# caki35/UNet-Torch

Measured on AMD Instinct MI355X. Metric: images/sec training step, 4-level U-Net 1ch→2cls 512×512, at 1/2/4/8 MI355X, higher is better.
Workload: dtype f16

## Files before the change

include/unetmi.h:

```cpp
#ifndef UNETMI_H
#define UNETMI_H
#include <stddef.h>
#include <stdint.h>

#ifdef __cplusplus
extern "C" {
#endif

typedef void* umi_stream_t;

enum { UMI_F32 = 0, UMI_F16 = 1 };
enum { UMI_OK = 0, UMI_ERR_BADARG = -1, UMI_ERR_UNSUPPORTED = -2, UMI_ERR_WORKSPACE = -3 };
enum { UMI_CONV_UPSAMPLE2 = 1,
       UMI_CONV_FORCE_GENERIC = 2,
       UMI_CONV_DGRAD_STRIDED = 4,
       UMI_CONV_ACCUMULATE = 8,
       UMI_CONV_F32_MFMA = 16,
       UMI_CONV_F32_MFMA_1X1 = 32   };

int umi_version(void);
const char* umi_arch(void);

int umi_tune_conv3x3_impl(int impl);

int umi_pack_kn(const float* src, void* dst, int T, int K, int N, long st, long sk, long sn,
                int flip_t, int Kpad, int Npad, int dtype, umi_stream_t stream);

int umi_pack_kn8(const float* src, void* dst, int T, int K, int N, long st, long sk, long sn,
                 int flip_t, int Kpad, int Npad, int dtype, umi_stream_t stream);

int umi_conv_fwd(const void* x, int ldx, const void* tx, const void* wp, const float* bias,
                 void* y, int ldy, float* stat_part,
                 int N, int H, int W, int Ci, int Co, int R, int S, int stride, int pad,
                 int Ho, int Wo, int off_h, int off_w, int out_H, int out_W,
                 int in_dtype, int out_dtype, int flags, umi_stream_t stream);
int umi_linear_fused(const void* x, int ldx, const void* wp8, const float* bias, void* y, int ldy, long M, int Ci, int Co,
                     int epi, float p, unsigned seed, const unsigned* seed_dev, void* mask, const void* aux, int ldaux,
                     void* y2, int ldy2, int dtype, umi_stream_t stream);

int umi_conv_fwd_plan(int N, int H, int W, int Ci, int Co, int R, int S, int stride, int pad,
                      int ldx, int ldy, int in_dtype, int out_dtype, int flags, int has_bias,
                      int* layout, int* stat_rows);

int umi_bn_finalize(const float* stat_part, int rows, int C, double count,
                    const float* gamma, const float* beta, float eps, float momentum,
                    float* running_mean, float* running_var,
                    void* tx_out, float* rstd_out, umi_stream_t stream);

int umi_pool2_fwd(const void* x, int ldx, const void* tx, void* y, int ldy,
                  int N, int H, int W, int C, int dtype, umi_stream_t stream);
int umi_pool2_bwd(const void* dpool, int lddp, const void* x, int ldx, const void* tx,
                  void* da, int ldda, int accumulate,
                  int N, int H, int W, int C, int dtype, umi_stream_t stream);

size_t umi_bn_bwd_ws_bytes(long M, int C);
int umi_bn_bwd_reduce(const void* da, int ldda, const void* y, int ldy, const void* tx,
                      const float* rstd, float* sum_dz, float* sum_dzx,
                      long M, int C, int dtype, void* ws, size_t ws_bytes, umi_stream_t stream);
int umi_bn_bwd_apply(void* da, int ldda, const void* y, int ldy, const void* tx,
                     const float* rstd, const float* sum_dz, const float* sum_dzx,
                     long M, int C, int dtype, umi_stream_t stream);

int umi_conv_dgrad_bnred(const void* dy, int lddy, const void* wp8, void* da, int ldda, const void* ybn, int ldybn,
                         const void* txbn, const float* rstd, float* part, int N, int H, int W, int Ci, int Co,
                         int dtype, umi_stream_t stream);

int umi_conv_gather_bnred_rows(int N, int H, int W, int Ci, int Co, int R, int S, int stride, int pad, int Ho, int Wo,
                               int ldx, int ldy, int dtype, int flags);
int umi_conv_gather_bnred(const void* x, int ldx, const void* wp8, void* y, int ldy, const void* ybn, int ldybn,
                          const void* txbn, const float* rstd, float* part, int N, int H, int W, int Ci, int Co, int R, int S,
                          int stride, int pad, int Ho, int Wo, int dtype, int flags, umi_stream_t stream);

int umi_head_dgrad_bnred_rows(long P, int Ci, int Co, int ldda, int dtype);
int umi_head_dgrad_bnred(const void* dl, int lddl, const void* wp, void* da, int ldda, const void* ybn, int ldybn,
                         const void* txbn, const float* rstd, float* part, long P, int Ci, int Co, int dtype,
                         umi_stream_t stream);
size_t umi_head_bwd_fused_ws_bytes(long P, int Ci, int Co);
int umi_head_bwd_fused(const void* dl, int lddl, const void* wp, void* da, int ldda, const void* ybn, int ldybn,
                       const void* txbn, const float* rstd, float* part, float* dW, long s_co, long s_ci, float out_scale,
                       void* ws, size_t ws_bytes, long P, int Ci, int Co, int dtype, umi_stream_t stream);

int umi_conv3x3_fwd_act(const void* x, int ldx, const void* tx, const void* wp8, const void* out_tx, void* y, int ldy,
                        int N, int H, int W, int Ci, int Co, int dtype, umi_stream_t stream);
int umi_bn_stats_rows(long M, int C);
int umi_bn_stats(const void* x, int ldx, float* part, long M, int C, int dtype, umi_stream_t stream);
int umi_pool2_bwd_bnred_stat_rows(int N, int H, int W, int C);
int umi_pool2_bwd_bnred(const void* dpool, int lddp, const void* x, int ldx, const void* tx, const float* rstd, void* da,
                        int ldda, int accumulate, float* part, int N, int H, int W, int C, int dtype, umi_stream_t stream);
int umi_bn_bwd_from_partials(const float* part, int rows, int C, float* sum_dz, float* sum_dzx, umi_stream_t stream);

size_t umi_conv_wgrad_ws_bytes(int N, int Ho, int Wo, int Ci, int Co, int R, int S, int dtype, int flags);
int umi_conv_wgrad(const void* x, int ldx, const void* txa, const void* dy, int lddy, const void* txb,
                   float* dW, long s_co, long s_ci, long s_t, float out_scale,
                   int N, int H, int W, int Ci, int Co, int R, int S, int stride, int pad,
                   int Ho, int Wo, int dtype, int flags, void* ws, size_t ws_bytes, umi_stream_t stream);
typedef struct umi_wgrad_pending {
    const float* part;
    float* dW;
    long s_co, s_ci, s_t;
    float scale;
    int splits, RS, Ci, Co;
} umi_wgrad_pending;
int umi_conv_wgrad_deferred(const void* x, int ldx, const void* txa, const void* dy, int lddy, const void* txb,
                            float* dW, long s_co, long s_ci, long s_t, float out_scale, int N, int H, int W, int Ci, int Co,
                            int R, int S, int stride, int pad, int Ho, int Wo, int dtype, int flags, void* ws, size_t ws_bytes,
                            umi_wgrad_pending* out, umi_stream_t stream);
int umi_wgrad_reduce_group(int n, const void* items , umi_stream_t stream);
int umi_conv_wgrad_bias(const void* x, int ldx, const void* dy, int lddy, const void* txb, float* dW, long s_co, long s_ci,
                        long s_t, float* dbias, float out_scale, int N, int H, int W, int Ci, int Co, int Ho, int Wo, int dtype,
                        int flags, void* ws, size_t ws_bytes, umi_wgrad_pending* out, umi_stream_t stream);
int umi_conv_wgrad_group(int n, const void* const* x, int ldx, const void* const* dy, int lddy, float* const* dW, long s_co,
                         long s_ci, float out_scale, long M, int Ci, int Co, int dtype, umi_stream_t stream);
int umi_conv_wgrad_bnapply(const void* x, int ldx, const void* txa, const void* da, int ldda, const void* y, int ldy,
                           const void* tx_bn, const float* rstd, const float* sum_dz, const float* sum_dzx, void* dz,
                           int lddz, float* dW, long s_co, long s_ci, long s_t, float out_scale, int N, int H, int W,
                           int Ci, int Co, int R, int S, int stride, int pad, int dtype, int flags, void* ws,
                           size_t ws_bytes, umi_stream_t stream);

size_t umi_colsum_ws_bytes(long M, int C);
int umi_colsum(const void* x, int ldx, float* out, float out_scale, long M, int C, int dtype,
               void* ws, size_t ws_bytes, umi_stream_t stream);
int umi_colsum_group(int n, const void* const* xs, int ldx, float* const* outs, float out_scale, long M, int C, int dtype,
                     void* ws, size_t ws_bytes, umi_stream_t stream);

int umi_materialize_nchw(const void* x, int ldx, const void* tx, float* y_nchw,
                         int N, int H, int W, int C, int dtype, umi_stream_t stream);


int umi_wstd_fwd(const float* w, float* wstd, float* rstd, int Co, int K, float eps, umi_stream_t stream);
int umi_wstd_bwd(const float* wstd, const float* rstd, const float* g, float* dw, int Co, int K, umi_stream_t stream);
typedef struct umi_wstd_desc {
    const float* w;
    float* ws;
    float* rstd;
    long off;
    int Co, K;
    float eps;
    int blk0;
    float* dw;
} umi_wstd_desc;
int umi_wstd_fwd_multi(const void* descs, int n_desc, int total_rows, umi_stream_t stream);
int umi_wstd_bwd_multi(const void* descs, int n_desc, int total_rows, const float* g_base, float* dw_base, umi_stream_t stream);

size_t umi_gn_fwd_ws_bytes(int N, long HW, int C);
int umi_gn_fwd(const void* x, int ldx, const float* gamma, const float* beta, const void* res, int ldr, void* y, int ldy,
               float* mean, float* rstd, int relu, int N, long HW, int C, int G, float eps, int dtype,
               void* ws, size_t ws_bytes, umi_stream_t stream);
size_t umi_gn_bwd_ws_bytes(int N, long HW, int C, int G);
int umi_gn_bwd(const void* dy, int lddy, const void* y, int ldy, const void* x, int ldx, const float* mean,
               const float* rstd, const float* gamma, int relu, void* dx, int lddx, void* dres, int lddr,
               float* dgamma, float* dbeta, float out_scale, int N, long HW, int C, int G, int dtype,
               void* ws, size_t ws_bytes, float* part_out, umi_stream_t stream);
int umi_gn_param_grads_group(int n, const float* const* parts, const int* Cs, int N, float* const* dgammas,
                             float* const* dbetas, float out_scale, umi_stream_t stream);

int umi_pool3s2_fwd(const void* x, int ldx, void* y, int ldy, void* idx, int N, int H, int W, int C, int dtype,
                    umi_stream_t stream);
int umi_pool3s2_bwd(const void* dy, int lddy, const void* x, int ldx, const void* idx, void* dx, int lddx, int N, int H, int W,
                    int C, int dtype, umi_stream_t stream);

int umi_ln_fwd(const void* x, int ldx, const float* gamma, const float* beta, void* y, int ldy, float* mean, float* rstd,
               long M, int C, float eps, int dtype, umi_stream_t stream);
size_t umi_ln_bwd_ws_bytes(long M, int C);
int umi_ln_bwd(const void* dy, int lddy, const void* x, int ldx, const float* gamma, const float* mean,
               const float* rstd, void* dx, int lddx, float* dgamma, float* dbeta, float out_scale, long M, int C,
               int dtype, void* ws, size_t ws_bytes, int* rows_out, umi_stream_t stream);

int umi_elementwise(int mode, const void* x, int ldx, const void* g, int ldg, void* y, int ldy, long M, int C,
                    long bcast_rows, int dtype, umi_stream_t stream);

int umi_dropout(const void* x, int ldx, void* y, int ldy, void* mask, int backward, float p, unsigned seed, long M, int C,
                int dtype, const void* tx, const unsigned* seed_dev, umi_stream_t stream);
int umi_dropout_fused(const void* x, int ldx, void* y, int ldy, void* mask, int backward, float p, unsigned seed, long M, int C,
                      int dtype, const unsigned* seed_dev, const void* aux, int ldaux, int gelu, umi_stream_t stream);

int umi_attn_fwd(const void* q, const void* k, const void* v, int ld, void* o, int ldo, float* lse, int B, int N, int heads,
                 int D, int dtype, umi_stream_t stream);
int umi_attn_bwd(const void* q, const void* k, const void* v, int ld, const void* o, const void* dO, int ldo,
                 const float* lse, void* dq, void* dk, void* dv, int ldd, float* delta, int B, int N, int heads, int D,
                 int dtype, umi_stream_t stream);
enum { UMI_ATTN_F32_MFMA = 1  };
int umi_attn_fwd_flags(const void* q, const void* k, const void* v, int ld, void* o, int ldo, float* lse, int B, int N, int heads,
                       int D, int dtype, int flags, umi_stream_t stream);
int umi_attn_bwd_flags(const void* q, const void* k, const void* v, int ld, const void* o, const void* dO, int ldo,
                       const float* lse, void* dq, void* dk, void* dv, int ldd, float* delta, int B, int N, int heads, int D,
                       int dtype, int flags, umi_stream_t stream);
int umi_attn_plan(int N, int heads, int D, int ld, int ldo, int ldd, int dtype, int flags, const void* q, const void* k,
                  const void* v, const void* o, int* kernel);

int umi_bilinear2x(const void* x, int ldx, const void* tx, void* y, int ldy, int backward, int N, int H, int W, int C,
                   int dtype, umi_stream_t stream);

size_t umi_dice_ce_ws_bytes(int N, int C, long HW);
int umi_dice_ce_fwd(const float* logits, const void* target, int target_dtype, int N, int C, long HW, float* stats, void* ws,
                    size_t ws_bytes, umi_stream_t stream);
int umi_dice_ce_bwd(const float* logits, const void* target, int target_dtype, const float* stats, const float* gout, int N,
                    int C, long HW, float* dlogits, umi_stream_t stream);

size_t umi_hdt_ws_bytes(int B, int H, int W);
int umi_hdt_fwd(const float* pred, const float* target, int B, int C, int H, int W, float alpha, float* D, float* fields,
                float* loss, void* ws, size_t ws_bytes, umi_stream_t stream);
int umi_hdt_bwd(const float* pred, const float* target, const float* D, const float* gout, int B, int C, int H, int W,
                float* dpred, umi_stream_t stream);

size_t umi_binloss_ws_bytes(int B, int C, long HW);
int umi_dice_bce_fwd(const float* pred, const float* target, int B, long HW, double* stats, float* loss, void* ws,
                     size_t ws_bytes, umi_stream_t stream);
int umi_dice_bce_bwd(const float* pred, const float* target, const double* stats, const float* gout, int B, long HW,
                     float* dpred, umi_stream_t stream);
int umi_tversky_fwd(const float* pred, const void* target, int target_dtype, int B, int C, long HW, float alpha, float beta,
                    double* stats, float* loss, void* ws, size_t ws_bytes, umi_stream_t stream);
int umi_tversky_bwd(const float* pred, const void* target, int target_dtype, const double* stats, const float* gout, int B,
                    int C, long HW, float alpha, float beta, float* dpred, umi_stream_t stream);

size_t umi_topk_loss_ws_bytes(long N);
int umi_topk_loss_fwd(const float* pred, const float* target, long N, long k, int mode, unsigned char* mask, float* loss,
                      void* ws, size_t ws_bytes, umi_stream_t stream);
int umi_topk_loss_bwd(const float* pred, const float* target, const unsigned char* mask, const float* gout, long N, long k,
                      float* dpred, umi_stream_t stream);

size_t umi_mt_ratio_ws_bytes(int B, long HW);
size_t umi_mt_ratio_stats_len(int B);
int umi_mt_ratio_fwd(const float* o1, const float* o2, const float* l1, const float* l2, int B, long HW, int gate,
                     const float* gate_dev, double* stats, float* loss, float* loss1, float* loss2, float* ratio, void* ws, size_t ws_bytes,
                     umi_stream_t stream);
int umi_mt_ratio_bwd(const float* o1, const float* o2, const float* l1, const float* l2, const double* stats,
                     const float* gout, int B, long HW, float* d1, float* d2, umi_stream_t stream);

typedef struct umi_optim_desc {
    float* p;
    const float* g;
    float* s0;
    float* s1;
    long n;
    int blk0;
    int pad_;
} umi_optim_desc;
int umi_optim_block_elems(void);
int umi_table_upload(const void* host_pinned, void* dev, size_t nbytes, umi_stream_t stream);
int umi_optim_sgd_multi(const void* descs, int n_desc, int total_blocks, double lr, double momentum, double dampening,
                        double weight_decay, int nesterov, int first_step, umi_stream_t stream);
int umi_optim_adam_multi(const void* descs, int n_desc, int total_blocks, double step_size, double beta1, double beta2,
                         double bc2_sqrt, double eps, double weight_decay, umi_stream_t stream);

typedef struct umi_optim_hyper {
    double lr, base_lr, iter, max_iter, power, adam_t, beta1, beta2;
    float lr_f, step_size_f, bc2_sqrt_f, pad_;
    double pad2_[2];
} umi_optim_hyper;
size_t umi_optim_hyper_bytes(void);
int umi_optim_hyper_pre(void* hyper, int adam, umi_stream_t stream);
int umi_optim_hyper_poly(void* hyper, umi_stream_t stream);
int umi_optim_sgd_multi_dev(const void* descs, int n_desc, int total_blocks, const void* hyper, double momentum,
                            double dampening, double weight_decay, int nesterov, int first_step, umi_stream_t stream);
int umi_optim_adam_multi_dev(const void* descs, int n_desc, int total_blocks, const void* hyper, double beta1, double beta2,
                             double eps, double weight_decay, umi_stream_t stream);

typedef struct umi_pack_desc {
    const float* src;
    void* dst;
    long st, sk, sn;
    int T, K, N, flip_t, Kpad, Npad, k8, blk0;
    int ldn, pad_;
} umi_pack_desc;
int umi_pack_block_elems(void);
int umi_pack_kn_multi(const void* descs, int n_desc, int total_blocks, int dtype, umi_stream_t stream);

int umi_add2_relu_fwd(const void* a, int lda, const void* txa, const void* b, int ldb, const void* txb, void* y, int ldy,
                      long M, int C, int dtype, umi_stream_t stream);
int umi_add2_relu_bwd(const void* dy, int lddy, const void* y, int ldy, void* da, int ldda, void* db, int lddb, long M, int C,
                      int dtype, umi_stream_t stream);
int umi_gate_fwd(const void* x, int ldx, const void* txx, const void* p, const void* txp, void* y, int ldy, long M, int C,
                 int dtype, umi_stream_t stream);
int umi_gate_bwd(const void* dy, int lddy, const void* x, int ldx, const void* txx, const void* p, const void* txp, void* dx,
                 int lddx, void* dp, long M, int C, int dtype, umi_stream_t stream);

size_t umi_znorm_ws_bytes(void);
int umi_znorm_hwc(const void* img, int src_dtype, float* out_chw, long HW, int C, int reverse_channels, void* ws,
                  size_t ws_bytes, umi_stream_t stream);
int umi_argmax_mask(const float* logits, unsigned char* mask, int N, int C, long HW, umi_stream_t stream);
size_t umi_zoom_cubic_ws_bytes(int H, int W, int C);
int umi_zoom_cubic_hwc(const void* img, int src_dtype, void* out, int H, int W, int C, int out_h, int out_w, void* ws,
                       size_t ws_bytes, umi_stream_t stream);

int umi_binary_mask(const float* logits, unsigned char* mask, long n, umi_stream_t stream);
int umi_zoom_nearest(const void* in, int dtype, void* out, int N, int H, int W, int out_h, int out_w, umi_stream_t stream);
size_t umi_sum_trunc_ws_bytes(int N);
int umi_sum_trunc(const float* x, int* out, int N, long HW, void* ws, size_t ws_bytes, umi_stream_t stream);

size_t umi_components_ws_bytes(int N, int H, int W);
int umi_components_cap(int H, int W);
int umi_count_components(const unsigned char* mask, int* counts, int N, int H, int W, void* ws, size_t ws_bytes,
                         umi_stream_t stream);
int umi_label_components(const unsigned char* mask, int* labels, int* counts, int* area, long long* sum_y, long long* sum_x,
                         int N, int H, int W, void* ws, size_t ws_bytes, umi_stream_t stream);

size_t umi_class_components_ws_bytes(int N, int H, int W, int n_classes);
int umi_count_class_components(const unsigned char* mask, int* class_counts, int N, int H, int W, int n_classes, void* ws,
                               size_t ws_bytes, umi_stream_t stream);
int umi_label_class_components(const unsigned char* mask, int* labels, int* counts, int* class_counts, unsigned char* label_class,
                               int* area, long long* sum_y, long long* sum_x, int N, int H, int W, int n_classes, int cap, void* ws,
                               size_t ws_bytes, umi_stream_t stream);

int umi_match_max_dots(void);
size_t umi_dot_lists_ws_bytes(int N, int H, int W);
int umi_dot_lists(const void* map, int dtype, int* dots, int* g_count, int N, int H, int W, int max_dots, void* ws, size_t ws_bytes,
                  umi_stream_t stream);
int umi_component_centers(const int* counts, const int* area, const long long* sum_y, const long long* sum_x, int* centers, int N,
                          int cap, umi_stream_t stream);
int umi_crowd_match(const int* dots, const int* g_count, int max_dots, const int* centers, const int* c_count, int cap,
                    const double* tables, size_t table_len, const int* radii, int S, const double* thresh, int T, int* out, int N,
                    umi_stream_t stream);
size_t umi_distance_match_ws_bytes(int N, int cap);
int umi_distance_match(const int* dots, const int* g_count, int max_dots, const int* centers, const int* c_count, int cap,
                       long long d2_max, int* out, int N, void* ws, size_t ws_bytes, umi_stream_t stream);
int umi_grid_sums(const void* map, int dtype, void* out, int N, int H, int W, int size, umi_stream_t stream);
int umi_scatter_centers(const int* centers, const int* c_count, int cap, unsigned char* map, int N, int H, int W,
                        umi_stream_t stream);
int umi_split_classes(const unsigned char* map, unsigned char* planes, int N, int H, int W, int n_classes, umi_stream_t stream);
int umi_class_center_lists(const int* counts, const unsigned char* label_class, const int* area, const long long* sum_y,
                           const long long* sum_x, int* centers, int* c_count, int N, int cap, int n_classes, umi_stream_t stream);

int umi_augment_geometry(const void* src, int dtype, void* dst, const int* params, const double* geom, int N, int H, int W, int C,
                         umi_stream_t stream);
int umi_augment_labels(const void* src, int src_dtype, void* dst, int dst_dtype, float scale, const int* params, const double* geom,
                       int N, int H, int W, int out_h, int out_w, umi_stream_t stream);
size_t umi_augment_znorm_ws_bytes(int N);
int umi_augment_znorm(const void* src, int dtype, float* out_nchw, const int* params, const double* geom, int N, int H, int W, int C,
                      int reverse_channels, void* ws, size_t ws_bytes, umi_stream_t stream);

#ifdef __cplusplus
}
#endif
#endif
```

unet-torch_amd/csrc/api.hip:

```cpp
#include "kernels.h"
#include <stdio.h>
#include <stdlib.h>

static ConvFwdProblem fwd_problem(int N, int H, int W, int Ci, int Co, int R, int S, int stride, int pad, int Ho, int Wo, int ldx,
                                  int ldy, int in_dtype, int out_dtype, int flags, bool has_tx, bool has_bias, bool has_stats) {
    return ConvFwdProblem{N, H, W, Ci, Co, R, S, stride, pad, Ho, Wo, ldx, ldy, in_dtype, out_dtype, flags, has_tx, has_bias, has_stats};
}
static ConvFwdProblem fwd_problem_3x3(int N, int H, int W, int Ci, int Co, int ldx, int ldy, int dtype, bool has_tx) {
    return fwd_problem(N, H, W, Ci, Co, 3, 3, 1, 1, H, W, ldx, ldy, dtype, dtype, 0, has_tx, false, false);
}

extern "C" int umi_version(void) { return 1; }
extern "C" const char* umi_arch(void) { return "gfx950"; }

extern "C" int umi_linear_fused(const void* x, int ldx, const void* wp8, const float* bias, void* y, int ldy, long M, int Ci,
                                int Co, int epi, float p, unsigned seed, const unsigned* seed_dev, void* mask, const void* aux,
                                int ldaux, void* y2, int ldy2, int dtype, umi_stream_t stream) {
    if (!x || !wp8 || !y || !mask || M <= 0 || M >= (1L << 31) || Ci <= 0 || Co <= 0 || !(p >= 0.f && p <= 1.f)) return UMI_ERR_BADARG;
    if (epi != 1 && epi != 2) return UMI_ERR_BADARG;
    if ((epi == 1 && (!y2 || ldy2 % 8)) || (epi == 2 && (!aux || ldaux % 8))) return UMI_ERR_BADARG;
    const ConvFwdProblem pr = fwd_problem(1, 1, (int)M, Ci, Co, 1, 1, 1, 0, 1, (int)M, ldx, ldy, dtype, dtype, 0, false, bias != nullptr, false);
    if (umi_conv_fwd_path(pr) != FWD_MFMA1X1) return UMI_ERR_UNSUPPORTED;
    if (((uintptr_t)x | (uintptr_t)y | (uintptr_t)wp8 | (uintptr_t)y2 | (uintptr_t)aux) & 15 || ((uintptr_t)mask & 7)) return UMI_ERR_UNSUPPORTED;
    const UmiLinearEpi e{epi, p, seed, seed_dev, mask, aux, ldaux, y2, ldy2, nullptr, nullptr, nullptr};
    return umi_conv1x1_mfma(pr, x, nullptr, wp8, bias, y, 0, 0, 1, (int)M, (hipStream_t)stream, &e);
}

extern "C" int umi_conv_gather_bnred_rows(int N, int H, int W, int Ci, int Co, int R, int S, int stride, int pad, int Ho, int Wo,
                                          int ldx, int ldy, int dtype, int flags) {
    if (flags & (UMI_CONV_UPSAMPLE2 | UMI_CONV_ACCUMULATE | UMI_CONV_FORCE_GENERIC)) return 0;
    const ConvFwdProblem p = fwd_problem(N, H, W, Ci, Co, R, S, stride, pad, Ho, Wo, ldx, ldy, dtype, dtype, flags, false, false, false);
    if (umi_conv_fwd_path(p) != FWD_MFMA1X1 || umi_conv3x3_mfma_ok(p)) return 0;
    return umi_conv1x1_bnred_rows((long)N * Ho * Wo, Co);
}
extern "C" int umi_conv_gather_bnred(const void* x, int ldx, const void* wp8, void* y, int ldy, const void* ybn, int ldybn,
                                     const void* txbn, const float* rstd, float* part, int N, int H, int W, int Ci, int Co, int R,
                                     int S, int stride, int pad, int Ho, int Wo, int dtype, int flags, umi_stream_t stream) {
    if (!x || !wp8 || !y || !ybn || !txbn || !rstd || !part || N <= 0 || H <= 0 || W <= 0) return UMI_ERR_BADARG;
    if (umi_conv_gather_bnred_rows(N, H, W, Ci, Co, R, S, stride, pad, Ho, Wo, ldx, ldy, dtype, flags) <= 0 || ldybn % 8 || ldybn < Co)
        return UMI_ERR_UNSUPPORTED;
    if (((uintptr_t)x | (uintptr_t)y | (uintptr_t)wp8 | (uintptr_t)ybn) & 15) return UMI_ERR_BADARG;
    const UmiLinearEpi e{3, 0.f, 0u, nullptr, nullptr, ybn, ldybn, nullptr, 0, txbn, rstd, part};
    const ConvFwdProblem p = fwd_problem(N, H, W, Ci, Co, R, S, stride, pad, Ho, Wo, ldx, ldy, dtype, dtype, flags, false, false, false);
    return umi_conv1x1_mfma(p, x, nullptr, wp8, nullptr, y, 0, 0, Ho, Wo, (hipStream_t)stream, &e);
}

extern "C" int umi_conv_fwd_plan(int N, int H, int W, int Ci, int Co, int R, int S, int stride, int pad, int ldx,
                                 int ldy, int in_dtype, int out_dtype, int flags, int has_bias, int* layout,
                                 int* stat_rows) {
    if (N <= 0 || H <= 0 || W <= 0 || Ci <= 0 || Co <= 0 || R <= 0 || S <= 0 || stride <= 0) return UMI_ERR_BADARG;
    const bool ups = flags & UMI_CONV_UPSAMPLE2;
    const int Ho = ups ? H : (H + 2 * pad - R) / stride + 1, Wo = ups ? W : (W + 2 * pad - S) / stride + 1;
    const ConvFwdPath path = umi_conv_fwd_path(fwd_problem(N, H, W, Ci, Co, R, S, stride, pad, Ho, Wo, ldx, ldy, in_dtype, out_dtype,
                                                           flags, false, has_bias != 0, true));
    if ((flags & UMI_CONV_ACCUMULATE) && path != FWD_MFMA1X1) return UMI_ERR_UNSUPPORTED;
    if (layout) *layout = (path == FWD_MFMA3X3 || path == FWD_MFMA1X1) ? 1 : 0;
    if (stat_rows)
        *stat_rows = path == FWD_MFMA3X3_F32 ? umi_conv3x3_f32_mfma_stat_rows(N, H, W)
                     : path == FWD_GEMM_F32 ? umi_gemm_f32_mfma_stat_rows((long)N * H * W)
                     : path == FWD_MFMA3X3 ? umi_conv3x3_mfma_stat_rows(N, H, W, Co)
                     : path == FWD_STEM  ? umi_stem_stat_rows(N, H, W)
                     : path == FWD_HEAD  ? umi_head_stat_rows((long)N * H * W, Ci)
                                         : umi_cdiv((long)N * Ho * Wo, 64);
    return UMI_OK;
}

extern "C" int umi_conv_dgrad_bnred(const void* dy, int lddy, const void* wp8, void* da, int ldda, const void* ybn, int ldybn,
                                    const void* txbn, const float* rstd, float* part, int N, int H, int W, int Ci, int Co,
                                    int dtype, umi_stream_t stream) {
    if (!dy || !wp8 || !da || !ybn || !txbn || !rstd || !part || N <= 0 || H <= 0 || W <= 0) return UMI_ERR_BADARG;
    const ConvFwdProblem p = fwd_problem_3x3(N, H, W, Ci, Co, lddy, ldda, dtype, false);
    if (umi_conv_fwd_path(p) != FWD_MFMA3X3 || ldybn % 8 || ldybn < Co) return UMI_ERR_UNSUPPORTED;
    if (((uintptr_t)dy | (uintptr_t)da | (uintptr_t)wp8 | (uintptr_t)ybn) & 15) return UMI_ERR_BADARG;
    return umi_conv3x3_mfma_bnred(p, dy, wp8, da, ybn, ldybn, txbn, rstd, part, (hipStream_t)stream);
}

static bool head_dgrad_ok(int Ci, int Co, int ldda, int dtype) {
    return umi_smallk_fwd_ok(fwd_problem(1, 1, 1, Ci, Co, 1, 1, 1, 0, 1, 1, Ci, ldda, dtype, dtype, 0, false, false, false));
}
extern "C" int umi_head_dgrad_bnred_rows(long P, int Ci, int Co, int ldda, int dtype) {
    if (!head_dgrad_ok(Ci, Co, ldda, dtype)) return 0;
    return umi_smallk_bnred_rows(P, Co);
}
extern "C" int umi_head_dgrad_bnred(const void* dl, int lddl, const void* wp, void* da, int ldda, const void* ybn, int ldybn,
                                    const void* txbn, const float* rstd, float* part, long P, int Ci, int Co, int dtype,
                                    umi_stream_t stream) {
    if (!dl || !wp || !da || !ybn || !txbn || !rstd || !part || P <= 0) return UMI_ERR_BADARG;
    if (!head_dgrad_ok(Ci, Co, ldda, dtype) || ldybn % 8 || ldybn < Co || lddl < Ci) return UMI_ERR_UNSUPPORTED;
    return umi_smallk_fwd_bnred(dl, lddl, wp, da, ldda, ybn, ldybn, txbn, rstd, part, P, Ci, Co, (hipStream_t)stream);
}
extern "C" size_t umi_head_bwd_fused_ws_bytes(long P, int Ci, int Co) {
    return (size_t)umi_smallk_bnred_rows(P, Co) * Co * Ci * sizeof(float);
}
extern "C" int umi_head_bwd_fused(const void* dl, int lddl, const void* wp, void* da, int ldda, const void* ybn, int ldybn,
                                  const void* txbn, const float* rstd, float* part, float* dW, long s_co, long s_ci, float out_scale,
                                  void* ws, size_t ws_bytes, long P, int Ci, int Co, int dtype, umi_stream_t stream) {
    if (!dl || !wp || !da || !ybn || !txbn || !rstd || !part || !dW || !ws || P <= 0) return UMI_ERR_BADARG;
    if (!head_dgrad_ok(Ci, Co, ldda, dtype) || Co > 256 || ldybn % 8 || ldybn < Co || lddl < Ci) return UMI_ERR_UNSUPPORTED;
    return umi_smallk_fwd_bnred(dl, lddl, wp, da, ldda, ybn, ldybn, txbn, rstd, part, P, Ci, Co, (hipStream_t)stream, dW, s_co, s_ci,
                                out_scale, ws, ws_bytes);
}

extern "C" int umi_conv3x3_fwd_act(const void* x, int ldx, const void* tx, const void* wp8, const void* out_tx, void* y, int ldy,
                                   int N, int H, int W, int Ci, int Co, int dtype, umi_stream_t stream) {
    if (!x || !wp8 || !out_tx || !y || N <= 0 || H <= 0 || W <= 0 || ldx < Ci || ldy < Co) return UMI_ERR_BADARG;
    const ConvFwdProblem p = fwd_problem_3x3(N, H, W, Ci, Co, ldx, ldy, dtype, tx != nullptr);
    if (umi_conv_fwd_path(p) != FWD_MFMA3X3) return UMI_ERR_UNSUPPORTED;
    if (((uintptr_t)x | (uintptr_t)y | (uintptr_t)wp8 | (uintptr_t)out_tx) & 15) return UMI_ERR_BADARG;
    return umi_conv3x3_mfma_act(p, x, tx, wp8, out_tx, y, (hipStream_t)stream);
}

extern "C" int umi_bn_stats_rows(long M, int C) { return umi_colsum_rows_f16v(M, C); }
extern "C" int umi_bn_stats(const void* x, int ldx, float* part, long M, int C, int dtype, umi_stream_t stream) {
    if (!x || !part || M <= 0 || C <= 0 || ldx < C) return UMI_ERR_BADARG;
    if (dtype != UMI_F16 || !umi_bn_stats_f16v(x, ldx, part, M, C, (hipStream_t)stream)) return UMI_ERR_UNSUPPORTED;
    UMI_LAUNCH_CHECK();
    return UMI_OK;
}

extern "C" int umi_pool2_bwd_bnred(const void* dpool, int lddp, const void* x, int ldx, const void* tx, const float* rstd,
                                   void* da, int ldda, int accumulate, float* part, int N, int H, int W, int C, int dtype,
                                   umi_stream_t stream) {
    if (!dpool || !x || !tx || !rstd || !da || !part || N <= 0 || H <= 0 || W <= 0 || C <= 0) return UMI_ERR_BADARG;
    if (dtype != UMI_F16) return UMI_ERR_UNSUPPORTED;
    if (!umi_pool2_bwd_bnred_f16v(dpool, lddp, x, ldx, tx, rstd, da, ldda, accumulate, part, N, H, W, C, (hipStream_t)stream))
        return UMI_ERR_UNSUPPORTED;
    UMI_LAUNCH_CHECK();
    return UMI_OK;
}
extern "C" int umi_pool2_bwd_bnred_stat_rows(int N, int H, int W, int C) { return umi_pool2_bwd_bnred_rows(N, H, W, C); }

extern "C" int umi_bn_bwd_from_partials(const float* part, int rows, int C, float* sum_dz, float* sum_dzx, umi_stream_t stream) {
    if (!part || !sum_dz || !sum_dzx || rows <= 0 || C <= 0) return UMI_ERR_BADARG;
    umi_launch_reduce_rows2(part, rows, C, sum_dz, sum_dzx, 1.f, (hipStream_t)stream);
    UMI_LAUNCH_CHECK();
    return UMI_OK;
}

static bool trace_generic() {
    static const bool on = [] { const char* e = getenv("UMI_TRACE_GENERIC"); return e && e[0] == '1'; }();
    return on;
}
#define UMI_TRACE(kind)                                                                                                  \
    if (trace_generic())                                                                                                 \
        fprintf(stderr, "[umi generic %s] N=%d H=%d W=%d Ci=%d Co=%d R=%d stride=%d pad=%d flags=%d\n", kind, N, H, W, Ci, Co, R, \
                stride, pad, flags)

extern "C" int umi_conv_fwd(const void* x, int ldx, const void* tx, const void* wp, const float* bias, void* y, int ldy,
                            float* stat_part, int N, int H, int W, int Ci, int Co, int R, int S, int stride, int pad,
                            int Ho, int Wo, int off_h, int off_w, int out_H, int out_W, int in_dtype, int out_dtype,
                            int flags, umi_stream_t stream) {
    if (!x || !wp || !y || N <= 0 || H <= 0 || W <= 0 || Ci <= 0 || Co <= 0 || R <= 0 || S <= 0 || stride <= 0 ||
        Ho <= 0 || Wo <= 0 || ldx < Ci || ldy < Co || out_H <= 0 || out_W <= 0)
        return UMI_ERR_BADARG;
    ConvFwdProblem p = fwd_problem(N, H, W, Ci, Co, R, S, stride, pad, Ho, Wo, ldx, ldy, in_dtype, out_dtype, flags,
                                   tx != nullptr, bias != nullptr, stat_part != nullptr);
    const ConvFwdPath path = umi_conv_fwd_path(p);
    if (path != FWD_MFMA3X3_F32 && path != FWD_GEMM_F32) p.flags = flags &= ~UMI_CONV_F32_OPT_IN;
    if ((flags & UMI_CONV_ACCUMULATE) && (stat_part || path != FWD_MFMA1X1)) return UMI_ERR_UNSUPPORTED;
    if (flags & UMI_CONV_DGRAD_STRIDED) {
        if (flags & UMI_CONV_UPSAMPLE2) return UMI_ERR_BADARG;
        if (H != (Ho + 2 * pad - R) / stride + 1 || W != (Wo + 2 * pad - S) / stride + 1) return UMI_ERR_BADARG;
        if (out_H != Ho || out_W != Wo || off_h || off_w || stat_part) return UMI_ERR_BADARG;
    } else if (!(flags & UMI_CONV_UPSAMPLE2)) {
        if (Ho != (H + 2 * pad - R) / stride + 1 || Wo != (W + 2 * pad - S) / stride + 1) return UMI_ERR_BADARG;
        if (out_H != Ho || out_W != Wo || off_h || off_w) return UMI_ERR_BADARG;
    } else {
        if (Ho != H || Wo != W) return UMI_ERR_BADARG;
    }
    const hipStream_t s = (hipStream_t)stream;
    switch (path) {
    case FWD_MFMA3X3_F32: return umi_conv3x3_f32_mfma(p, x, tx, wp, y, stat_part, s);
    case FWD_GEMM_F32: return umi_gemm_f32_mfma(p, x, tx, wp, bias, y, stat_part, s);
    case FWD_MFMA3X3:
        if (((uintptr_t)x | (uintptr_t)y | (uintptr_t)wp) & 15) return UMI_ERR_BADARG;
        return umi_conv3x3_mfma(p, x, tx, wp, y, stat_part, s);
    case FWD_MFMA1X1:
        if (stat_part) return UMI_ERR_UNSUPPORTED;
        if (((uintptr_t)x | (uintptr_t)y | (uintptr_t)wp) & 15) return UMI_ERR_BADARG;
        return umi_conv1x1_mfma(p, x, tx, wp, bias, y, off_h, off_w, out_H, out_W, s);
    case FWD_STEM: return umi_stem_fwd(p, x, tx, wp, y, stat_part, s);
    case FWD_HEAD: return umi_head_fwd(p, x, tx, wp, bias, y, stat_part, s);
    case FWD_SMALLK: return umi_smallk_fwd(p, x, wp, y, s);
    case FWD_ROOT: return umi_root_fwd(p, x, wp, y, s);
    case FWD_HEAD3: return umi_head3_fwd(p, x, tx, wp, bias, y, s);
    case FWD_GENERIC: break;
    }
    UMI_TRACE((flags & UMI_CONV_DGRAD_STRIDED) ? "dgrad_strided" : "fwd");
    return umi_conv_fwd_generic(p, x, tx, wp, bias, y, stat_part, off_h, off_w, out_H, out_W, s);
}

static WgradProblem wgrad_problem(int N, int H, int W, int Ci, int Co, int R, int S, int stride, int pad, int Ho, int Wo, int ldx,
                                  int lddy, int dtype, int flags, bool has_txa, bool has_txb) {
    return WgradProblem{N, H, W, Ci, Co, R, S, stride, pad, Ho, Wo, ldx, lddy, dtype, flags, has_txa, has_txb};
}

extern "C" size_t umi_conv_wgrad_ws_bytes(int N, int Ho, int Wo, int Ci, int Co, int R, int S, int dtype, int flags) {
    WgradProblem p = wgrad_problem(N, 0, 0, Ci, Co, R, S, 0, 0, Ho, Wo, 0, 0, dtype, flags, false, false);
    const size_t f32_mfma = umi_wgrad3x3_f32_mfma_ws_bound(p), f32_gemm = umi_wgrad_gemm_f32_mfma_ws_bound(p);
    p.flags &= ~UMI_CONV_F32_OPT_IN;
    const size_t bounds[] = {f32_mfma, f32_gemm, umi_wgrad3x3_mfma_ws_bound(p), umi_wgrad1x1_mfma_ws_bound(p), umi_wgradT_mfma_ws_bound(p),
                             umi_wgrad_gather_mfma_ws_bound(p), umi_stem_wgrad_ws_bound(p), umi_head_wgrad_ws_bound(p),
                             umi_root_wgrad_ws_bound(p), umi_head3_wgrad_ws_bound(p), umi_conv_wgrad_generic_ws_bound(p)};
    size_t most = 0;
    for (size_t b : bounds) most = b > most ? b : most;
    return most;
}

static int conv_wgrad(const WgradProblem& asked, WgradPath path, const void* x, const void* txa, const void* dy, const void* txb,
                      const WgradOut& o, hipStream_t s) {
    WgradProblem p = asked;
    if (path != WGRAD_MFMA3X3_F32 && path != WGRAD_GEMM_F32) p.flags &= ~UMI_CONV_F32_OPT_IN;
    if (!x || !dy || !o.dW || !o.ws || p.N <= 0 || p.H <= 0 || p.W <= 0 || p.Ci <= 0 || p.Co <= 0 || p.ldx < p.Ci || p.lddy < p.Co)
        return UMI_ERR_BADARG;
    switch (path) {
    case WGRAD_MFMA3X3_F32: return umi_wgrad3x3_f32_mfma(p, x, txa, dy, o, s);
    case WGRAD_GEMM_F32: return umi_wgrad_gemm_f32_mfma(p, x, txa, dy, o, s);
    case WGRAD_MFMA3X3: return umi_wgrad3x3_mfma(p, x, txa, dy, o, s);
    case WGRAD_MFMA1X1: return umi_wgrad1x1_mfma(p, x, txa, dy, o, s);
    case WGRAD_T: return umi_wgradT_mfma(p, x, dy, txb, o, s);
    case WGRAD_GATHER: return umi_wgrad_gather_mfma(p, x, txa, dy, o, s);
    case WGRAD_STEM: return umi_stem_wgrad(p, x, txa, dy, o, s);
    case WGRAD_HEAD: return umi_head_wgrad(p, x, txa, dy, o, s);
    case WGRAD_ROOT: return umi_root_wgrad(p, x, dy, o, s);
    case WGRAD_HEAD3: return umi_head3_wgrad(p, x, txa, dy, o, s);
    case WGRAD_GENERIC: break;
    }
    if (trace_generic())
        fprintf(stderr, "[umi generic wgrad] N=%d H=%d W=%d Ci=%d Co=%d R=%d stride=%d pad=%d flags=%d\n", p.N, p.H, p.W, p.Ci, p.Co,
                p.R, p.stride, p.pad, p.flags);
    return umi_conv_wgrad_generic(p, x, txa, dy, txb, o, s);
}

extern "C" int umi_conv_wgrad(const void* x, int ldx, const void* txa, const void* dy, int lddy, const void* txb,
                              float* dW, long s_co, long s_ci, long s_t, float out_scale, int N, int H, int W, int Ci,
                              int Co, int R, int S, int stride, int pad, int Ho, int Wo, int dtype, int flags, void* ws,
                              size_t ws_bytes, umi_stream_t stream) {
    const WgradProblem p = wgrad_problem(N, H, W, Ci, Co, R, S, stride, pad, Ho, Wo, ldx, lddy, dtype, flags, txa != nullptr, txb != nullptr);
    const WgradOut o{dW, s_co, s_ci, s_t, out_scale, ws, ws_bytes, nullptr, nullptr};
    return conv_wgrad(p, umi_conv_wgrad_path(p), x, txa, dy, txb, o, (hipStream_t)stream);
}

extern "C" int umi_conv_wgrad_deferred(const void* x, int ldx, const void* txa, const void* dy, int lddy, const void* txb,
                                       float* dW, long s_co, long s_ci, long s_t, float out_scale, int N, int H, int W, int Ci,
                                       int Co, int R, int S, int stride, int pad, int Ho, int Wo, int dtype, int flags, void* ws,
                                       size_t ws_bytes, umi_wgrad_pending* out, umi_stream_t stream) {
    if (!out) return UMI_ERR_BADARG;
    out->part = nullptr;
    const WgradProblem p = wgrad_problem(N, H, W, Ci, Co, R, S, stride, pad, Ho, Wo, ldx, lddy, dtype, flags, txa != nullptr, txb != nullptr);
    const WgradOut o{dW, s_co, s_ci, s_t, out_scale, ws, ws_bytes, out, nullptr};
    return conv_wgrad(p, umi_conv_wgrad_path(p), x, txa, dy, txb, o, (hipStream_t)stream);
}

extern "C" int umi_conv_wgrad_bias(const void* x, int ldx, const void* dy, int lddy, const void* txb, float* dW, long s_co,
                                   long s_ci, long s_t, float* dbias, float out_scale, int N, int H, int W, int Ci, int Co, int Ho,
                                   int Wo, int dtype, int flags, void* ws, size_t ws_bytes, umi_wgrad_pending* out,
                                   umi_stream_t stream) {
    if (!dbias) return UMI_ERR_BADARG;
    const WgradProblem p = wgrad_problem(N, H, W, Ci, Co, 2, 2, 2, 0, Ho, Wo, ldx, lddy, dtype, flags, false, txb != nullptr);
    if (umi_conv_wgrad_path(p) != WGRAD_T) return UMI_ERR_UNSUPPORTED;
    if (out) out->part = nullptr;
    const WgradOut o{dW, s_co, s_ci, s_t, out_scale, ws, ws_bytes, out, dbias};
    return conv_wgrad(p, WGRAD_T, x, nullptr, dy, txb, o, (hipStream_t)stream);
}

extern "C" int umi_conv_wgrad_group(int n, const void* const* x, int ldx, const void* const* dy, int lddy, float* const* dW,
                                    long s_co, long s_ci, float out_scale, long M, int Ci, int Co, int dtype,
                                    umi_stream_t stream) {
    if (n <= 0 || !x || !dy || !dW || M <= 0 || Ci <= 0 || Co <= 0 || ldx < Ci || lddy < Co) return UMI_ERR_BADARG;
    for (int i = 0; i < n; ++i)
        if (!x[i] || !dy[i] || !dW[i]) return UMI_ERR_BADARG;
    if (M >= (1L << 31) ||
        umi_conv_wgrad_path(wgrad_problem(1, 1, (int)M, Ci, Co, 1, 1, 1, 0, 1, (int)M, ldx, lddy, dtype, 0, false, false)) != WGRAD_MFMA1X1)
        return UMI_ERR_UNSUPPORTED;
    return umi_wgrad1x1_mfma_group(n, x, ldx, dy, lddy, dW, s_co, s_ci, out_scale, M, Ci, Co, (hipStream_t)stream);
}

extern "C" int umi_conv_wgrad_bnapply(const void* x, int ldx, const void* txa, const void* da, int ldda, const void* y, int ldy,
                                      const void* tx_bn, const float* rstd, const float* sum_dz, const float* sum_dzx,
                                      void* dz, int lddz, float* dW, long s_co, long s_ci, long s_t, float out_scale, int N,
                                      int H, int W, int Ci, int Co, int R, int S, int stride, int pad, int dtype, int flags,
                                      void* ws, size_t ws_bytes, umi_stream_t stream) {
    if (!x || !da || !y || !tx_bn || !rstd || !sum_dz || !sum_dzx || !dW || !ws || N <= 0 || H <= 0 || W <= 0 || Ci <= 0 ||
        Co <= 0 || ldx < Ci || ldda < Co || ldy < Co || (dz && (lddz < Co || dz == da || dz == y)))
        return UMI_ERR_BADARG;
    const WgradProblem p = wgrad_problem(N, H, W, Ci, Co, R, S, stride, pad, H, W, ldx, ldda, dtype, flags, txa != nullptr, false);
    const WgradPath path = umi_conv_wgrad_path(p);
    const WgradOut o{dW, s_co, s_ci, s_t, out_scale, ws, ws_bytes, nullptr, nullptr};
    const WgradBnApply bna{y, ldy, tx_bn, rstd, sum_dz, sum_dzx, dz, lddz};
    if (!dz) {
        if (path != WGRAD_STEM || ldy % 8) return UMI_ERR_UNSUPPORTED;
        return umi_stem_wgrad(p, x, txa, da, o, (hipStream_t)stream, &bna);
    }
    if (path != WGRAD_MFMA3X3 || ldy % 8 || lddz % 8 || (long)H * W * (ldy > lddz ? ldy : lddz) * 2 >= 0x7FFFFFF0L)
        return UMI_ERR_UNSUPPORTED;
    return umi_wgrad3x3_mfma(p, x, txa, da, o, (hipStream_t)stream, &bna);
}
```

unet-torch_amd/csrc/generic_kernels.hip:

```cpp
#include "kernels.h"

template <typename T, bool K8>
__global__ void pack_kn_kernel(const float* __restrict__ src, T* __restrict__ dst, int Tn, int K, int N,
                               long st, long sk, long sn, int flip_t, int Kpad, int Npad) {
    long total = (long)Tn * Kpad * Npad;
    for (long i = (long)blockIdx.x * blockDim.x + threadIdx.x; i < total; i += (long)gridDim.x * blockDim.x) {
        int n, k, t;
        if (K8) {
            int k8 = (int)(i & 7);
            long r = i >> 3;
            n = (int)(r % Npad); r /= Npad;
            int kb = (int)(r % (Kpad / 8));
            t = (int)(r / (Kpad / 8));
            k = kb * 8 + k8;
        } else {
            n = (int)(i % Npad);
            long r = i / Npad;
            k = (int)(r % Kpad);
            t = (int)(r / Kpad);
        }
        float v = 0.f;
        if (k < K && n < N) {
            int ts = flip_t ? (Tn - 1 - t) : t;
            v = src[ts * st + k * sk + n * sn];
// ... 523 lines not shown
            vs[i] = ws[((long)rc * 2 + 0) * C + c];
            vq[i] = ws[((long)rc * 2 + w1) * C + c];
        }
#pragma unroll
        for (int i = 0; i < 8; ++i) asm volatile("" : "+v"(vs[i]), "+v"(vq[i]));
#pragma unroll
        for (int i = 0; i < 8; ++i) { const bool ok = r0 + 256 * i < rows; vs[i] = ok ? vs[i] : 0.f; vq[i] = (ok && out1) ? vq[i] : 0.f; }
#pragma unroll
        for (int i = 0; i < 8; ++i) { s += (double)vs[i]; q += (double)vq[i]; }
    }
    sh[0][tid] = s;
    sh[1][tid] = q;
    __syncthreads();
    for (int o = 128; o > 0; o >>= 1) {
        if (tid < o) { sh[0][tid] += sh[0][tid + o]; sh[1][tid] += sh[1][tid + o]; }
        __syncthreads();
    }
    if (tid == 0) {
        out0[c] = (float)(sh[0][0] * (double)scale);
        if (out1) out1[c] = (float)(sh[1][0] * (double)scale);
    }
}

__global__ __launch_bounds__(256) void reduce_rows2_2d_kernel(const float* __restrict__ ws, int rows, int C,
                                                              float* __restrict__ out0, float* __restrict__ out1,
                                                              float scale, int region) {
    double tot = 0.0;
    if (!red2d_block(ws, rows, C, out1 != nullptr, region, tot)) return;
    const int lane = threadIdx.x & 63, c = blockIdx.x * 32 + (lane & 31);
    if (c < C) {
        if (lane < 32) out0[c] = (float)(tot * (double)scale);
        else if (out1) out1[c] = (float)(tot * (double)scale);
    }
}

__global__ __launch_bounds__(256) void reduce_rows2_wide_kernel(const float* __restrict__ ws, int rows, int C,
                                                                float* __restrict__ out0, float* __restrict__ out1, float scale) {
    const int c = blockIdx.x * 256 + threadIdx.x;
    if (c >= C) return;
    double s = 0.0, q = 0.0;
    for (int r = 0; r < rows; ++r) {
        s += (double)ws[((long)r * 2 + 0) * C + c];
        if (out1) q += (double)ws[((long)r * 2 + 1) * C + c];
    }
    out0[c] = (float)(s * (double)scale);
    if (out1) out1[c] = (float)(q * (double)scale);
}

void umi_launch_reduce_rows2(const float* ws, int rows, int C, float* out0, float* out1, float scale, hipStream_t s) {
    if (rows <= 64 && C >= 4096)
        hipLaunchKernelGGL(reduce_rows2_wide_kernel, dim3((C + 255) / 256), dim3(256), 0, s, ws, rows, C, out0, out1, scale);
    else if (red2d_ok(rows, C))
        hipLaunchKernelGGL(reduce_rows2_2d_kernel, dim3((C + 31) / 32, (rows + RED_RPS - 1) / RED_RPS), dim3(256), 0, s, ws,
                           rows, C, out0, out1, scale, red2d_region());
    else
        hipLaunchKernelGGL(reduce_rows2_kernel, dim3(C), dim3(256), 0, s, ws, rows, C, out0, out1, scale);
}

template <typename T>
__global__ void bn_bwd_apply_kernel(T* __restrict__ da, int ldda, const T* __restrict__ y, int ldy,
                                    const float4* __restrict__ tx, const float* __restrict__ rstd,
                                    const float* __restrict__ sum_dz, const float* __restrict__ sum_dzx, long M, int C) {
    const float invM = 1.f / (float)M;
    long total = M * C;
    for (long i = (long)blockIdx.x * blockDim.x + threadIdx.x; i < total; i += (long)gridDim.x * blockDim.x) {
        int c = (int)(i % C);
        long r = i / C;
        da[r * ldda + c] = umi_bn_dz<T>((float)y[r * ldy + c], (float)da[r * ldda + c], tx[c], rstd[c], sum_dz[c] * invM,
                                        sum_dzx[c] * invM);
    }
}

extern "C" size_t umi_bn_bwd_ws_bytes(long M, int C) {
    const int a = umi_cdiv(M, BNB_RPB), b = umi_cdiv(M, umi_bn_bwd_rpb_f16v(M));
    return (size_t)(a > b ? a : b) * 2 * (size_t)C * sizeof(float);
}

extern "C" int umi_bn_bwd_reduce(const void* da, int ldda, const void* y, int ldy, const void* tx, const float* rstd,
                                 float* sum_dz, float* sum_dzx, long M, int C, int dtype, void* ws, size_t ws_bytes,
                                 umi_stream_t stream) {
    if (!da || !y || !tx || !rstd || M <= 0 || C <= 0) return UMI_ERR_BADARG;
    if (ws_bytes < umi_bn_bwd_ws_bytes(M, C)) return UMI_ERR_WORKSPACE;
    int rows = umi_cdiv(M, BNB_RPB);
    hipStream_t s = (hipStream_t)stream;
    if (dtype == UMI_F16 && umi_bn_bwd_reduce1_f16v(da, ldda, y, ldy, tx, rstd, (float*)ws, M, C, s)) {
        UMI_LAUNCH_CHECK();
        rows = umi_cdiv(M, umi_bn_bwd_rpb_f16v(M));
        umi_launch_reduce_rows2((const float*)ws, rows, C, sum_dz, sum_dzx, 1.f, s);
        UMI_LAUNCH_CHECK();
        return UMI_OK;
    }
    if (dtype == UMI_F32) hipLaunchKernelGGL(bn_bwd_reduce1_kernel<float>, dim3(rows), dim3(256), 0, s, (const float*)da, ldda, (const float*)y, ldy, (const float4*)tx, rstd, (float*)ws, M, C);
    else if (dtype == UMI_F16) hipLaunchKernelGGL(bn_bwd_reduce1_kernel<half_t>, dim3(rows), dim3(256), 0, s, (const half_t*)da, ldda, (const half_t*)y, ldy, (const float4*)tx, rstd, (float*)ws, M, C);
    else return UMI_ERR_BADARG;
    UMI_LAUNCH_CHECK();
    umi_launch_reduce_rows2((const float*)ws, rows, C, sum_dz, sum_dzx, 1.f, s);
    UMI_LAUNCH_CHECK();
    return UMI_OK;
}

extern "C" int umi_bn_bwd_apply(void* da, int ldda, const void* y, int ldy, const void* tx, const float* rstd,
                                const float* sum_dz, const float* sum_dzx, long M, int C, int dtype,
                                umi_stream_t stream) {
    if (!da || !y || !tx || !rstd || M <= 0 || C <= 0) return UMI_ERR_BADARG;
    long total = M * C;
    int grid = (int)((total + 255) / 256);
    if (grid > 16384) grid = 16384;
    hipStream_t s = (hipStream_t)stream;
    if (dtype == UMI_F16 && umi_bn_bwd_apply_f16v(da, ldda, y, ldy, tx, rstd, sum_dz, sum_dzx, M, C, s)) {
        UMI_LAUNCH_CHECK();
        return UMI_OK;
    }
    if (dtype == UMI_F32) hipLaunchKernelGGL(bn_bwd_apply_kernel<float>, dim3(grid), dim3(256), 0, s, (float*)da, ldda, (const float*)y, ldy, (const float4*)tx, rstd, sum_dz, sum_dzx, M, C);
    else if (dtype == UMI_F16) hipLaunchKernelGGL(bn_bwd_apply_kernel<half_t>, dim3(grid), dim3(256), 0, s, (half_t*)da, ldda, (const half_t*)y, ldy, (const float4*)tx, rstd, sum_dz, sum_dzx, M, C);
    else return UMI_ERR_BADARG;
    UMI_LAUNCH_CHECK();
    return UMI_OK;
}

template <typename T>
__global__ __launch_bounds__(256) void colsum1_kernel(const T* __restrict__ x, int ldx, float* __restrict__ ws, long M,
                                                      int C, long rows_per_split, float* __restrict__ out, float scale) {
    __shared__ float red[4][64];
    const int cl = threadIdx.x & 63, rl = threadIdx.x >> 6;
    const int c = blockIdx.x * 64 + cl;
    const long r0 = (long)blockIdx.y * rows_per_split;
    long r1 = r0 + rows_per_split;
    if (r1 > M) r1 = M;
    float s = 0.f;
    if (c < C)
        for (long r = r0 + rl; r < r1; r += 4) s += (float)x[r * ldx + c];
    red[rl][cl] = s;
    __syncthreads();
    if (rl == 0 && c < C) {
        const float t = red[0][cl] + red[1][cl] + red[2][cl] + red[3][cl];
        if (gridDim.y == 1) out[c] = t * scale;
        else ws[((long)blockIdx.y * 2 + 0) * C + c] = t;
    }
}

__global__ void fold_cols_kernel(const float* __restrict__ tmp8, int C, float* __restrict__ out, float scale) {
    const int c = threadIdx.x;
    if (c < C) {
        float s = 0.f;
        for (int k = c; k < 8; k += C) s += tmp8[k];
        out[c] = s * scale;
    }
}

static void colsum_plan(long M, int C, int* splits, long* rps) {
    long ctiles = (C + 63) / 64;
    long want = (1024 + ctiles - 1) / ctiles;
    long maxs = (M + 31) / 32;
    if (want > maxs) want = maxs;
    if (want < 1) want = 1;
    *rps = (M + want - 1) / want;
    *splits = (int)((M + *rps - 1) / *rps);
}

extern "C" size_t umi_colsum_ws_bytes(long M, int C) {
    int splits; long rps;
    colsum_plan(M, C, &splits, &rps);
    const int vrows = umi_colsum_rows_f16v(M, C);
    size_t b = (size_t)(splits > vrows ? splits : vrows) * 2 * (size_t)C * sizeof(float);
    if (C < 8 && 8 % C == 0 && (M * C) % 8 == 0) {
        const size_t b8 = ((size_t)umi_colsum_rows_f16v(M * C / 8, 8) * 2 * 8 + 8) * sizeof(float);
        if (b8 > b) b = b8;
    }
    return b;
}

extern "C" int umi_colsum_group(int n, const void* const* xs, int ldx, float* const* outs, float out_scale, long M, int C,
                                int dtype, void* ws, size_t ws_bytes, umi_stream_t stream) {
    if (n <= 0 || !xs || !outs || M <= 0 || C <= 0 || !ws) return UMI_ERR_BADARG;
    for (int i = 0; i < n; ++i)
        if (!xs[i] || !outs[i]) return UMI_ERR_BADARG;
    if (ws_bytes < (size_t)(n < 16 ? n : 16) * umi_colsum_ws_bytes(M, C)) return UMI_ERR_WORKSPACE;
    if (dtype != UMI_F16 || !umi_colsum_group_f16v(n, xs, ldx, outs, out_scale, (float*)ws, M, C, (hipStream_t)stream))
        return UMI_ERR_UNSUPPORTED;
    UMI_LAUNCH_CHECK();
    return UMI_OK;
}

extern "C" int umi_colsum(const void* x, int ldx, float* out, float out_scale, long M, int C, int dtype, void* ws,
                          size_t ws_bytes, umi_stream_t stream) {
    if (!x || !out || M <= 0 || C <= 0) return UMI_ERR_BADARG;
    if (ws_bytes < umi_colsum_ws_bytes(M, C)) return UMI_ERR_WORKSPACE;
    int splits; long rps;
    colsum_plan(M, C, &splits, &rps);
    hipStream_t s = (hipStream_t)stream;
    if (dtype == UMI_F16 && umi_colsum_f16v(x, ldx, (float*)ws, M, C, s)) {
        UMI_LAUNCH_CHECK();
        umi_launch_reduce_rows2((const float*)ws, umi_colsum_rows_f16v(M, C), C, out, (float*)nullptr, out_scale, s);
        UMI_LAUNCH_CHECK();
        return UMI_OK;
    }
    if (dtype == UMI_F16 && C < 8 && 8 % C == 0 && ldx == C && (M * C) % 8 == 0 &&
        ws_bytes >= ((size_t)umi_colsum_rows_f16v(M * C / 8, 8) * 2 * 8 + 8) * sizeof(float)) {
        const long M8 = M * C / 8;
        float* tmp = (float*)ws + (size_t)umi_colsum_rows_f16v(M8, 8) * 2 * 8;
        if (umi_colsum_f16v(x, 8, (float*)ws, M8, 8, s)) {
            UMI_LAUNCH_CHECK();
            umi_launch_reduce_rows2((const float*)ws, umi_colsum_rows_f16v(M8, 8), 8, tmp, (float*)nullptr, 1.f, s);
            hipLaunchKernelGGL(fold_cols_kernel, dim3(1), dim3(64), 0, s, (const float*)tmp, C, out, out_scale);
            UMI_LAUNCH_CHECK();
            return UMI_OK;
        }
    }
    dim3 grid((C + 63) / 64, splits);
    if (dtype == UMI_F32) hipLaunchKernelGGL(colsum1_kernel<float>, grid, dim3(256), 0, s, (const float*)x, ldx, (float*)ws, M, C, rps, out, out_scale);
    else if (dtype == UMI_F16) hipLaunchKernelGGL(colsum1_kernel<half_t>, grid, dim3(256), 0, s, (const half_t*)x, ldx, (float*)ws, M, C, rps, out, out_scale);
    else return UMI_ERR_BADARG;
    UMI_LAUNCH_CHECK();
    if (splits > 1) {
        umi_launch_reduce_rows2((const float*)ws, splits, C, out, (float*)nullptr, out_scale, s);
        UMI_LAUNCH_CHECK();
    }
    return UMI_OK;
}

template <typename T>
__global__ __launch_bounds__(256) void wgrad_generic_kernel(
    const T* __restrict__ x, int ldx, const float4* __restrict__ txa, const T* __restrict__ dy, int lddy,
    const float4* __restrict__ txb, float* __restrict__ part, int N, int H, int W, int Ci, int Co, int R, int S,
    int stride, int pad, int Ho, int Wo, long chunk, int tiles_co) {
    __shared__ __attribute__((aligned(16))) float As[GBK][64 + 4];
    __shared__ __attribute__((aligned(16))) float Bs[GBK][64 + 4];
    const int tid = threadIdx.x;
    const int txi = tid & 15, tyi = tid >> 4;
    const int tile_ci = blockIdx.x / tiles_co, tile_co = blockIdx.x % tiles_co;
    const int ci0 = tile_ci * 64, co0 = tile_co * 64;
    const int tap = blockIdx.y;
    const int r = tap / S, s = tap - r * S;
    const long P = (long)N * Ho * Wo;
    const long k_begin = (long)blockIdx.z * chunk;
    long k_end = k_begin + chunk;
    if (k_end > P) k_end = P;

    const int lk = tid >> 4;
    const int lc = (tid & 15) * 4;
    float acc[4][4];
#pragma unroll
    for (int i = 0; i < 4; ++i)
#pragma unroll
        for (int j = 0; j < 4; ++j) acc[i][j] = 0.f;

    for (long k0 = k_begin; k0 < k_end; k0 += GBK) {
        long pg = k0 + lk;
        bool pv = pg < k_end;
        int n = 0, ho = 0, wo = 0;
        if (pv) {
            n = (int)(pg / ((long)Ho * Wo));
            int rem = (int)(pg - (long)n * Ho * Wo);
            ho = rem / Wo;
            wo = rem - ho * Wo;
        }
        int hi = ho * stride - pad + r, wi = wo * stride - pad + s;
        bool inb = pv && hi >= 0 && hi < H && wi >= 0 && wi < W;
        const T* xp = x + ((long)((long)n * H + hi) * W + wi) * ldx;
        const T* dp = dy + pg * lddy;
#pragma unroll
        for (int j = 0; j < 4; ++j) {
            int ci = ci0 + lc + j;
            float v = 0.f;
            if (inb && ci < Ci) {
                v = (float)xp[ci];
                if (txa) v = umi_tx(v, txa[ci]);
            }
            As[lk][lc + j] = v;
            int co = co0 + lc + j;
            float g = 0.f;
            if (pv && co < Co) {
                g = (float)dp[co];
                if (txb) g = umi_tx(g, txb[co]);
            }
            Bs[lk][lc + j] = g;
        }
        __syncthreads();
#pragma unroll
        for (int kk = 0; kk < GBK; ++kk) {
            float4 a = *(const float4*)&As[kk][tyi * 4];
            float4 b = *(const float4*)&Bs[kk][txi * 4];
            float av[4] = {a.x, a.y, a.z, a.w};
            float bv[4] = {b.x, b.y, b.z, b.w};
#pragma unroll
            for (int i = 0; i < 4; ++i)
#pragma unroll
                for (int j = 0; j < 4; ++j) acc[i][j] = fmaf(av[i], bv[j], acc[i][j]);
        }
        __syncthreads();
    }
#pragma unroll
    for (int i = 0; i < 4; ++i) {
        int ci = ci0 + tyi * 4 + i;
        if (ci >= Ci) continue;
#pragma unroll
        for (int j = 0; j < 4; ++j) {
            int co = co0 + txi * 4 + j;
            if (co < Co) part[(((long)blockIdx.z * R * S + tap) * Ci + ci) * Co + co] = acc[i][j];
        }
    }
}

__global__ __launch_bounds__(256) void wgrad_reduce_kernel(const float* __restrict__ part, int splits, int RS, int Ci,
                                                           int Co, float* __restrict__ dW, long s_co, long s_ci, long s_t,
                                                           float scale) {
    __shared__ float red[8][33];
    const long total = (long)RS * Ci * Co;
    const int ox = threadIdx.x & 31, sl = threadIdx.x >> 5;
    for (long base = (long)blockIdx.x * 32; base < total; base += (long)gridDim.x * 32) {
        long i = base + ox;
        float s = 0.f;
        if (i < total)
            for (int z = sl; z < splits; z += 8) s += part[(long)z * total + i];
        red[sl][ox] = s;
        __syncthreads();
        if (sl == 0 && i < total) {
            float a = 0.f;
#pragma unroll
            for (int k = 0; k < 8; ++k) a += red[k][ox];
            int co = (int)(i % Co);
            long rr = i / Co;
            int ci = (int)(rr % Ci);
            int t = (int)(rr / Ci);
            dW[co * s_co + ci * s_ci + t * s_t] = a * scale;
        }
        __syncthreads();
    }
}

__global__ __launch_bounds__(256) void wgrad_reduce_v4_kernel(const float* __restrict__ part, int splits, int RS, int Ci,
                                                              int Co, float* __restrict__ dW, long s_co, long s_ci, long s_t,
                                                              float scale) {
    __shared__ float4 red[8][33];
    const long total4 = (long)RS * Ci * Co / 4;
    const int Co4 = Co >> 2;
    const int ox = threadIdx.x & 31, sl = threadIdx.x >> 5;
    for (long base = (long)blockIdx.x * 32; base < total4; base += (long)gridDim.x * 32) {
        const long i = base + ox;
        float4 a = make_float4(0.f, 0.f, 0.f, 0.f), b = a;
        if (i < total4) {
            const float4* p = reinterpret_cast<const float4*>(part) + i;
            int z = sl;
            for (; z + 8 < splits; z += 16) {
                float4 u = p[(long)z * total4], v = p[(long)(z + 8) * total4];
                a.x += u.x; a.y += u.y; a.z += u.z; a.w += u.w;
                b.x += v.x; b.y += v.y; b.z += v.z; b.w += v.w;
            }
            if (z < splits) { float4 u = p[(long)z * total4]; a.x += u.x; a.y += u.y; a.z += u.z; a.w += u.w; }
        }
        red[sl][ox] = make_float4(a.x + b.x, a.y + b.y, a.z + b.z, a.w + b.w);
        __syncthreads();
        if (sl == 0 && i < total4) {
            float4 t4 = red[0][ox];
#pragma unroll
            for (int k = 1; k < 8; ++k) { float4 u = red[k][ox]; t4.x += u.x; t4.y += u.y; t4.z += u.z; t4.w += u.w; }
            const int co = (int)(i % Co4) * 4;
            const long rr = i / Co4;
            const int ci = (int)(rr % Ci), t = (int)(rr / Ci);
            float* o = dW + ci * s_ci + t * s_t;
            o[(co + 0) * s_co] = t4.x * scale;
            o[(co + 1) * s_co] = t4.y * scale;
            o[(co + 2) * s_co] = t4.z * scale;
            o[(co + 3) * s_co] = t4.w * scale;
        }
        __syncthreads();
    }
}

constexpr int WGT_CO = 32, WGT_CI = 8;
__host__ __device__ inline int wg_tmode(const umi_wgrad_pending& d) {
    if (d.Co % WGT_CO || d.Ci % WGT_CI || d.RS > 9 || d.s_t != 1 || (((uintptr_t)d.part) & 15)) return 0;
    if ((long)(d.Co / WGT_CO) * (d.Ci / WGT_CI) < 512) return 0;
    if (d.s_ci == d.RS && d.s_co == (long)d.Ci * d.RS) return 1;
    if (d.s_co == d.RS && d.s_ci == (long)d.Co * d.RS) return 2;
    return 0;
}
__device__ void wg_reduce_tiles(const umi_wgrad_pending& d, int mode, int my_blk, int n_blk) {
    __shared__ float4 redt[8][33];
    __shared__ float tile[WGT_CO * WGT_CI * 9 + 64];
    const int ox = threadIdx.x & 31, sl = threadIdx.x >> 5;
    const int RS = d.RS, ncob = d.Co / WGT_CO, ncib = d.Ci / WGT_CI, rows = WGT_CI * RS;
    const long total4 = (long)RS * d.Ci * d.Co / 4;
    for (int tl = my_blk; tl < ncob * ncib; tl += n_blk) {
        const int cob = tl % ncob, cib = tl / ncob;
        for (int r0 = 0; r0 < rows; r0 += 4) {
            const int row = r0 + (ox >> 3), c4 = ox & 7;
            const int tap = row / WGT_CI, cil = row - tap * WGT_CI;
            float4 a = make_float4(0.f, 0.f, 0.f, 0.f), b = a;
            if (row < rows) {
                const float4* p = reinterpret_cast<const float4*>(d.part) + (((long)tap * d.Ci + cib * WGT_CI + cil) * d.Co + cob * WGT_CO) / 4 + c4;
                int z = sl;
                for (; z + 8 < d.splits; z += 16) {
                    float4 u = p[(long)z * total4], v = p[(long)(z + 8) * total4];
                    a.x += u.x; a.y += u.y; a.z += u.z; a.w += u.w;
                    b.x += v.x; b.y += v.y; b.z += v.z; b.w += v.w;
                }
                if (z < d.splits) { float4 u = p[(long)z * total4]; a.x += u.x; a.y += u.y; a.z += u.z; a.w += u.w; }
                a = make_float4(a.x + b.x, a.y + b.y, a.z + b.z, a.w + b.w);
            }
            redt[sl][ox] = a;
            __syncthreads();
            if (sl == 0 && row < rows) {
                float4 t4 = redt[0][ox];
#pragma unroll
                for (int k = 1; k < 8; ++k) { float4 u = redt[k][ox]; t4.x += u.x; t4.y += u.y; t4.z += u.z; t4.w += u.w; }
                const float v[4] = {t4.x * d.scale, t4.y * d.scale, t4.z * d.scale, t4.w * d.scale};
#pragma unroll
                for (int k = 0; k < 4; ++k) {
                    const int co = c4 * 4 + k;
                    const int idx = mode == 1 ? co * (WGT_CI * RS + 1) + cil * RS + tap : cil * (WGT_CO * RS + 1) + co * RS + tap;
                    tile[idx] = v[k];
                }
            }
            __syncthreads();
        }
        const int inner = mode == 1 ? WGT_CI * RS : WGT_CO * RS, outer = mode == 1 ? WGT_CO : WGT_CI;
        for (int e = threadIdx.x; e < inner * outer; e += 256) {
            const int o = e / inner, r = e - o * inner;
            float* dst = mode == 1 ? d.dW + (long)(cob * WGT_CO + o) * d.s_co + (long)(cib * WGT_CI) * d.s_ci + r
                                   : d.dW + (long)(cib * WGT_CI + o) * d.s_ci + (long)(cob * WGT_CO) * d.s_co + r;
            *dst = tile[o * (inner + 1) + r];
        }
        __syncthreads();
    }
}

struct WgTable { umi_wgrad_pending e[16]; int blk0[17]; };
__global__ __launch_bounds__(256) void wgrad_reduce_group_kernel(WgTable t) {
    __shared__ float4 red[8][33];
    int ent = 0;
#pragma unroll
    for (int i = 1; i < 16; ++i) ent += (int)blockIdx.x >= t.blk0[i];
    const umi_wgrad_pending d = t.e[ent];
    const int my_blk = (int)blockIdx.x - t.blk0[ent], n_blk = t.blk0[ent + 1] - t.blk0[ent];
    if (const int tm = wg_tmode(d)) { wg_reduce_tiles(d, tm, my_blk, n_blk); return; }
    const int ox = threadIdx.x & 31, sl = threadIdx.x >> 5;
    const bool vec = d.Co % 4 == 0 && (((uintptr_t)d.part) & 15) == 0;
    const int W4 = vec ? 4 : 1;
    const long total = (long)d.RS * d.Ci * d.Co / W4;
    const int CoW = d.Co / W4;
    for (long base = (long)my_blk * 32; base < total; base += (long)n_blk * 32) {
        const long i = base + ox;
        float4 a = make_float4(0.f, 0.f, 0.f, 0.f), b = a;
        if (i < total) {
            if (vec) {
                const float4* p = reinterpret_cast<const float4*>(d.part) + i;
                int z = sl;
                for (; z + 8 < d.splits; z += 16) {
                    float4 u = p[(long)z * total], v = p[(long)(z + 8) * total];
                    a.x += u.x; a.y += u.y; a.z += u.z; a.w += u.w;
                    b.x += v.x; b.y += v.y; b.z += v.z; b.w += v.w;
                }
                if (z < d.splits) { float4 u = p[(long)z * total]; a.x += u.x; a.y += u.y; a.z += u.z; a.w += u.w; }
                a = make_float4(a.x + b.x, a.y + b.y, a.z + b.z, a.w + b.w);
            } else {
                for (int z = sl; z < d.splits; z += 8) a.x += d.part[(long)z * total + i];
            }
        }
        red[sl][ox] = a;
        __syncthreads();
        if (sl == 0 && i < total) {
            float4 t4 = red[0][ox];
            if (vec) {
#pragma unroll
                for (int k = 1; k < 8; ++k) { float4 u = red[k][ox]; t4.x += u.x; t4.y += u.y; t4.z += u.z; t4.w += u.w; }
            } else {
                float s0 = 0.f;
#pragma unroll
                for (int k = 0; k < 8; ++k) s0 += red[k][ox].x;
                t4.x = s0;
            }
            const int co = (int)(i % CoW) * W4;
            const long rr = i / CoW;
            const int ci = (int)(rr % d.Ci), tp = (int)(rr / d.Ci);
            float* o = d.dW + ci * d.s_ci + tp * d.s_t;
            o[(co + 0) * d.s_co] = t4.x * d.scale;
            if (vec) {
                o[(co + 1) * d.s_co] = t4.y * d.scale;
                o[(co + 2) * d.s_co] = t4.z * d.scale;
                o[(co + 3) * d.s_co] = t4.w * d.scale;
            }
        }
        __syncthreads();
    }
}

extern "C" int umi_wgrad_reduce_group(int n, const void* items, umi_stream_t stream) {
    if (n <= 0 || !items) return UMI_ERR_BADARG;
    const umi_wgrad_pending* it = (const umi_wgrad_pending*)items;
    for (int i = 0; i < n; ++i)
        if (!it[i].part || !it[i].dW || it[i].splits <= 0 || it[i].RS <= 0 || it[i].Ci <= 0 || it[i].Co <= 0) return UMI_ERR_BADARG;
    for (int g0 = 0; g0 < n; g0 += 16) {
        const int cnt = n - g0 < 16 ? n - g0 : 16;
        WgTable t;
        int total_blk = 0;
        for (int i = 0; i < 16; ++i) {
            t.e[i] = it[g0 + (i < cnt ? i : 0)];
            t.blk0[i] = total_blk;
            if (i >= cnt) continue;
            const bool vec = t.e[i].Co % 4 == 0 && (((uintptr_t)t.e[i].part) & 15) == 0;
            long g = ((long)t.e[i].RS * t.e[i].Ci * t.e[i].Co / (vec ? 4 : 1) + 31) / 32;
            if (wg_tmode(t.e[i])) g = (long)(t.e[i].Co / WGT_CO) * (t.e[i].Ci / WGT_CI);
            total_blk += (int)(g > 4096 ? 4096 : g);
        }
        t.blk0[16] = total_blk;
        hipLaunchKernelGGL(wgrad_reduce_group_kernel, dim3((unsigned)total_blk), dim3(256), 0, (hipStream_t)stream, t);
        UMI_LAUNCH_CHECK();
    }
    return UMI_OK;
}

void umi_launch_wgrad_reduce(int splits, int RS, int Ci, int Co, const WgradOut& o, hipStream_t st) {
    const float* part = (const float*)o.ws;
    float* const dW = o.dW;
    const long s_co = o.s_co, s_ci = o.s_ci, s_t = o.s_t;
    const float scale = o.out_scale;
    if (o.defer) {
        *o.defer = umi_wgrad_pending{part, dW, s_co, s_ci, s_t, scale, splits, RS, Ci, Co};
        return;
    }
    {
        const umi_wgrad_pending one{part, dW, s_co, s_ci, s_t, scale, splits, RS, Ci, Co};
        if (wg_tmode(one)) {
            WgTable t;
            for (int i = 0; i < 16; ++i) { t.e[i] = one; t.blk0[i] = 0; }
            long g = (long)(Co / WGT_CO) * (Ci / WGT_CI);
            if (g > 4096) g = 4096;
            for (int i = 1; i <= 16; ++i) t.blk0[i] = (int)g;
            hipLaunchKernelGGL(wgrad_reduce_group_kernel, dim3((unsigned)g), dim3(256), 0, st, t);
            return;
        }
    }
    if (Co % 4 == 0 && (((uintptr_t)part) & 15) == 0) {
        long g4 = ((long)RS * Ci * Co / 4 + 31) / 32;
        if (g4 > 16384) g4 = 16384;
        hipLaunchKernelGGL(wgrad_reduce_v4_kernel, dim3((unsigned)g4), dim3(256), 0, st, part, splits, RS, Ci, Co, dW, s_co, s_ci, s_t, scale);
        return;
    }
    long total = (long)RS * Ci * Co;
    long g = (total + 31) / 32;
    if (g > 16384) g = 16384;
    hipLaunchKernelGGL(wgrad_reduce_kernel, dim3((unsigned)g), dim3(256), 0, st, part, splits, RS, Ci, Co, dW, s_co, s_ci, s_t, scale);
}


static void wgrad_generic_plan(long P, int Ci, int Co, int RS, int* splits, long* chunk) {
    long tiles = (long)umi_cdiv(Ci, 64) * umi_cdiv(Co, 64) * RS;
    long want = (2048 + tiles - 1) / tiles;
    long maxs = (P + 255) / 256;
    if (want > maxs) want = maxs;
    if (want < 1) want = 1;
    long ch = (P + want - 1) / want;
    ch = (ch + GBK - 1) / GBK * GBK;
    *chunk = ch;
    *splits = (int)((P + ch - 1) / ch);
}

size_t umi_conv_wgrad_generic_ws_bound(const WgradProblem& p) {
    int splits; long chunk;
    wgrad_generic_plan((long)p.N * p.Ho * p.Wo, p.Ci, p.Co, p.R * p.S, &splits, &chunk);
    return (size_t)splits * p.R * p.S * p.Ci * p.Co * sizeof(float);
}

int umi_conv_wgrad_generic(const WgradProblem& p, const void* x, const void* txa, const void* dy, const void* txb,
                           const WgradOut& o, hipStream_t st) {
    const int N = p.N, H = p.H, W = p.W, Ci = p.Ci, Co = p.Co, R = p.R, S = p.S, stride = p.stride, pad = p.pad, Ho = p.Ho, Wo = p.Wo,
              ldx = p.ldx, lddy = p.lddy, dtype = p.dtype;
    void* const ws = o.ws;
    if (o.ws_bytes < umi_conv_wgrad_generic_ws_bound(p)) return UMI_ERR_WORKSPACE;
    int splits; long chunk;
    wgrad_generic_plan((long)N * Ho * Wo, Ci, Co, R * S, &splits, &chunk);
    const int tiles_co = umi_cdiv(Co, 64);
    dim3 grid(umi_cdiv(Ci, 64) * tiles_co, R * S, splits), block(256);
    if (dtype == UMI_F32) hipLaunchKernelGGL(wgrad_generic_kernel<float>, grid, block, 0, st, (const float*)x, ldx, (const float4*)txa, (const float*)dy, lddy, (const float4*)txb, (float*)ws, N, H, W, Ci, Co, R, S, stride, pad, Ho, Wo, chunk, tiles_co);
    else if (dtype == UMI_F16) hipLaunchKernelGGL(wgrad_generic_kernel<half_t>, grid, block, 0, st, (const half_t*)x, ldx, (const float4*)txa, (const half_t*)dy, lddy, (const float4*)txb, (float*)ws, N, H, W, Ci, Co, R, S, stride, pad, Ho, Wo, chunk, tiles_co);
    else return UMI_ERR_BADARG;
    UMI_LAUNCH_CHECK();
    umi_launch_wgrad_reduce(splits, R * S, Ci, Co, o, st);
    UMI_LAUNCH_CHECK();
    return UMI_OK;
}

template <typename T>
__global__ void materialize_nchw_kernel(const T* __restrict__ x, int ldx, const float4* __restrict__ tx,
                                        float* __restrict__ y, int N, int H, int W, int C) {
    long total = (long)N * C * H * W;
    for (long i = (long)blockIdx.x * blockDim.x + threadIdx.x; i < total; i += (long)gridDim.x * blockDim.x) {
        int w = (int)(i % W);
        long r = i / W;
        int h = (int)(r % H);
        r /= H;
        int c = (int)(r % C);
        int n = (int)(r / C);
        float v = (float)x[((long)((long)n * H + h) * W + w) * ldx + c];
        if (tx) v = umi_tx(v, tx[c]);
        y[i] = v;
    }
}

extern "C" int umi_materialize_nchw(const void* x, int ldx, const void* tx, float* y, int N, int H, int W, int C,
                                    int dtype, umi_stream_t stream) {
    if (!x || !y || N <= 0 || H <= 0 || W <= 0 || C <= 0) return UMI_ERR_BADARG;
    long total = (long)N * C * H * W;
    int grid = (int)((total + 255) / 256);
    if (grid > 16384) grid = 16384;
    hipStream_t s = (hipStream_t)stream;
    if (dtype == UMI_F32) hipLaunchKernelGGL(materialize_nchw_kernel<float>, dim3(grid), dim3(256), 0, s, (const float*)x, ldx, (const float4*)tx, y, N, H, W, C);
    else if (dtype == UMI_F16) hipLaunchKernelGGL(materialize_nchw_kernel<half_t>, dim3(grid), dim3(256), 0, s, (const half_t*)x, ldx, (const float4*)tx, y, N, H, W, C);
    else return UMI_ERR_BADARG;
    UMI_LAUNCH_CHECK();
    return UMI_OK;
}
```

unet-torch_amd/csrc/optim_kernels.hip:

```cpp
#include "common.h"
#include <stdint.h>

namespace {

constexpr int OPT_BLOCK = 4096;
constexpr int PACK_BLOCK = 2048;

template <typename D>
__device__ inline int find_desc(const D* d, int n, int blk) {
    int lo = 0, hi = n - 1;
    while (lo < hi) {
        int mid = (lo + hi + 1) >> 1;
        if (d[mid].blk0 <= blk) lo = mid; else hi = mid - 1;
    }
    return lo;
}

struct Hyper {
    double lr, base_lr, iter, max_iter, power, adam_t, beta1, beta2;
    float lr_f, step_size_f, bc2_sqrt_f, pad_;
    double pad2_[2];
};
static_assert(sizeof(Hyper) == 96, "umi_optim_hyper is 96 bytes");

struct SgdArgs { float lr, momentum, omd, wd; int nesterov, first; const Hyper* hp; };

__device__ inline void sgd_one(float& p, float g, float& m, const SgdArgs a) {
    if (a.wd != 0.f) g = fmaf(a.wd, p, g);
    if (a.momentum != 0.f) {
        if (a.first) m = g;
        else {
            float mm = __fmul_rn(m, a.momentum);
            m = a.omd == 1.f ? __fadd_rn(mm, g) : fmaf(a.omd, g, mm);
        }
        g = a.nesterov ? fmaf(a.momentum, m, g) : m;
    }
    p = fmaf(-a.lr, g, p);
}

struct AdamArgs { float step_size, omb1, beta2, omb2, bc2_sqrt, eps, wd; const Hyper* hp; };

__device__ inline void adam_one(float& p, float g, float& m, float& v, const AdamArgs a) {
    if (a.wd != 0.f) g = fmaf(a.wd, p, g);
    m = fmaf(a.omb1, g - m, m);
    v = fmaf(a.omb2 * g, g, __fmul_rn(v, a.beta2));
    const float denom = __fdiv_rn(__fsqrt_rn(v), a.bc2_sqrt) + a.eps;
    p = fmaf(-a.step_size, __fdiv_rn(m, denom), p);
}

template <bool ADAM, typename A>
__global__ __launch_bounds__(256) void optim_multi_kernel(const umi_optim_desc* __restrict__ descs, int n_desc, A a) {
    if (a.hp) {
        if constexpr (ADAM) { a.step_size = a.hp->step_size_f; a.bc2_sqrt = a.hp->bc2_sqrt_f; }
        else a.lr = a.hp->lr_f;
    }
    const int blk = blockIdx.x;
    const umi_optim_desc d = descs[find_desc(descs, n_desc, blk)];
    const long base = (long)(blk - d.blk0) * OPT_BLOCK;
    const long left = d.n - base;
    const int cnt = left < OPT_BLOCK ? (int)left : OPT_BLOCK;
    float* p = d.p + base;
    const float* g = d.g + base;
    float* s0 = d.s0 ? d.s0 + base : nullptr;
    float* s1 = d.s1 ? d.s1 + base : nullptr;
    const unsigned long al = (unsigned long)p | (unsigned long)g | (unsigned long)s0 | (unsigned long)s1;
    if ((al & 15) == 0) {
        for (int i = threadIdx.x * 4; i + 4 <= cnt; i += 1024) {
            float4 pv = *reinterpret_cast<float4*>(p + i);
            const float4 gv = *reinterpret_cast<const float4*>(g + i);
            float4 mv = s0 ? *reinterpret_cast<float4*>(s0 + i) : make_float4(0.f, 0.f, 0.f, 0.f);
            float4 vv = (ADAM && s1) ? *reinterpret_cast<float4*>(s1 + i) : make_float4(0.f, 0.f, 0.f, 0.f);
            if constexpr (ADAM) {
                adam_one(pv.x, gv.x, mv.x, vv.x, a); adam_one(pv.y, gv.y, mv.y, vv.y, a);
                adam_one(pv.z, gv.z, mv.z, vv.z, a); adam_one(pv.w, gv.w, mv.w, vv.w, a);
                *reinterpret_cast<float4*>(s1 + i) = vv;
            } else {
                sgd_one(pv.x, gv.x, mv.x, a); sgd_one(pv.y, gv.y, mv.y, a);
                sgd_one(pv.z, gv.z, mv.z, a); sgd_one(pv.w, gv.w, mv.w, a);
            }
            *reinterpret_cast<float4*>(p + i) = pv;
            if (s0) *reinterpret_cast<float4*>(s0 + i) = mv;
        }
        const int tail0 = cnt & ~3;
        const int i = tail0 + threadIdx.x;
        if (i < cnt) {
            float pv = p[i], mv = s0 ? s0[i] : 0.f;
            if constexpr (ADAM) { float vv = s1[i]; adam_one(pv, g[i], mv, vv, a); s1[i] = vv; }
            else sgd_one(pv, g[i], mv, a);
            p[i] = pv;
            if (s0) s0[i] = mv;
        }
    } else {
        for (int i = threadIdx.x; i < cnt; i += 256) {
            float pv = p[i], mv = s0 ? s0[i] : 0.f;
            if constexpr (ADAM) { float vv = s1[i]; adam_one(pv, g[i], mv, vv, a); s1[i] = vv; }
            else sgd_one(pv, g[i], mv, a);
            p[i] = pv;
            if (s0) s0[i] = mv;
        }
    }
}

constexpr int PT = 32;
template <typename T, int U>
__device__ __forceinline__ void pack_stage(const umi_pack_desc& d, T* tl, int k0, int n0, bool k_inner) {
    const int TT = d.T;
    for (int e0 = threadIdx.x; e0 < PT * PT * TT; e0 += 256 * U) {
        float v[U];
        int li[U];
        bool ok[U];
#pragma unroll
        for (int u = 0; u < U; ++u) {
            const int e = e0 + 256 * u;
            const int o_ = e / (PT * TT), r = e - o_ * (PT * TT);
            const int i_ = r / TT, t = r - i_ * TT;
            const int kl = k_inner ? i_ : o_, nl = k_inner ? o_ : i_;
            const int k = k0 + kl, n = n0 + nl;
            ok[u] = e < PT * PT * TT && k < d.K && n < d.N;
            li[u] = e < PT * PT * TT ? (t * PT + kl) * (PT + 2) + nl : -1;
            const int tc = t < TT ? t : TT - 1, kc = k < d.K ? k : d.K - 1, nc = n < d.N ? n : d.N - 1;
            v[u] = d.src[(long)(d.flip_t ? TT - 1 - tc : tc) * d.st + (long)kc * d.sk + (long)nc * d.sn];
        }
#pragma unroll
        for (int u = 0; u < U; ++u) asm volatile("" : "+v"(v[u]));
#pragma unroll
        for (int u = 0; u < U; ++u) v[u] = ok[u] ? v[u] : 0.f;
#pragma unroll
        for (int u = 0; u < U; ++u)
            if (li[u] >= 0) tl[li[u]] = (T)v[u];
    }
}

template <typename T>
__device__ void pack_tiles_k8(const umi_pack_desc& d, int my_blk, int n_blk) {
    __shared__ T tl[9 * PT * (PT + 2)];
    const int nkt = (d.Kpad + PT - 1) / PT, nnt = (d.Npad + PT - 1) / PT;
    const int kb8 = d.Kpad >> 3, ldn = d.ldn ? d.ldn : d.Npad, TT = d.T;
    const bool k_inner = d.sk <= d.sn;
    T* dst = (T*)d.dst;
    for (int tile = my_blk; tile < nkt * nnt; tile += n_blk) {
        const int k0 = (tile % nkt) * PT, n0 = (tile / nkt) * PT;
        if (TT == 9) pack_stage<T, 12>(d, tl, k0, n0, k_inner);
        else pack_stage<T, 4>(d, tl, k0, n0, k_inner);
        __syncthreads();
        for (int e = threadIdx.x; e < TT * (PT / 8) * PT; e += 256) {
            const int nl = e % PT, r = e / PT, kg = r % (PT / 8), t = r / (PT / 8);
            const int k = k0 + kg * 8, n = n0 + nl;
            if (k >= d.Kpad || n >= d.Npad) continue;
            T pk[8];
#pragma unroll
            for (int j = 0; j < 8; ++j) pk[j] = tl[(t * PT + kg * 8 + j) * (PT + 2) + nl];
            T* o = dst + (((long)t * kb8 + (k >> 3)) * ldn + n) * 8;
            typedef T vec8 __attribute__((ext_vector_type(8)));
            vec8 pv;
#pragma unroll
            for (int j = 0; j < 8; ++j) pv[j] = pk[j];
            *reinterpret_cast<vec8*>(o) = pv;
        }
        __syncthreads();
    }
}

template <typename T>
__global__ __launch_bounds__(256) void pack_multi_kernel(const umi_pack_desc* __restrict__ descs, int n_desc) {
    const int blk = blockIdx.x;
    const umi_pack_desc d = descs[find_desc(descs, n_desc, blk)];
    const long total = (long)d.T * d.Kpad * d.Npad;
    if (d.k8 && d.T <= 9 && sizeof(T) == 2) {
        pack_tiles_k8<T>(d, blk - d.blk0, (int)((total + PACK_BLOCK - 1) / PACK_BLOCK));
        return;
    }
    const long base = (long)(blk - d.blk0) * PACK_BLOCK;
    T* dst = (T*)d.dst;
    const int kb8 = d.Kpad >> 3;
    const int ldn = d.ldn ? d.ldn : d.Npad;
#pragma unroll 2
    for (int j = 0; j < PACK_BLOCK / 256; ++j) {
        const long i = base + j * 256 + threadIdx.x;
        if (i >= total) break;
        int n, k, t;
        long o;
        if (d.k8) {
            const int k8 = (int)(i & 7);
            long r = i >> 3;
            n = (int)(r % d.Npad); r /= d.Npad;
            const int kb = (int)(r % kb8);
            t = (int)(r / kb8);
            k = kb * 8 + k8;
            o = (((long)t * kb8 + kb) * ldn + n) * 8 + k8;
        } else {
            n = (int)(i % d.Npad);
            const long r = i / d.Npad;
            k = (int)(r % d.Kpad);
            t = (int)(r / d.Kpad);
            o = ((long)t * d.Kpad + k) * ldn + n;
        }
        float v = 0.f;
        if (k < d.K && n < d.N) {
            const int ts = d.flip_t ? (d.T - 1 - t) : t;
            v = d.src[ts * d.st + k * d.sk + n * d.sn];
        }
        dst[o] = (T)v;
    }
}

}

__global__ __launch_bounds__(256) void table_upload_kernel(const uint4* __restrict__ src, uint4* __restrict__ dst, int n16) {
    for (int i = blockIdx.x * 256 + threadIdx.x; i < n16; i += gridDim.x * 256) dst[i] = src[i];
}
extern "C" int umi_table_upload(const void* host_pinned, void* dev, size_t nbytes, umi_stream_t stream) {
    if (!host_pinned || !dev || nbytes == 0 || (nbytes & 15) || (((uintptr_t)host_pinned | (uintptr_t)dev) & 15)) return UMI_ERR_BADARG;
    const int n16 = (int)(nbytes / 16);
    int grid = (n16 + 255) / 256;
    if (grid > 64) grid = 64;
    hipLaunchKernelGGL(table_upload_kernel, dim3(grid), dim3(256), 0, (hipStream_t)stream, (const uint4*)host_pinned, (uint4*)dev, n16);
    UMI_LAUNCH_CHECK();
    return UMI_OK;
}

extern "C" int umi_optim_block_elems(void) { return OPT_BLOCK; }
extern "C" int umi_pack_block_elems(void) { return PACK_BLOCK; }

extern "C" int umi_optim_sgd_multi(const void* descs, int n_desc, int total_blocks, double lr, double momentum,
                                   double dampening, double weight_decay, int nesterov, int first_step,
                                   umi_stream_t stream) {
    if (!descs || n_desc <= 0 || total_blocks <= 0) return UMI_ERR_BADARG;
    SgdArgs a{(float)lr, (float)momentum, (float)(1.0 - dampening), (float)weight_decay, nesterov, first_step, nullptr};
    hipLaunchKernelGGL((optim_multi_kernel<false, SgdArgs>), dim3(total_blocks), dim3(256), 0, (hipStream_t)stream,
                       (const umi_optim_desc*)descs, n_desc, a);
    UMI_LAUNCH_CHECK();
    return UMI_OK;
}

extern "C" int umi_optim_adam_multi(const void* descs, int n_desc, int total_blocks, double step_size, double beta1,
                                    double beta2, double bc2_sqrt, double eps, double weight_decay, umi_stream_t stream) {
    if (!descs || n_desc <= 0 || total_blocks <= 0) return UMI_ERR_BADARG;
    AdamArgs a{(float)step_size, (float)(1.0 - beta1), (float)beta2, (float)(1.0 - beta2), (float)bc2_sqrt, (float)eps,
               (float)weight_decay, nullptr};
    hipLaunchKernelGGL((optim_multi_kernel<true, AdamArgs>), dim3(total_blocks), dim3(256), 0, (hipStream_t)stream,
                       (const umi_optim_desc*)descs, n_desc, a);
    UMI_LAUNCH_CHECK();
    return UMI_OK;
}

__global__ void hyper_pre_kernel(Hyper* h, int adam) {
    if (adam) {
        const double t = h->adam_t + 1.0;
        h->adam_t = t;
        const double bc1 = 1.0 - pow(h->beta1, t), bc2 = 1.0 - pow(h->beta2, t);
        h->step_size_f = (float)(h->lr / bc1);
        h->bc2_sqrt_f = (float)sqrt(bc2);
    }
    h->lr_f = (float)h->lr;
}
__global__ void hyper_poly_kernel(Hyper* h) {
    h->lr = h->base_lr * pow(1.0 - h->iter / h->max_iter, h->power);
    h->iter += 1.0;
}

extern "C" size_t umi_optim_hyper_bytes(void) { return sizeof(Hyper); }

extern "C" int umi_optim_hyper_pre(void* hyper, int adam, umi_stream_t stream) {
    if (!hyper || ((uintptr_t)hyper & 7)) return UMI_ERR_BADARG;
    hipLaunchKernelGGL(hyper_pre_kernel, dim3(1), dim3(1), 0, (hipStream_t)stream, (Hyper*)hyper, adam);
    UMI_LAUNCH_CHECK();
    return UMI_OK;
}

extern "C" int umi_optim_hyper_poly(void* hyper, umi_stream_t stream) {
    if (!hyper || ((uintptr_t)hyper & 7)) return UMI_ERR_BADARG;
    hipLaunchKernelGGL(hyper_poly_kernel, dim3(1), dim3(1), 0, (hipStream_t)stream, (Hyper*)hyper);
    UMI_LAUNCH_CHECK();
    return UMI_OK;
}

extern "C" int umi_optim_sgd_multi_dev(const void* descs, int n_desc, int total_blocks, const void* hyper, double momentum,
                                       double dampening, double weight_decay, int nesterov, int first_step,
                                       umi_stream_t stream) {
    if (!descs || !hyper || n_desc <= 0 || total_blocks <= 0) return UMI_ERR_BADARG;
    SgdArgs a{0.f, (float)momentum, (float)(1.0 - dampening), (float)weight_decay, nesterov, first_step, (const Hyper*)hyper};
    hipLaunchKernelGGL((optim_multi_kernel<false, SgdArgs>), dim3(total_blocks), dim3(256), 0, (hipStream_t)stream,
                       (const umi_optim_desc*)descs, n_desc, a);
    UMI_LAUNCH_CHECK();
    return UMI_OK;
}

extern "C" int umi_optim_adam_multi_dev(const void* descs, int n_desc, int total_blocks, const void* hyper, double beta1,
                                        double beta2, double eps, double weight_decay, umi_stream_t stream) {
    if (!descs || !hyper || n_desc <= 0 || total_blocks <= 0) return UMI_ERR_BADARG;
    AdamArgs a{0.f, (float)(1.0 - beta1), (float)beta2, (float)(1.0 - beta2), 1.f, (float)eps, (float)weight_decay,
               (const Hyper*)hyper};
    hipLaunchKernelGGL((optim_multi_kernel<true, AdamArgs>), dim3(total_blocks), dim3(256), 0, (hipStream_t)stream,
                       (const umi_optim_desc*)descs, n_desc, a);
    UMI_LAUNCH_CHECK();
    return UMI_OK;
}

extern "C" int umi_pack_kn_multi(const void* descs, int n_desc, int total_blocks, int dtype, umi_stream_t stream) {
    if (!descs || n_desc <= 0 || total_blocks <= 0) return UMI_ERR_BADARG;
    if (dtype == UMI_F16)
        hipLaunchKernelGGL((pack_multi_kernel<half_t>), dim3(total_blocks), dim3(256), 0, (hipStream_t)stream,
                           (const umi_pack_desc*)descs, n_desc);
    else if (dtype == UMI_F32)
        hipLaunchKernelGGL((pack_multi_kernel<float>), dim3(total_blocks), dim3(256), 0, (hipStream_t)stream,
                           (const umi_pack_desc*)descs, n_desc);
    else return UMI_ERR_BADARG;
    UMI_LAUNCH_CHECK();
    return UMI_OK;
}
```

unet-torch_amd/umi/graph.py:

```python
import math
import os

import torch

from . import lib as L
from . import ops
from .deferred import Deferred


def _fuse_bnred():
    return os.environ.get("UMI_NO_BNRED_FUSION") != "1"


def _defer_wgrad_reduce():
    return os.environ.get("UMI_NO_WGRAD_REDUCE_GROUP") != "1"


def _fuse_bnapply(Ci):
    mode = os.environ.get("UMI_BNAPPLY_FUSION", "")
    return mode != "0" and (Ci <= int(os.environ.get("UMI_BNAPPLY_MAXCI", "64")) or mode == "all")


class Act:
    __slots__ = ("raw", "tx", "grad", "parts", "needs_grad", "bn_rstd", "bn_part", "bn_part_at", "gives")

    def __init__(self, raw, tx=None, parts=None, needs_grad=True):
        self.raw, self.tx, self.grad, self.parts, self.needs_grad = raw, tx, None, parts, needs_grad
        self.bn_rstd = None
        self.bn_part = None
        self.gives = 0
        self.bn_part_at = -1

    @property
    def shape(self):
        return tuple(self.raw.shape)

    def full_tx(self):
        return self.tx


class Tape:
    def __init__(self, dtype, training, record, loss_scale=1.0, grad_sink=None, pack_cache=None, seed=0, seed_dev=None):
        self.dtype = dtype
        self._seed = int(seed)
        self._seed_dev = seed_dev
        self._drop_count = 0
        self.pack_cache = pack_cache
        self.grad_sink = grad_sink
        self.training = training
        self.record = record
        self.loss_scale = float(loss_scale)
        self.inv = (grad_sink.grad_scale if grad_sink is not None else 1.0) / self.loss_scale
        self.steps = []
        self.param_grads = {}
        self._deferred_unscale = []
        self._nbt = []
        d = self.deferred = Deferred(self)
        d.register("wgrad_reduce", lambda _, items, tape: ops.wgrad_reduce_flush(items),
                   on=lambda tape: (tape.grad_sink is None or tape.deferred.marks) and _defer_wgrad_reduce())
        d.register("zero", lambda _, items, tape: torch._foreach_zero_(items),
                   on=lambda tape: tape.grad_sink is None)
        self._inputs = []
        self.conv3x3_flags = 0
        self.conv1x1_flags = 0

    def alloc(self, N, H, W, C, dtype=None, zero=False, device=None):
        f = torch.zeros if zero else torch.empty
        return f((N, H, W, C), dtype=dtype or self.dtype, device=device)

    def _pack(self, kind, weight, wf, k8):
        c = self.pack_cache
        if c is not None and isinstance(weight, torch.nn.Parameter) and weight.dtype == torch.float32:
            return c.get(kind, weight, self.dtype, k8)
        return ops.PACKERS[kind](wf, self.dtype, k8=k8)

    def _fk(self, R, S, stride, pad, cin, cout):
        if (R, S, stride, pad) == (3, 3, 1, 1):
            return self.conv3x3_flags if cin % 8 == 0 else 0
        if (R, S, stride, pad) == (1, 1, 1, 0):
            return self.conv1x1_flags if cin % 8 == 0 and cout % 8 == 0 else 0
        return 0

    def _packer(self, kind, weight, wf):
        return lambda lay: self._pack(kind, weight, wf, bool(lay))

    def _new_pgrad(self, p):
        v = self.grad_sink.buffer_for(p) if self.grad_sink is not None else None
        return v if v is not None else torch.empty_like(p, dtype=torch.float32)

    def _set_pgrad(self, p, g):
        key = id(p)
        if key in self.param_grads:
            dst = self.param_grads[key][1]
            if self.grad_sink is not None and self.grad_sink.buffer_for(p) is not None:
                raise NotImplementedError("a parameter used twice in one tape under a gradient sink (umi.ddp.GradReducer)")
            if self.deferred.pending(dst) or self.deferred.pending(g):
                self.deferred.park_add(dst, g)
            else:
                dst.add_(g)
            return
        v = self.grad_sink.buffer_for(p) if self.grad_sink is not None else None
        late = False
        if v is not None:
            late = self.deferred.pending(g)
            if v.data_ptr() != g.data_ptr():
                if late:
                    raise RuntimeError("deferred gradient fills must target the sink's bucket slot (Tape._new_pgrad)")
                v.copy_(g)
            g = v
        self.param_grads[key] = (p, g)
        if v is not None:
            if late:
                self.deferred.park_ready(p)
            else:
                self.grad_sink.mark_ready(p)

    def _set_pgrad_scaled(self, p, g, scale):
        v = self.grad_sink.buffer_for(p) if self.grad_sink is not None else None
        if v is not None and id(p) not in self.param_grads and v.shape == g.shape:
            torch.mul(g, scale, out=v)
            self._set_pgrad(p, v)
        else:
            self._set_pgrad(p, g * scale)

    def _give(self, act: Act, g):
        if act.parts is not None:
            for part, c0, c1 in act.parts:
                self._give(part, g[..., c0:c1])
            return
        if not act.needs_grad:
            return
        act.gives += 1
        if act.grad is None:
            act.grad = g
        else:
            act.grad.add_(g)

    def _accumulate_target(self, act: Act, src, R, S, stride, pad):
        if (act.parts is not None or not act.needs_grad or act.grad is None or act.grad.dtype != torch.float16
                or os.environ.get("UMI_NO_DGRAD_ACCUMULATE") == "1"):
            return None
        return act.grad if ops.conv_accumulate_ok(src, act.grad, R, S, stride, pad) else None

    def finish_forward(self):
        if self._nbt:
            torch._foreach_add_(self._nbt, 1)
            self._nbt = []

    def input_nchw(self, x: torch.Tensor, needs_grad=False):
        if not x.is_cuda:
            raise RuntimeError("unet-torch_amd: the HIP path needs the input on device 'cuda' (MI355X); "
                               "no CPU fallback exists in the product path")
        N, C, H, W = x.shape
        raw = torch.empty((N, H, W, C), dtype=self.dtype, device=x.device)
        if C == 1 and x.is_contiguous():
            raw.view(-1).copy_(x.view(-1))
        else:
            raw.copy_(x.permute(0, 2, 3, 1))
        a = Act(raw, None, needs_grad=needs_grad)
        self._inputs.append(a)
        return a

    def input_nhwc(self, raw, tx=None, needs_grad=False):
        a = Act(raw, tx, needs_grad=needs_grad)
        self._inputs.append(a)
        return a

    def conv_bn(self, a: Act, weight, bn, out=None, stride=1, pad=1, input_exclusive=False, relu=True, bias=None):
        Co, Ci, R, S = weight.shape
        N, H, W, Ca = a.shape
        assert Ca == Ci, f"conv expects {Ci} input channels, got {Ca}"
        Ho, Wo = (H + 2 * pad - R) // stride + 1, (W + 2 * pad - S) // stride + 1
        if out is None:
            out = self.alloc(N, Ho, Wo, Co, device=a.raw.device)
        wf = weight.detach().float()
        if (not self.training and not self.record and _eval_fold() and self.dtype == torch.float16 and (R, S, stride, pad) == (3, 3, 1, 1)
                and ops.conv_plan(a.raw, out, 3, 3, 1, 1)[0] == 1):
            tx, _ = ops.eval_bn_tx(bn.weight.detach(), bn.bias.detach(), bn.running_mean, bn.running_var, bn.eps)
            if bias is not None:
                tx[:, 2] += tx[:, 1] * bias.detach().float()
            if not relu:
                tx[:, 3] = ops.NEG_INF
            if ops.conv3x3_fwd_act(a.raw, a.tx, self._pack("conv_fwd", weight, wf, True), tx, out):
                return Act(out, None)
        part, flags, two_pass = None, self._fk(R, S, stride, pad, Ci, Co), False
        if self.training and (R, S) == (1, 1) and not (flags and self.dtype == torch.float32):
            two_pass = (self.dtype == torch.float16 and Co % 8 == 0 and
                        ops.conv_plan(a.raw, out, R, S, stride, pad, 0, False)[0] == 1)
            narrow = self.dtype == torch.float16 and Co <= 8
            flags = 0 if (two_pass or narrow) else L.CONV_FORCE_GENERIC
        res = ops.conv_fwd(a.raw, a.tx, self._packer("conv_fwd", weight, wf), None, out,
                           R, S, stride, pad, want_stats=self.training and not two_pass, flags=flags)
        part = ops.bn_stats(out) if two_pass else res
        if self.training and part is None:
            raise RuntimeError("conv_bn: no BatchNorm statistics were produced for this layer")
        if self.training:
            mom = bn.momentum if bn.momentum is not None else 0.1
            tx, rstd = ops.bn_finalize(part, Co, N * Ho * Wo, bn.weight.detach(), bn.bias.detach(), bn.eps, mom,
                                       bn.running_mean if bn.track_running_stats else None,
                                       bn.running_var if bn.track_running_stats else None)
            if bn.track_running_stats and bn.num_batches_tracked is not None:
                self._nbt.append(bn.num_batches_tracked)
            if bias is not None and bn.track_running_stats:
                bn.running_mean.add_(bias.detach().float(), alpha=mom)
        else:
            tx, rstd = ops.eval_bn_tx(bn.weight.detach(), bn.bias.detach(), bn.running_mean, bn.running_var, bn.eps)
            if bias is not None:
                tx[:, 2] += tx[:, 1] * bias.detach().float()
        if not relu:
            tx[:, 3] = ops.NEG_INF
        o = Act(out, tx)
        o.bn_rstd = rstd
        if self.record:
            def bwd():
                if o.grad is None:
                    return
                if not self.training:
                    raise RuntimeError("backward through BatchNorm in eval mode is not supported by the HIP path")
                inv = self.inv
                partials = o.bn_part if o.bn_part_at == o.gives else None
                fuse = (_fuse_bnapply(Ci) and self.dtype == torch.float16 and (R, S, stride, pad) == (3, 3, 1, 1)
                        and Ci % 8 == 0 and Co % 8 == 0)
                stem_fuse = (not fuse and self.dtype == torch.float16 and (R, S, stride, pad) == (3, 3, 1, 1) and Ci <= 4
                             and Co % 8 == 0 and not _wants_grad(a) and os.environ.get("UMI_NO_STEM_BNAPPLY") != "1")
                dbeta, dgamma = ops.bn_bwd(o.grad, out, tx, rstd, partials=partials, apply=not (fuse or stem_fuse))
                o.bn_part = None
                if self.grad_sink is None and inv != 1.0:
                    self._deferred_unscale += [dgamma, dbeta]
                    self._set_pgrad(bn.weight, dgamma)
                    self._set_pgrad(bn.bias, dbeta)
                else:
                    self._set_pgrad_scaled(bn.weight, dgamma, inv)
                    self._set_pgrad_scaled(bn.bias, dbeta, inv)
                gw = self._new_pgrad(weight)
                if fuse:
                    dz = self.alloc(N, Ho, Wo, Co, device=out.device)
                    if ops.conv_wgrad_bnapply(a.raw, a.tx, o.grad, out, tx, rstd, dbeta, dgamma, dz, gw, Ci * R * S, R * S, 1,
                                              inv, R, S, stride, pad):
                        o.grad = dz
                    else:
                        fuse = False
                        ops.bn_bwd_apply(o.grad, out, tx, rstd, dbeta, dgamma)
                if stem_fuse:
                    if not ops.conv_wgrad_bnapply(a.raw, a.tx, o.grad, out, tx, rstd, dbeta, dgamma, None, gw, Ci * R * S, R * S, 1,
                                                  inv, R, S, stride, pad):
                        stem_fuse = False
                        ops.bn_bwd_apply(o.grad, out, tx, rstd, dbeta, dgamma)
                if not fuse and not stem_fuse:
                    ops.conv_wgrad(a.raw, a.tx, o.grad, None, gw, Ci * R * S, R * S, 1, inv, R, S, stride, pad,
                                   flags=self._fk(R, S, stride, pad, Ci, Co), defer=self.deferred.open("wgrad_reduce", fills=(gw,)))
                self._set_pgrad(weight, gw)
                if bias is not None:
                    gb = self._new_pgrad(bias)
                    if not self.deferred.defer("zero", None, gb, fills=(gb,)):
                        gb.zero_()
                    self._set_pgrad(bias, gb)
                if _wants_grad(a):
                    if stride != 1:
                        raise NotImplementedError("dgrad for strided conv_bn")
                    tgt = self._accumulate_target(a, o.grad, R, S, 1, R - 1 - pad)
                    if tgt is not None:
                        ops.conv_fwd(o.grad, None, self._packer("conv_dgrad", weight, wf), None, tgt,
                                     R, S, 1, R - 1 - pad, flags=L.CONV_ACCUMULATE)
                        a.gives += 1
                        return
                    dx = self.alloc(N, H, W, Ci, device=out.device)
                    part = None
                    if (input_exclusive and _fuse_bnred() and a.grad is None and a.parts is None and a.bn_rstd is not None
                            and a.tx is not None and (R, S, pad) == (3, 3, 1) and self.dtype == torch.float16):
                        part = ops.conv_dgrad_bnred(o.grad, self._pack("conv_dgrad", weight, wf, True), dx, a.raw, a.tx,
                                                    a.bn_rstd)
                    if part is not None:
                        a.bn_part, a.bn_part_at = part, a.gives + 1
                    else:
                        ops.conv_fwd(o.grad, None, self._packer("conv_dgrad", weight, wf), None, dx,
                                     R, S, 1, R - 1 - pad, flags=self._fk(R, S, stride, R - 1 - pad, Co, Ci))
                    self._give(a, dx)
            self.steps.append(bwd)
        return o

    def conv_bias(self, a: Act, weight, bias, out_dtype=None, pad=0):
        Co, Ci, R, S = weight.shape
        N, H, W, Ca = a.shape
        assert Ca == Ci
        out = self.alloc(N, H + 2 * pad - R + 1, W + 2 * pad - S + 1, Co, dtype=out_dtype or self.dtype,
                         device=a.raw.device)
        wf0 = weight.detach().float()
        ops.conv_fwd(a.raw, a.tx, self._packer("conv_fwd", weight, wf0),
                     bias.detach().float() if bias is not None else None, out, R, S, 1, pad, flags=self._fk(R, S, 1, pad, Ci, Co))
        o = Act(out, None)
        if self.record:
            def bwd():
                if o.grad is None:
                    return
                inv = self.inv
                g = o.grad
                gw = self._new_pgrad(weight)
                dx, part, fused_w = None, None, False
                if (_wants_grad(a) and (R, S, pad) == (1, 1, 0) and _fuse_bnred() and os.environ.get("UMI_NO_HEAD_BNRED") != "1"
                        and a.grad is None and a.parts is None and a.bn_rstd is not None and a.tx is not None
                        and self.dtype == torch.float16 and g.dtype == torch.float16):
                    dx = self.alloc(N, H, W, Ci, device=out.device)
                    wf = weight.detach().float()
                    want_w = os.environ.get("UMI_NO_HEAD_WGRAD_FUSION") != "1"
                    part = ops.head_dgrad_bnred(g, self._pack("conv_dgrad", weight, wf, False), dx, a.raw, a.tx, a.bn_rstd,
                                                dW=gw if want_w else None, out_scale=inv)
                    fused_w = part is not None and want_w
                if not fused_w:
                    ops.conv_wgrad(a.raw, a.tx, g, None, gw, Ci * R * S, R * S, 1, inv, R, S, 1, pad,
                                   flags=self._fk(R, S, 1, pad, Ci, Co), defer=self.deferred.open("wgrad_reduce", fills=(gw,)))
                self._set_pgrad(weight, gw)
                if bias is not None:
                    gb = self._new_pgrad(bias)
                    ops.colsum(g, gb, inv)
                    self._set_pgrad(bias, gb)
                if _wants_grad(a):
                    if dx is None:
                        dx = self.alloc(N, H, W, Ci, device=out.device)
                    if part is not None:
                        a.bn_part, a.bn_part_at = part, a.gives + 1
                    else:
                        wf = weight.detach().float()
                        ops.conv_fwd(g, None, self._packer("conv_dgrad", weight, wf), None, dx,
                                     R, S, 1, R - 1 - pad, flags=self._fk(R, S, 1, R - 1 - pad, Co, Ci))
                    self._give(a, dx)
            self.steps.append(bwd)
        return o

    def pool2(self, a: Act):
        N, H, W, C = a.shape
        out = self.alloc(N, H // 2, W // 2, C, device=a.raw.device)
        ops.pool2_fwd(a.raw, a.tx, out)
        o = Act(out, None)
        if self.record:
            def bwd():
                if o.grad is None or not _wants_grad(a):
                    return
                if a.parts is not None:
                    raise NotImplementedError("pool2 backward into a concat input")
                acc = a.grad is not None
                if not acc:
                    a.grad = self.alloc(N, H, W, C, device=out.device)
                part = None
                if (a.bn_rstd is not None and a.tx is not None and self.dtype == torch.float16 and _fuse_bnred()
                        and os.environ.get("UMI_NO_POOLRED_FUSION") != "1"):
                    part = ops.pool2_bwd_bnred(o.grad, a.raw, a.tx, a.bn_rstd, a.grad, acc)
                if part is None:
                    ops.pool2_bwd(o.grad, a.raw, a.tx, a.grad, acc)
                a.gives += 1
                a.bn_part, a.bn_part_at = part, a.gives
            self.steps.append(bwd)
        return o

    def conv_transpose2x2(self, a: Act, weight, bias, dest, out_hw=None, bias_cancelled=False):
        Cin, Cout = weight.shape[:2]
        N, h, w, Ca = a.shape
        assert Ca == Cin
        _, Hd, Wd, Cd = dest.shape
        assert Cd == Cout
        dY, dX = Hd - 2 * h, Wd - 2 * w
        if dY < 0 or dX < 0:
            raise NotImplementedError("skip smaller than the upsampled map (negative F.pad) is not supported")
        oy, ox = dY // 2, dX // 2
        if dY or dX:
            dest.zero_()
        wf = weight.detach().float()
        ops.conv_fwd(a.raw, a.tx, self._packer("convT_fwd", weight, wf),
                     bias.detach().float() if bias is not None else None, dest, 2, 2, 2, 0,
                     flags=L.CONV_UPSAMPLE2, up_offset=(oy, ox))
        o = Act(dest, None)
        if self.record:
            def bwd():
                if o.grad is None:
                    return
                inv = self.inv
                g = o.grad
                if dY or dX:
                    g = g[:, oy:oy + 2 * h, ox:ox + 2 * w, :].contiguous()
                gw = self._new_pgrad(weight)
                dlist = self.deferred.open("wgrad_reduce", fills=(gw,))
                fused = False
                if bias is not None:
                    gb = self._new_pgrad(bias)
                    if bias_cancelled and self.training and not (dY or dX):
                        gb.zero_()
                    elif os.environ.get("UMI_NO_CONVT_BIAS_FUSION") != "1" and ops.convT_wgrad_bias(g, a.raw, a.tx, gw, gb, inv,
                                                                                                    defer=dlist):
                        fused = True
                    else:
                        ops.colsum(g, gb, inv)
                    self._set_pgrad(bias, gb)
                if not fused:
                    ops.conv_wgrad(g, None, a.raw, a.tx, gw, Cout * 4, 4, 1, inv, 2, 2, 2, 0, defer=dlist)
                self._set_pgrad(weight, gw)
                if _wants_grad(a):
                    tgt = self._accumulate_target(a, g, 2, 2, 2, 0)
                    if tgt is not None:
                        ops.conv_fwd(g, None, self._packer("convT_dgrad", weight, wf), None, tgt, 2, 2, 2, 0, flags=L.CONV_ACCUMULATE)
                        a.gives += 1
                        return
                    dx = self.alloc(N, h, w, Cin, device=dest.device)
                    part = None
                    if (_fuse_bnred() and os.environ.get("UMI_NO_CONVT_BNRED") != "1" and a.grad is None and a.parts is None
                            and a.bn_rstd is not None and a.tx is not None and self.dtype == torch.float16 and g.dtype == torch.float16):
                        part = ops.conv_gather_bnred(g, self._pack("convT_dgrad", weight, wf, True), dx, a.raw, a.tx, a.bn_rstd,
                                                     2, 2, 2, 0)
                    if part is not None:
                        a.bn_part, a.bn_part_at = part, a.gives + 1
                    else:
                        ops.conv_fwd(g, None, self._packer("convT_dgrad", weight, wf), None, dx, 2, 2, 2, 0)
                    self._give(a, dx)
            self.steps.append(bwd)
        return o

    def dropout(self, a: Act, p):
        if not self.training or p <= 0.0:
            return a
        from . import ops_tu
        N, H, W, C = a.shape
        out = self.alloc(N, H, W, C, device=a.raw.device)
        mask = torch.empty(N * H * W * C, dtype=torch.uint8, device=a.raw.device)
        self._drop_count += 1
        ops_tu.dropout(a.raw, out, mask, False, p, (self._seed * 7919 + self._drop_count) & 0x7FFFFFFF, a.tx,
                       seed_dev=self._seed_dev)
        o = Act(out, None)
        if self.record:
            def bwd():
                if o.grad is None or not _wants_grad(a):
                    return
                dx = self.alloc(N, H, W, C, device=out.device)
                ops_tu.dropout(o.grad, dx, mask, True, p, 0)
                self._give(a, dx)
            self.steps.append(bwd)
        return o

    def copy_into(self, a: Act, dest):
        assert a.parts is None and tuple(dest.shape) == a.shape
        dest.copy_(a.raw)
        o = Act(dest, a.tx, needs_grad=a.needs_grad)
        if self.record:
            def bwd():
                if o.grad is not None and _wants_grad(a):
                    self._give(a, o.grad)
            self.steps.append(bwd)
        return o

    def add_relu(self, a: Act, b: Act):
        N, H, W, C = a.shape
        assert b.shape == a.shape
        out = self.alloc(N, H, W, C, device=a.raw.device)
        ops.add2_relu(a.raw, a.tx, b.raw, b.tx, out)
        o = Act(out, None)
        if self.record:
            def bwd():
                if o.grad is None:
                    return
                da = self.alloc(N, H, W, C, device=out.device)
                db = self.alloc(N, H, W, C, device=out.device)
                ops.add2_relu_bwd(o.grad, out, da, db)
                self._give(a, da)
                self._give(b, db)
            self.steps.append(bwd)
        return o

    def gate(self, x: Act, p: Act, dest):
        N, H, W, C = x.shape
        assert p.shape == (N, H, W, 1) and tuple(dest.shape) == x.shape
        ops.gate(x.raw, x.tx, p.raw, p.tx, dest)
        o = Act(dest, None)
        if self.record:
            def bwd():
                if o.grad is None:
                    return
                dx = self.alloc(N, H, W, C, device=dest.device)
                dp = self.alloc(N, H, W, 1, device=dest.device)
                ops.gate_bwd(o.grad, x.raw, x.tx, p.raw, p.tx, dx, dp)
                self._give(x, dx)
                self._give(p, dp)
            self.steps.append(bwd)
        return o

    def concat(self, buf, acts):
        txs, parts, c0 = [], [], 0
        for a in acts:
            C = a.shape[3]
            assert a.raw.data_ptr() == buf[..., c0:c0 + C].data_ptr(), "concat part is not a slice of the buffer"
            txs.append(a.tx if a.tx is not None else ops.passthrough_tx_const(C, buf.device))
            parts.append((a, c0, c0 + C))
            c0 += C
        assert c0 == buf.shape[3]
        if all(a.tx is None for a in acts):
            return Act(buf, None, parts=parts)
        return Act(buf, torch.cat(txs, 0).contiguous(), parts=parts)

    def output_nchw_plain(self, a: Act):
        assert a.tx is None
        return a.raw.permute(0, 3, 1, 2).contiguous().float()

    def seed_grad_nchw(self, a: Act, g_nchw: torch.Tensor):
        N, C, H, W = g_nchw.shape
        g = g_nchw.permute(0, 2, 3, 1)
        if self.loss_scale != 1.0:
            g = g * self.loss_scale
        a.grad = torch.empty((N, H, W, C), dtype=self.dtype, device=g_nchw.device)
        a.grad.copy_(g)

    def backward(self):
        for step in reversed(self.steps):
            step()
        self.steps = []
        self.deferred.flush()
        if self._deferred_unscale:
            torch._foreach_mul_(self._deferred_unscale, self.inv)
            self._deferred_unscale = []
        if self.grad_sink is not None:
            self.grad_sink.finish()

    def input_grad_nchw(self, a: Act):
        if a.grad is None:
            return None
        g = a.grad.permute(0, 3, 1, 2).float()
        if self.loss_scale != 1.0:
            g = g / self.loss_scale
        return g.contiguous()


def _eval_fold():
    return os.environ.get("UMI_NO_EVAL_FOLD") != "1"


def dropout_seeds(module, device, training):
    if not training or device.type != "cuda":
        return 0, None
    if getattr(module, "_drop_base", None) is None:
        module._drop_base = int(torch.randint(0, 2 ** 31 - 1, (1,)).item())
    ctr = getattr(module, "_drop_step", None)
    if ctr is None or ctr.device != device:
        if torch.cuda.is_current_stream_capturing():
            raise RuntimeError("first training forward inside a HIP-graph capture; run one eager step first")
        ctr = module._drop_step = torch.zeros(1, dtype=torch.int32, device=device)
    ctr.add_(1)
    return module._drop_base, ctr


def pack_cache_of(module):
    if os.environ.get("UMI_NO_PACK_CACHE") == "1":
        return None
    c = module.__dict__.get("_umi_pack_cache")
# ... 17 lines not shown
```

unet-torch_amd/umi/ops.py:

```python

import numpy as np
import torch

from . import lib as L

NEG_INF = float("-inf")


def _dt(t: torch.Tensor) -> int:
    if t.dtype == torch.float32:
        return L.UMI_F32
    if t.dtype == torch.float16:
        return L.UMI_F16
    raise TypeError(f"libunetmi supports float32/float16 storage, got {t.dtype}")


def torch_dtype(code: int):
    return torch.float32 if code == L.UMI_F32 else torch.float16


def _stream():
    return torch.cuda.current_stream().cuda_stream


def _need_cuda(*ts):
    for t in ts:
        if t is not None and not t.is_cuda:
            raise RuntimeError("libunetmi ops need tensors on the MI355X (device 'cuda'); "
                               "there is no CPU fallback in the product path")


def _nhwc(t: torch.Tensor):
    if t.dim() != 4 or (t.stride(3) != 1 and t.shape[3] != 1):
        raise ValueError(f"expected NHWC view with contiguous channels, got {tuple(t.shape)} / {t.stride()}")
    N, H, W, C = t.shape
    ld = t.stride(2) if W > 1 else (t.stride(1) if H > 1 else (t.stride(0) // max(H * W, 1) if N > 1 else C))
    ok = ld >= C and (H == 1 or t.stride(1) == W * ld) and (N == 1 or t.stride(0) == H * W * ld)
    if not ok:
        raise ValueError(f"NHWC view must be dense in N,H,W with one pixel stride: {tuple(t.shape)} / {t.stride()}")
    return N, H, W, C, ld


def _ptr(t):
    return None if t is None else t.data_ptr()


def passthrough_tx(C, device):
    t = torch.zeros(C, 4, dtype=torch.float32, device=device)
    t[:, 1] = 1.0
    t[:, 3] = NEG_INF
    return t


_passthrough = {}


def passthrough_tx_const(C, device):
    key = (C, str(device))
    t = _passthrough.get(key)
    if t is None and torch.cuda.is_current_stream_capturing():
        return passthrough_tx(C, device)
    if t is None:
        t = _passthrough[key] = passthrough_tx(C, device)
    return t


def eval_bn_tx(weight, bias, running_mean, running_var, eps):
    rstd = torch.rsqrt(running_var.float() + eps)
    scale = weight.float() * rstd
    return torch.stack([running_mean.float(), scale, bias.float() - running_mean.float() * scale,
                        torch.zeros_like(rstd)], dim=1).contiguous(), rstd


def pack_kn(src: torch.Tensor, T, K, N, st, sk, sn, flip_t, dtype, Kpad=None, Npad=None, k8=False):
    _need_cuda(src)
    assert src.dtype == torch.float32 and src.is_contiguous()
    Kpad, Npad = Kpad or K, Npad or N
    out = torch.empty(T * Kpad * Npad, dtype=dtype, device=src.device)
    L.call("umi_pack_kn8" if k8 else "umi_pack_kn",
           src.data_ptr(), out.data_ptr(), T, K, N, st, sk, sn, int(flip_t), Kpad, Npad, _dt(out), _stream())
    return out


def pack_conv_fwd(w: torch.Tensor, dtype, k8=False):
    Co, Ci, R, S = w.shape
    return pack_kn(w, R * S, Ci, Co, 1, R * S, Ci * R * S, False, dtype, k8=k8)


def pack_conv_dgrad(w: torch.Tensor, dtype, k8=False):
    Co, Ci, R, S = w.shape
    return pack_kn(w, R * S, Co, Ci, 1, Ci * R * S, R * S, True, dtype, k8=k8)


def pack_convT_fwd(w: torch.Tensor, dtype, k8=False):
    Cin, Cout = w.shape[:2]
    return pack_kn(w, 4, Cin, Cout, 1, Cout * 4, 4, False, dtype, k8=k8)


def pack_convT_dgrad(w: torch.Tensor, dtype, k8=False):
    Cin, Cout = w.shape[:2]
    return pack_kn(w, 4, Cout, Cin, 1, 4, Cout * 4, False, dtype, k8=k8)


def _pack_args(kind, shape):
    if len(shape) == 2:
        shape = (shape[0], shape[1], 1, 1)
    if kind == "conv_fwd":
        Co, Ci, R, S = shape
        return R * S, Ci, Co, 1, R * S, Ci * R * S, 0
    if kind == "conv_dgrad":
        Co, Ci, R, S = shape
        return R * S, Co, Ci, 1, Ci * R * S, R * S, 1
    if kind == "conv_dgrad_strided":
        Co, Ci, R, S = shape
        return R * S, Co, Ci, 1, Ci * R * S, R * S, 0
    if kind == "bias":
        return 1, 1, shape[0], 0, 0, 1, 0
    if kind == "convT_fwd":
        Cin, Cout = shape[:2]
        return 4, Cin, Cout, 1, Cout * 4, 4, 0
    if kind == "convT_dgrad":
        Cin, Cout = shape[:2]
        return 4, Cout, Cin, 1, 4, Cout * 4, 0
    raise KeyError(kind)


def pack_conv_dgrad_strided(w, dtype, k8=False):
    Co, Ci, R, S = w.shape
    return pack_kn(w, R * S, Co, Ci, 1, Ci * R * S, R * S, False, dtype, k8=k8)


PACKERS = {"conv_fwd": pack_conv_fwd, "conv_dgrad": pack_conv_dgrad, "convT_fwd": pack_convT_fwd,
           "convT_dgrad": pack_convT_dgrad, "conv_dgrad_strided": pack_conv_dgrad_strided}


class PackCache:

    class _Ent:
        __slots__ = ("w", "args", "dst", "ver", "k8", "ptr", "ldn")

    class _Wstd:
        __slots__ = ("w", "ws", "rstd", "eps", "ver", "off")

    def __init__(self):
        self.ents = {}
        self.cats = {}
        self.wstds = {}
        self.wstd_total = 0
        self._tables = {}

    _CAP = 1 << 18

    def _buffers(self):
        if getattr(self, "_dev", None) is None:
            if torch.cuda.is_current_stream_capturing():
                raise RuntimeError("PackCache: first use inside a HIP-graph capture; run one eager forward first")
            self._dev = torch.empty(self._CAP, dtype=torch.uint8, device="cuda")
            self._host = torch.empty(self._CAP, dtype=torch.uint8).pin_memory()
            self._used = 0
        return self._host, self._dev

    def _upload(self, arr):
        raw = np.ascontiguousarray(arr).view(np.uint8).reshape(-1)
        nbytes = (raw.size + 15) // 16 * 16
        host, dev = self._buffers()
        if self._used + nbytes > self._CAP:
            if torch.cuda.is_current_stream_capturing():
                raise RuntimeError("PackCache: descriptor-table space exhausted during a HIP-graph capture")
            torch.cuda.current_stream().synchronize()
            self._tables.clear()
            self._used = 0
        off = self._used
        host.numpy()[off:off + raw.size] = raw
        L.call("umi_table_upload", host.data_ptr() + off, dev.data_ptr() + off, nbytes, _stream())
        self._used = off + nbytes
        return dev.data_ptr() + off

    def __deepcopy__(self, memo):
        return PackCache()

    def __reduce__(self):
        return (PackCache, ())

    @staticmethod
    def _ver(w):
        return (w._version, w.data_ptr())

    def _new_ent(self, kind, w, k8, dst, ptr, ldn):
        import weakref
        e = PackCache._Ent()
        e.w, e.args, e.k8, e.ver = weakref.ref(w), _pack_args(kind, w.shape), bool(k8), None
        e.dst, e.ptr, e.ldn = dst, ptr, ldn
        if not torch.cuda.is_current_stream_capturing():
            self._buffers()
        return e

    def get(self, kind, w, dtype, k8):
        key = (id(w), kind, dtype, bool(k8))
        e = self.ents.get(key)
        if e is not None and e.w() is not w:
            e = None
        if e is None:
            T, K, N = _pack_args(kind, w.shape)[:3]
            dst = torch.empty(T * K * N, dtype=dtype, device=w.device)
            e = self.ents[key] = self._new_ent(kind, w, k8, dst, dst.data_ptr(), 0)
        ver = self._ver(w)
        if e.ver != ver:
            T, K, N, st, sk, sn, flip = e.args
            L.call("umi_pack_kn8" if e.k8 else "umi_pack_kn",
                   w.data_ptr(), e.dst.data_ptr(), T, K, N, st, sk, sn, flip, K, N, _dt(e.dst), _stream())
            e.ver = ver
        return e.dst

    def get_cat(self, kind, ws, dtype, k8):
        key = (tuple(id(w) for w in ws), kind, dtype, bool(k8))
        c = self.cats.get(key)
        if c is not None and any(e.w() is not w for e, w in zip(c[1], ws)):
            c = None
        if c is None:
            args = [_pack_args(kind, w.shape) for w in ws]
            assert all(a[0] == 1 for a in args), "get_cat packs single-tap (1x1 / Linear) weights"
            esz = torch.empty(0, dtype=dtype).element_size()
            if kind == "conv_dgrad":
                assert len({a[2] for a in args}) == 1 and (not k8 or all(a[1] % 8 == 0 for a in args))
                offs, tot, ldn = [], 0, 0
                for a in args:
                    offs.append(tot)
                    tot += a[1] * a[2]
            else:
                assert len({a[1] for a in args}) == 1
                ntot = sum(a[2] for a in args)
                offs, n0 = [], 0
                for a in args:
                    offs.append(n0 * (8 if k8 else 1))
                    n0 += a[2]
                tot, ldn = args[0][1] * ntot, ntot
            dst = torch.empty(tot, dtype=dtype, device=ws[0].device)
            ents = []
            for w, off in zip(ws, offs):
                e = self._new_ent(kind, w, k8, dst, dst.data_ptr() + off * esz, ldn)
                self.ents[(id(w), kind + "@cat", dtype, bool(k8), id(dst))] = e
                ents.append(e)
            c = self.cats[key] = (dst, ents)
        stale = [(None, e, w) for e, w in zip(c[1], ws) if e.ver != self._ver(w)]
        if stale:
            self._repack(stale)
        return c[0]

    def wstd(self, w, eps):
        import weakref
        e = self.wstds.get(id(w))
        if e is not None and e.w() is not w:
            e = None
        ver = self._ver(w)
        if e is None:
            assert w.dtype == torch.float32 and w.is_contiguous()
            e = self.wstds[id(w)] = PackCache._Wstd()
            e.w, e.eps, e.ver, e.off = weakref.ref(w), float(eps), None, self.wstd_total
            e.ws = torch.empty(w.shape, dtype=torch.float32, device=w.device)
            e.rstd = torch.empty(w.shape[0], dtype=torch.float32, device=w.device)
            self.wstd_total += (w.numel() + 63) // 64 * 64
        if e.ver != ver:
            L.call("umi_wstd_fwd", w.data_ptr(), e.ws.data_ptr(), e.rstd.data_ptr(), w.shape[0], w[0].numel(), e.eps,
                   _stream())
            torch.autograd.graph.increment_version(e.ws)
            e.ver = ver
        return e

    def _wstd_table(self, ents, dws=None):
        tkey = ("wstd",) + tuple((id(e), e.w().data_ptr()) for e in ents) + (tuple(t.data_ptr() for t in dws) if dws else ())
        tab = self._tables.get(tkey)
        if tab is None:
            arr = np.zeros(len(ents), dtype=_WSTD_DESC)
            b0 = 0
            for i, e in enumerate(ents):
                w = e.w()
                arr[i] = (w.data_ptr(), e.ws.data_ptr(), e.rstd.data_ptr(), e.off, w.shape[0], w[0].numel(), e.eps, b0,
                          dws[i].data_ptr() if dws else 0)
                b0 += w.shape[0]
            tab = self._tables[tkey] = (self._upload(arr), b0, len(ents))
        return tab

    def wstd_bwd(self, ents, g_flat, dw_flat, dws=None):
        dev_ptr, rows, n = self._wstd_table(ents, dws)
        L.call("umi_wstd_bwd_multi", dev_ptr, n, rows, g_flat.data_ptr(), dw_flat.data_ptr() if dw_flat is not None else None,
               _stream())

    def _repack(self, items):
        by_dtype = {}
        for it in items:
            by_dtype.setdefault(it[1].dst.dtype, []).append(it)
        blk = None
        for dtype, its in by_dtype.items():
            tkey = tuple((id(e), w.data_ptr()) for _, e, w in its)
            tab = self._tables.get(tkey)
            if tab is None:
                blk = blk or L.fn("umi_pack_block_elems")()
                arr = np.zeros(len(its), dtype=_PACK_DESC)
                b0 = 0
                for i, (_, e, w) in enumerate(its):
                    T, K, N, st, sk, sn, flip = e.args
                    arr[i] = (w.data_ptr(), e.ptr, st, sk, sn, T, K, N, flip, K, N, int(e.k8), b0, e.ldn, 0)
                    b0 += (T * K * N + blk - 1) // blk
                tab = self._tables[tkey] = (self._upload(arr), b0, len(its))
            dev_ptr, total, n = tab
            L.call("umi_pack_kn_multi", dev_ptr, n, total, L.UMI_F32 if dtype == torch.float32 else L.UMI_F16,
                   _stream())
            for _, e, w in its:
                e.ver = self._ver(w)

    def refresh(self):
        force = torch.cuda.is_available() and torch.cuda.is_current_stream_capturing()
        wst = []
        for key, e in list(self.wstds.items()):
            w = e.w()
            if w is None:
                del self.wstds[key]
            elif force or e.ver != self._ver(w):
                wst.append(e)
        if wst:
            dev_ptr, rows, n = self._wstd_table(wst)
            L.call("umi_wstd_fwd_multi", dev_ptr, n, rows, _stream())
            torch.autograd.graph.increment_version([e.ws for e in wst])
            for e in wst:
                e.ver = self._ver(e.w())
        stale = []
        for key, e in list(self.ents.items()):
            w = e.w()
            if w is None:
                del self.ents[key]
                continue
            if force or e.ver != self._ver(w):
                stale.append((key, e, w))
        if stale:
            self._repack(stale)


_PACK_DESC, OPTIM_DESC, _WSTD_DESC = (np.dtype(L.STRUCTS[n]) for n in ("umi_pack_desc", "umi_optim_desc", "umi_wstd_desc"))


def conv_plan(x, y, R, S, stride, pad, flags=0, has_bias=False):
    import ctypes
    N, H, W, Ci, ldx = _nhwc(x)
    _, _, _, Co, ldy = _nhwc(y)
    lay, rows = ctypes.c_int(0), ctypes.c_int(0)
    L.call("umi_conv_fwd_plan", N, H, W, Ci, Co, R, S, stride, pad, ldx, ldy, _dt(x), _dt(y), flags,
           int(has_bias), ctypes.addressof(lay), ctypes.addressof(rows))
    return lay.value, rows.value


def conv_accumulate_ok(x, y, R, S, stride, pad, flags=0):
    N, H, W, Ci, ldx = _nhwc(x)
    _, _, _, Co, ldy = _nhwc(y)
    if (x.data_ptr() | y.data_ptr()) & 15:
        return False
    return L.fn("umi_conv_fwd_plan")(N, H, W, Ci, Co, R, S, stride, pad, ldx, ldy, _dt(x), _dt(y),
                                     flags | L.CONV_ACCUMULATE, 0, None, None) == L.UMI_OK


def conv_fwd(x, tx, wp, bias, y, R, S, stride, pad, want_stats=False, flags=0, up_offset=(0, 0)):
    _need_cuda(x, y)
    N, H, W, Ci, ldx = _nhwc(x)
    N2, oH, oW, Co, ldy = _nhwc(y)
    assert N2 == N
    if flags & L.CONV_UPSAMPLE2:
        Ho, Wo = H, W
    else:
        Ho, Wo = (H + 2 * pad - R) // stride + 1, (W + 2 * pad - S) // stride + 1
        assert (oH, oW) == (Ho, Wo), f"output view {oH}x{oW} != conv output {Ho}x{Wo}"
    part = None
    layout, rows = conv_plan(x, y, R, S, stride, pad, flags, bias is not None)
    if callable(wp):
        wp = wp(layout)
    elif layout != 0:
        raise ValueError("this conv takes the MFMA path: pass a callable so the weights get the k8 packing")
    if want_stats:
        part = torch.empty(rows * 2 * Co, dtype=torch.float32, device=x.device)
    if tx is not None:
        assert tx.shape == (Ci, 4) and tx.dtype == torch.float32 and tx.is_contiguous()
    L.call("umi_conv_fwd", x.data_ptr(), ldx, _ptr(tx), wp.data_ptr(), _ptr(bias), y.data_ptr(), ldy,
           _ptr(part), N, H, W, Ci, Co, R, S, stride, pad, Ho, Wo,
           up_offset[0], up_offset[1], oH, oW, _dt(x), _dt(y), flags, _stream())
    return part


def conv3x3_fwd_act(x, tx, wp8, out_tx, y):
    N, H, W, Ci, ldx = _nhwc(x)
    _, _, _, Co, ldy = _nhwc(y)
    return L.supported("umi_conv3x3_fwd_act", x.data_ptr(), ldx, _ptr(tx), wp8.data_ptr(), out_tx.data_ptr(), y.data_ptr(), ldy,
                       N, H, W, Ci, Co, _dt(x), _stream())


def bn_finalize(part, C, count, gamma, beta, eps, momentum, running_mean, running_var):
    rows = part.numel() // (2 * C)
    tx = torch.empty(C, 4, dtype=torch.float32, device=part.device)
    rstd = torch.empty(C, dtype=torch.float32, device=part.device)
    L.call("umi_bn_finalize", part.data_ptr(), rows, C, float(count), _ptr(gamma), _ptr(beta), eps, momentum,
           _ptr(running_mean), _ptr(running_var), tx.data_ptr(), rstd.data_ptr(),
           _stream())
    return tx, rstd


def pool2_fwd(x, tx, y):
    N, H, W, C, ldx = _nhwc(x)
    _, Ho, Wo, _, ldy = _nhwc(y)
    assert (Ho, Wo) == (H // 2, W // 2)
    L.call("umi_pool2_fwd", x.data_ptr(), ldx, _ptr(tx), y.data_ptr(), ldy, N, H, W, C, _dt(x), _stream())


def pool2_bwd(dpool, x, tx, da, accumulate):
    N, H, W, C, ldx = _nhwc(x)
    _, _, _, _, lddp = _nhwc(dpool)
    _, _, _, _, ldda = _nhwc(da)
    L.call("umi_pool2_bwd", dpool.data_ptr(), lddp, x.data_ptr(), ldx, _ptr(tx), da.data_ptr(), ldda,
           int(accumulate), N, H, W, C, _dt(x), _stream())


def bn_stats(y):
    N, H, W, C, ldy = _nhwc(y)
    M = N * H * W
    rows = L.fn("umi_bn_stats_rows")(M, C) if y.dtype == torch.float16 else 0
    if rows <= 0:
        return None
    part = torch.empty(rows * 2 * C, dtype=torch.float32, device=y.device)
    if not L.supported("umi_bn_stats", y.data_ptr(), ldy, part.data_ptr(), M, C, _dt(y), _stream()):
        return None
    return part


def pool2_bwd_bnred(dpool, x, tx, rstd, da, accumulate):
    N, H, W, C, ldx = _nhwc(x)
    rows = L.fn("umi_pool2_bwd_bnred_stat_rows")(N, H, W, C)
    if rows <= 0 or x.dtype != torch.float16 or tx is None or rstd is None:
        return None
    part = torch.empty(rows * 2 * C, dtype=torch.float32, device=x.device)
    if not L.supported("umi_pool2_bwd_bnred", dpool.data_ptr(), _nhwc(dpool)[4], x.data_ptr(), ldx, tx.data_ptr(),
                       rstd.data_ptr(), da.data_ptr(), _nhwc(da)[4], int(accumulate), part.data_ptr(), N, H, W, C, _dt(x),
                       _stream()):
        return None
    return part


_ws_cache = {}
_ws_high = {}
_ws_pinned = []


def workspace(nbytes, device):
    key = (device, torch.cuda.current_stream().cuda_stream)
    buf = _ws_cache.get(key)
    need = max(int(nbytes), _ws_high.get(device, 1 << 20))
    _ws_high[device] = need
    if buf is None or buf.numel() < nbytes:
        if buf is not None and torch.cuda.is_current_stream_capturing():
            _ws_pinned.append(buf)
        buf = torch.empty(need, dtype=torch.uint8, device=device)
        _ws_cache[key] = buf
    return buf


def conv_dgrad_bnred(dy, wp8, da, ybn, txbn, rstd):
    N, H, W, Ci, lddy = _nhwc(dy)
    _, _, _, Co, ldda = _nhwc(da)
    ldybn = _nhwc(ybn)[4]
    lay, rows = conv_plan(dy, da, 3, 3, 1, 1)
    if lay != 1:
        return None
    part = torch.empty(rows * 2 * Co, dtype=torch.float32, device=dy.device)
    if not L.supported("umi_conv_dgrad_bnred", dy.data_ptr(), lddy, wp8.data_ptr(), da.data_ptr(), ldda, ybn.data_ptr(), ldybn,
                       txbn.data_ptr(), rstd.data_ptr(), part.data_ptr(), N, H, W, Ci, Co, _dt(dy), _stream()):
        return None
    return part


def conv_gather_bnred(x, wp8, y, ybn, txbn, rstd, R, S, stride, pad, flags=0):
    N, H, W, Ci, ldx = _nhwc(x)
    _, Ho, Wo, Co, ldy = _nhwc(y)
    ldybn = _nhwc(ybn)[4]
    if x.dtype != torch.float16 or y.dtype != torch.float16 or ybn.dtype != torch.float16:
        return None
    if (x.data_ptr() | y.data_ptr() | ybn.data_ptr()) & 15:
        return None
    rows = L.fn("umi_conv_gather_bnred_rows")(N, H, W, Ci, Co, R, S, stride, pad, Ho, Wo, ldx, ldy, _dt(x), flags)
    if rows <= 0:
        return None
    part = torch.empty(rows * 2 * Co, dtype=torch.float32, device=x.device)
    if not L.supported("umi_conv_gather_bnred", x.data_ptr(), ldx, wp8.data_ptr(), y.data_ptr(), ldy, ybn.data_ptr(), ldybn,
                       txbn.data_ptr(), rstd.data_ptr(), part.data_ptr(), N, H, W, Ci, Co, R, S, stride, pad,
                       Ho, Wo, _dt(x), flags, _stream()):
        return None
    return part


def head_dgrad_bnred(dl, wp, da, ybn, txbn, rstd, dW=None, out_scale=1.0):
    N, H, W, Ci, lddl = _nhwc(dl)
    _, _, _, Co, ldda = _nhwc(da)
    ldybn = _nhwc(ybn)[4]
    P = N * H * W
    if dl.dtype != torch.float16 or da.dtype != torch.float16 or ybn.dtype != torch.float16:
        return None
    rows = L.fn("umi_head_dgrad_bnred_rows")(P, Ci, Co, ldda, _dt(dl))
    if rows <= 0:
        return None
    part = torch.empty(rows * 2 * Co, dtype=torch.float32, device=dl.device)
    if dW is not None:
        assert dW.dtype == torch.float32 and dW.is_contiguous() and dW.numel() == Ci * Co
        ws = workspace(L.fn("umi_head_bwd_fused_ws_bytes")(P, Ci, Co), dl.device)
        if not L.supported("umi_head_bwd_fused", dl.data_ptr(), lddl, wp.data_ptr(), da.data_ptr(), ldda, ybn.data_ptr(), ldybn,
                           txbn.data_ptr(), rstd.data_ptr(), part.data_ptr(), dW.data_ptr(), Co, 1, out_scale,
                           ws.data_ptr(), ws.numel(), P, Ci, Co, _dt(dl), _stream()):
            return None
        return part
    if not L.supported("umi_head_dgrad_bnred", dl.data_ptr(), lddl, wp.data_ptr(), da.data_ptr(), ldda, ybn.data_ptr(), ldybn,
                       txbn.data_ptr(), rstd.data_ptr(), part.data_ptr(), P, Ci, Co, _dt(dl), _stream()):
        return None
    return part


def bn_bwd(da, y, tx, rstd, partials=None, apply=True):
    N, H, W, C, ldy = _nhwc(y)
    _, _, _, _, ldda = _nhwc(da)
    M = N * H * W
    nb = L.fn("umi_bn_bwd_ws_bytes")(M, C)
    ws = workspace(nb, y.device)
    sums = torch.empty(2, C, dtype=torch.float32, device=y.device)
    if partials is not None:
        L.call("umi_bn_bwd_from_partials", partials.data_ptr(), partials.numel() // (2 * C), C, sums[0].data_ptr(),
               sums[1].data_ptr(), _stream())
    else:
        L.call("umi_bn_bwd_reduce", da.data_ptr(), ldda, y.data_ptr(), ldy, tx.data_ptr(), rstd.data_ptr(),
               sums[0].data_ptr(), sums[1].data_ptr(), M, C, _dt(y), ws.data_ptr(),
               ws.numel(), _stream())
    if apply:
        bn_bwd_apply(da, y, tx, rstd, sums[0], sums[1])
    return sums[0], sums[1]


def bn_bwd_apply(da, y, tx, rstd, sum_dz, sum_dzx):
    N, H, W, C, ldy = _nhwc(y)
    L.call("umi_bn_bwd_apply", da.data_ptr(), _nhwc(da)[4], y.data_ptr(), ldy, tx.data_ptr(), rstd.data_ptr(),
           sum_dz.data_ptr(), sum_dzx.data_ptr(), N * H * W, C, _dt(y), _stream())


def conv_wgrad_bnapply(x, txa, da, y, tx_bn, rstd, sum_dz, sum_dzx, dz, dW, s_co, s_ci, s_t, out_scale, R, S, stride, pad):
    N, H, W, Ci, ldx = _nhwc(x)
    _, Ho, Wo, Co, ldda = _nhwc(da)
    if (Ho, Wo) != (H, W) or da.dtype != torch.float16:
        return False
    assert dW.dtype == torch.float32 and dW.is_contiguous() and (dz is None or dz.shape == da.shape)
    nb = L.fn("umi_conv_wgrad_ws_bytes")(N, Ho, Wo, Ci, Co, R, S, _dt(x), 0)
    ws = workspace(nb, x.device)
    return L.supported("umi_conv_wgrad_bnapply", x.data_ptr(), ldx, _ptr(txa), da.data_ptr(), ldda, y.data_ptr(), _nhwc(y)[4],
                       tx_bn.data_ptr(), rstd.data_ptr(), sum_dz.data_ptr(), sum_dzx.data_ptr(),
                       _ptr(dz), _nhwc(dz)[4] if dz is not None else 0, dW.data_ptr(), s_co, s_ci, s_t, out_scale,
                       N, H, W, Ci, Co, R, S, stride, pad, _dt(x), 0, ws.data_ptr(), ws.numel(), _stream())


_WgPending = L.STRUCTS["umi_wgrad_pending"]


def conv_wgrad(x, txa, dy, txb, dW, s_co, s_ci, s_t, out_scale, R, S, stride, pad, flags=0, defer=None):
    import ctypes
    N, H, W, Ci, ldx = _nhwc(x)
    _, Ho, Wo, Co, lddy = _nhwc(dy)
    assert dW.dtype == torch.float32 and dW.is_contiguous()
    nb = L.fn("umi_conv_wgrad_ws_bytes")(N, Ho, Wo, Ci, Co, R, S, _dt(x), flags)
    if defer is None:
        ws = workspace(nb, x.device)
        L.call("umi_conv_wgrad", x.data_ptr(), ldx, _ptr(txa), dy.data_ptr(), lddy, _ptr(txb), dW.data_ptr(),
               s_co, s_ci, s_t, out_scale, N, H, W, Ci, Co, R, S, stride, pad, Ho, Wo,
               _dt(x), flags, ws.data_ptr(), ws.numel(), _stream())
        return
    ws = torch.empty(max(nb, 16), dtype=torch.uint8, device=x.device)
    pend = _WgPending()
    L.call("umi_conv_wgrad_deferred", x.data_ptr(), ldx, _ptr(txa), dy.data_ptr(), lddy, _ptr(txb), dW.data_ptr(),
           s_co, s_ci, s_t, out_scale, N, H, W, Ci, Co, R, S, stride, pad, Ho, Wo,
           _dt(x), flags, ws.data_ptr(), ws.numel(), ctypes.addressof(pend), _stream())
    if pend.part:
        defer.append((pend, ws, dW))


def convT_wgrad_bias(g, y, txy, dW, dbias, out_scale, defer=None):
    import ctypes
    N, H, W, Ci, ldx = _nhwc(g)
    _, Ho, Wo, Co, lddy = _nhwc(y)
    if g.dtype != torch.float16 or (H, W) != (2 * Ho, 2 * Wo):
        return False
    assert dW.dtype == torch.float32 and dW.is_contiguous() and dbias.dtype == torch.float32 and dbias.numel() == Ci
    nb = L.fn("umi_conv_wgrad_ws_bytes")(N, Ho, Wo, Ci, Co, 2, 2, _dt(g), 0)
    ws = torch.empty(max(nb, 16), dtype=torch.uint8, device=g.device) if defer is not None else workspace(nb, g.device)
    pend = _WgPending()
    assert dW.numel() == Ci * Co * 4
    if not L.supported("umi_conv_wgrad_bias", g.data_ptr(), ldx, y.data_ptr(), lddy, _ptr(txy), dW.data_ptr(), Ci * 4, 4, 1,
                       dbias.data_ptr(), out_scale, N, H, W, Ci, Co, Ho, Wo, _dt(g), 0, ws.data_ptr(), ws.numel(),
                       ctypes.addressof(pend) if defer is not None else None, _stream()):
        return False
    if defer is not None and pend.part:
        defer.append((pend, ws, dW))
    return True


def wgrad_pending(part, dW, s_co, s_ci, s_t, scale, splits, RS, Ci, Co):
    addr = [p.data_ptr() if torch.is_tensor(p) else p for p in (part, dW)]
    return _WgPending(addr[0], addr[1], s_co, s_ci, s_t, scale, splits, RS, Ci, Co)


def wgrad_reduce_group(pending, check=True):
    import ctypes
    arr = (_WgPending * max(len(pending), 1))(*pending)
    st = L.fn("umi_wgrad_reduce_group")(len(pending), ctypes.addressof(arr), _stream())
    if check:
        L.check(st, "umi_wgrad_reduce_group")
    return st


def wgrad_reduce_flush(defer):
    if defer:
        wgrad_reduce_group([d[0] for d in defer])
        del defer[:]


def conv_wgrad_group(xs, dys, dWs, s_co, s_ci, out_scale):
    import ctypes
    n = len(xs)
    N, H, W, Ci, ldx = _nhwc(xs[0])
    _, _, _, Co, lddy = _nhwc(dys[0])
    for x, dy, dW in zip(xs, dys, dWs):
        assert _nhwc(x) == (N, H, W, Ci, ldx) and _nhwc(dy) == (N, H, W, Co, lddy) and x.dtype == xs[0].dtype
        assert dW.dtype == torch.float32
    arr = ctypes.c_void_p * n
    ptrs = [arr(*[t.data_ptr() for t in ts]) for ts in (xs, dys, dWs)]
    return L.supported("umi_conv_wgrad_group", n, ctypes.cast(ptrs[0], ctypes.c_void_p), ldx,
                       ctypes.cast(ptrs[1], ctypes.c_void_p), lddy, ctypes.cast(ptrs[2], ctypes.c_void_p), s_co, s_ci, out_scale,
                       N * H * W, Ci, Co, _dt(xs[0]), _stream())


def colsum(x, out, out_scale):
    N, H, W, C, ldx = _nhwc(x)
    M = N * H * W
    ws = workspace(L.fn("umi_colsum_ws_bytes")(M, C), x.device)
    L.call("umi_colsum", x.data_ptr(), ldx, out.data_ptr(), out_scale, M, C, _dt(x), ws.data_ptr(),
           ws.numel(), _stream())


def colsum_group(xs, outs, out_scale):
    import ctypes
    n = len(xs)
    N, H, W, C, ldx = _nhwc(xs[0])
    M = N * H * W
    if xs[0].dtype != torch.float16 or C % 8 or ldx % 8:
        return False
    for x, o in zip(xs, outs):
        assert _nhwc(x) == (N, H, W, C, ldx) and o.dtype == torch.float32 and o.numel() == C
    ws = workspace(min(n, 16) * L.fn("umi_colsum_ws_bytes")(M, C), xs[0].device)
    arr = ctypes.c_void_p * n
    px, po = arr(*[t.data_ptr() for t in xs]), arr(*[t.data_ptr() for t in outs])
    return L.supported("umi_colsum_group", n, ctypes.cast(px, ctypes.c_void_p), ldx, ctypes.cast(po, ctypes.c_void_p), out_scale,
                       M, C, _dt(xs[0]), ws.data_ptr(), ws.numel(), _stream())


def add2_relu(a, txa, b, txb, y):
    N, H, W, C, lda = _nhwc(a)
    _, _, _, _, ldb = _nhwc(b)
    _, _, _, _, ldy = _nhwc(y)
    assert a.shape == b.shape == y.shape
    L.call("umi_add2_relu_fwd", a.data_ptr(), lda, _ptr(txa), b.data_ptr(), ldb, _ptr(txb), y.data_ptr(), ldy,
           N * H * W, C, _dt(a), _stream())


def add2_relu_bwd(dy, y, da, db):
    N, H, W, C, lddy = _nhwc(dy)
    L.call("umi_add2_relu_bwd", dy.data_ptr(), lddy, y.data_ptr(), _nhwc(y)[4], da.data_ptr(), _nhwc(da)[4],
           db.data_ptr(), _nhwc(db)[4], N * H * W, C, _dt(dy), _stream())


def gate(x, txx, p, txp, y):
    N, H, W, C, ldx = _nhwc(x)
    assert tuple(p.shape) == (N, H, W, 1) and p.is_contiguous() and y.shape == x.shape
    L.call("umi_gate_fwd", x.data_ptr(), ldx, _ptr(txx), p.data_ptr(), _ptr(txp), y.data_ptr(), _nhwc(y)[4],
           N * H * W, C, _dt(x), _stream())


def gate_bwd(dy, x, txx, p, txp, dx, dp):
    N, H, W, C, ldx = _nhwc(x)
    assert dp.is_contiguous() and tuple(dp.shape) == (N, H, W, 1)
    L.call("umi_gate_bwd", dy.data_ptr(), _nhwc(dy)[4], x.data_ptr(), ldx, _ptr(txx), p.data_ptr(), _ptr(txp),
           dx.data_ptr(), _nhwc(dx)[4], dp.data_ptr(), N * H * W, C, _dt(x), _stream())


def materialize_nchw(x, tx):
    N, H, W, C, ldx = _nhwc(x)
    y = torch.empty(N, C, H, W, dtype=torch.float32, device=x.device)
    L.call("umi_materialize_nchw", x.data_ptr(), ldx, _ptr(tx), y.data_ptr(), N, H, W, C, _dt(x), _stream())
    return y
```

Measured before the change: 761.5.

## Defer BN-fused wgrad reductions, restructure split-K reduce kernels, pair weight pack jobs

Lets the BN-apply-fused weight-gradient path defer its split-K reduction into the grouped wgrad reduce queue instead of reducing inline. The split-K reduction kernels are rewritten with unrolled multi-load lane sums and a tile-based few/many-split scheme. A new paired k8 weight-pack kernel packs matching (e.g. flipped/transposed) views of the same weight in one launch. The aim is fewer kernel launches and more memory-level parallelism in the reductions, at the cost of extra per-call workspace allocations and more complex code paths.

Result: no change. 761.3 (-0.0%).

```diff
diff --git a/include/unetmi.h b/include/unetmi.h
--- a/include/unetmi.h
+++ b/include/unetmi.h
@@ -116,6 +116,11 @@
                            int lddz, float* dW, long s_co, long s_ci, long s_t, float out_scale, int N, int H, int W,
                            int Ci, int Co, int R, int S, int stride, int pad, int dtype, int flags, void* ws,
                            size_t ws_bytes, umi_stream_t stream);
+int umi_conv_wgrad_bnapply_deferred(const void* x, int ldx, const void* txa, const void* da, int ldda, const void* y, int ldy,
+                                    const void* tx_bn, const float* rstd, const float* sum_dz, const float* sum_dzx, void* dz,
+                                    int lddz, float* dW, long s_co, long s_ci, long s_t, float out_scale, int N, int H, int W,
+                                    int Ci, int Co, int R, int S, int stride, int pad, int dtype, int flags, void* ws,
+                                    size_t ws_bytes, umi_wgrad_pending* out, umi_stream_t stream);
 
 size_t umi_colsum_ws_bytes(long M, int C);
 int umi_colsum(const void* x, int ldx, float* out, float out_scale, long M, int C, int dtype,
@@ -265,6 +270,7 @@
 } umi_pack_desc;
 int umi_pack_block_elems(void);
 int umi_pack_kn_multi(const void* descs, int n_desc, int total_blocks, int dtype, umi_stream_t stream);
+int umi_pack_kn8_pairs(const void* descs, int n_pairs, int total_blocks, int dtype, umi_stream_t stream);
 
 int umi_add2_relu_fwd(const void* a, int lda, const void* txa, const void* b, int ldb, const void* txb, void* y, int ldy,
                       long M, int C, int dtype, umi_stream_t stream);
diff --git a/unet-torch_amd/csrc/api.hip b/unet-torch_amd/csrc/api.hip
--- a/unet-torch_amd/csrc/api.hip
+++ b/unet-torch_amd/csrc/api.hip
@@ -276,17 +276,17 @@
     return umi_wgrad1x1_mfma_group(n, x, ldx, dy, lddy, dW, s_co, s_ci, out_scale, M, Ci, Co, (hipStream_t)stream);
 }
 
-extern "C" int umi_conv_wgrad_bnapply(const void* x, int ldx, const void* txa, const void* da, int ldda, const void* y, int ldy,
-                                      const void* tx_bn, const float* rstd, const float* sum_dz, const float* sum_dzx,
-                                      void* dz, int lddz, float* dW, long s_co, long s_ci, long s_t, float out_scale, int N,
-                                      int H, int W, int Ci, int Co, int R, int S, int stride, int pad, int dtype, int flags,
-                                      void* ws, size_t ws_bytes, umi_stream_t stream) {
+static int conv_wgrad_bnapply(const void* x, int ldx, const void* txa, const void* da, int ldda, const void* y, int ldy,
+                              const void* tx_bn, const float* rstd, const float* sum_dz, const float* sum_dzx,
+                              void* dz, int lddz, float* dW, long s_co, long s_ci, long s_t, float out_scale, int N,
+                              int H, int W, int Ci, int Co, int R, int S, int stride, int pad, int dtype, int flags,
+                              void* ws, size_t ws_bytes, umi_wgrad_pending* defer, umi_stream_t stream) {
     if (!x || !da || !y || !tx_bn || !rstd || !sum_dz || !sum_dzx || !dW || !ws || N <= 0 || H <= 0 || W <= 0 || Ci <= 0 ||
         Co <= 0 || ldx < Ci || ldda < Co || ldy < Co || (dz && (lddz < Co || dz == da || dz == y)))
         return UMI_ERR_BADARG;
     const WgradProblem p = wgrad_problem(N, H, W, Ci, Co, R, S, stride, pad, H, W, ldx, ldda, dtype, flags, txa != nullptr, false);
     const WgradPath path = umi_conv_wgrad_path(p);
-    const WgradOut o{dW, s_co, s_ci, s_t, out_scale, ws, ws_bytes, nullptr, nullptr};
+    const WgradOut o{dW, s_co, s_ci, s_t, out_scale, ws, ws_bytes, defer, nullptr};
     const WgradBnApply bna{y, ldy, tx_bn, rstd, sum_dz, sum_dzx, dz, lddz};
     if (!dz) {
         if (path != WGRAD_STEM || ldy % 8) return UMI_ERR_UNSUPPORTED;
@@ -296,3 +296,24 @@
         return UMI_ERR_UNSUPPORTED;
     return umi_wgrad3x3_mfma(p, x, txa, da, o, (hipStream_t)stream, &bna);
 }
+
+extern "C" int umi_conv_wgrad_bnapply(const void* x, int ldx, const void* txa, const void* da, int ldda, const void* y, int ldy,
+                                      const void* tx_bn, const float* rstd, const float* sum_dz, const float* sum_dzx,
+                                      void* dz, int lddz, float* dW, long s_co, long s_ci, long s_t, float out_scale, int N,
+                                      int H, int W, int Ci, int Co, int R, int S, int stride, int pad, int dtype, int flags,
+                                      void* ws, size_t ws_bytes, umi_stream_t stream) {
+    return conv_wgrad_bnapply(x, ldx, txa, da, ldda, y, ldy, tx_bn, rstd, sum_dz, sum_dzx, dz, lddz, dW, s_co, s_ci, s_t, out_scale,
+                              N, H, W, Ci, Co, R, S, stride, pad, dtype, flags, ws, ws_bytes, nullptr, stream);
+}
+
+extern "C" int umi_conv_wgrad_bnapply_deferred(const void* x, int ldx, const void* txa, const void* da, int ldda, const void* y,
+                                               int ldy, const void* tx_bn, const float* rstd, const float* sum_dz,
+                                               const float* sum_dzx, void* dz, int lddz, float* dW, long s_co, long s_ci,
+                                               long s_t, float out_scale, int N, int H, int W, int Ci, int Co, int R, int S,
+                                               int stride, int pad, int dtype, int flags, void* ws, size_t ws_bytes,
+                                               umi_wgrad_pending* out, umi_stream_t stream) {
+    if (!out) return UMI_ERR_BADARG;
+    out->part = nullptr;
+    return conv_wgrad_bnapply(x, ldx, txa, da, ldda, y, ldy, tx_bn, rstd, sum_dz, sum_dzx, dz, lddz, dW, s_co, s_ci, s_t, out_scale,
+                              N, H, W, Ci, Co, R, S, stride, pad, dtype, flags, ws, ws_bytes, out, stream);
+}
diff --git a/unet-torch_amd/csrc/generic_kernels.hip b/unet-torch_amd/csrc/generic_kernels.hip
--- a/unet-torch_amd/csrc/generic_kernels.hip
+++ b/unet-torch_amd/csrc/generic_kernels.hip
@@ -849,70 +849,116 @@
     }
 }
 
+__device__ __forceinline__ void wg_add4(float4& a, const float4 v) { a.x += v.x; a.y += v.y; a.z += v.z; a.w += v.w; }
+__device__ __forceinline__ void wg_pin4(float4& v) { asm volatile("" : "+v"(v.x), "+v"(v.y), "+v"(v.z), "+v"(v.w)); }
+
+template <int U>
+__device__ __forceinline__ float4 wg_lane_sum2(const float4* __restrict__ p, long stride, int z0, int splits) {
+    float4 a = make_float4(0.f, 0.f, 0.f, 0.f), b = a;
+    const int n = z0 < splits ? (splits - z0 + 7) >> 3 : 0;
+    int j = 0;
+    for (; j + U <= n; j += U) {
+        float4 v[U];
+#pragma unroll
+        for (int u = 0; u < U; ++u) v[u] = p[(long)(z0 + 8 * (j + u)) * stride];
+#pragma unroll
+        for (int u = 0; u < U; u += 2) { wg_add4(a, v[u]); wg_add4(b, v[u + 1]); }
+    }
+    if (j < n) {
+        float4 v[U];
+#pragma unroll
+        for (int u = 0; u < U; ++u) { const int jj = j + u < n ? j + u : n - 1; v[u] = p[(long)(z0 + 8 * jj) * stride]; }
+#pragma unroll
+        for (int u = 0; u < U; ++u) wg_pin4(v[u]);
+#pragma unroll
+        for (int u = 0; u < U; u += 2) {
+            if (j + u < n) wg_add4(a, v[u]);
+            if (j + u + 1 < n) wg_add4(b, v[u + 1]);
+        }
+    }
+    return make_float4(a.x + b.x, a.y + b.y, a.z + b.z, a.w + b.w);
+}
+
+template <int U>
+__device__ __forceinline__ float wg_lane_sum1(const float* __restrict__ p, long stride, int z0, int splits) {
+    float s = 0.f;
+    const int n = z0 < splits ? (splits - z0 + 7) >> 3 : 0;
+    int j = 0;
+    for (; j + U <= n; j += U) {
+        float v[U];
+#pragma unroll
+        for (int u = 0; u < U; ++u) v[u] = p[(long)(z0 + 8 * (j + u)) * stride];
+#pragma unroll
+        for (int u = 0; u < U; ++u) s += v[u];
+    }
+    if (j < n) {
+        float v[U];
+#pragma unroll
+        for (int u = 0; u < U; ++u) { const int jj = j + u < n ? j + u : n - 1; v[u] = p[(long)(z0 + 8 * jj) * stride]; }
+#pragma unroll
+        for (int u = 0; u < U; ++u) asm volatile("" : "+v"(v[u]));
+#pragma unroll
+        for (int u = 0; u < U; ++u)
+            if (j + u < n) s += v[u];
+    }
+    return s;
+}
+
+template <bool VEC>
+__device__ __forceinline__ void wg_reduce_elems(const umi_wgrad_pending& d, float4 (*red)[33], int my_blk, int n_blk) {
+    const int ox = threadIdx.x & 31, sl = threadIdx.x >> 5;
+    const long total = (long)d.RS * d.Ci * d.Co / (VEC ? 4 : 1);
+    const int CoW = d.Co / (VEC ? 4 : 1);
+    for (long base = (long)my_blk * 32; base < total; base += (long)n_blk * 32) {
+        const long i = base + ox;
+        float4 a = make_float4(0.f, 0.f, 0.f, 0.f);
+        if (i < total) {
+            if (VEC) {
+                const float4* p = reinterpret_cast<const float4*>(d.part) + i;
+                a = d.splits >= 512 ? wg_lane_sum2<16>(p, total, sl, d.splits) : wg_lane_sum2<8>(p, total, sl, d.splits);
+            } else {
+                a.x = wg_lane_sum1<8>(d.part + i, total, sl, d.splits);
+            }
+        }
+        red[sl][ox] = a;
+        __syncthreads();
+        const int o = VEC ? threadIdx.x >> 2 : threadIdx.x, k = VEC ? threadIdx.x & 3 : 0;
+        const long io = base + o;
+        if (threadIdx.x < (VEC ? 128 : 32) && io < total) {
+            const float* r = reinterpret_cast<const float*>(&red[0][0]) + o * 4 + k;
+            float t;
+            if (VEC) {
+                t = r[0];
+#pragma unroll
+                for (int l = 1; l < 8; ++l) t += r[l * 33 * 4];
+            } else {
+                t = 0.f;
+#pragma unroll
+                for (int l = 0; l < 8; ++l) t += r[l * 33 * 4];
+            }
+            const int co = (int)(io % CoW) * (VEC ? 4 : 1) + k;
+            const long rr = io / CoW;
+            const int ci = (int)(rr % d.Ci), tp = (int)(rr / d.Ci);
+            d.dW[co * d.s_co + ci * d.s_ci + tp * d.s_t] = t * d.scale;
+        }
+        __syncthreads();
+    }
+}
+
 __global__ __launch_bounds__(256) void wgrad_reduce_kernel(const float* __restrict__ part, int splits, int RS, int Ci,
                                                            int Co, float* __restrict__ dW, long s_co, long s_ci, long s_t,
                                                            float scale) {
-    __shared__ float red[8][33];
-    const long total = (long)RS * Ci * Co;
-    const int ox = threadIdx.x & 31, sl = threadIdx.x >> 5;
-    for (long base = (long)blockIdx.x * 32; base < total; base += (long)gridDim.x * 32) {
-        long i = base + ox;
-        float s = 0.f;
-        if (i < total)
-            for (int z = sl; z < splits; z += 8) s += part[(long)z * total + i];
-        red[sl][ox] = s;
-        __syncthreads();
-        if (sl == 0 && i < total) {
-            float a = 0.f;
-#pragma unroll
-            for (int k = 0; k < 8; ++k) a += red[k][ox];
-            int co = (int)(i % Co);
-            long rr = i / Co;
-            int ci = (int)(rr % Ci);
-            int t = (int)(rr / Ci);
-            dW[co * s_co + ci * s_ci + t * s_t] = a * scale;
-        }
-        __syncthreads();
-    }
+    __shared__ float4 red[8][33];
+    const umi_wgrad_pending d{part, dW, s_co, s_ci, s_t, scale, splits, RS, Ci, Co};
+    wg_reduce_elems<false>(d, red, (int)blockIdx.x, (int)gridDim.x);
 }
 
 __global__ __launch_bounds__(256) void wgrad_reduce_v4_kernel(const float* __restrict__ part, int splits, int RS, int Ci,
                                                               int Co, float* __restrict__ dW, long s_co, long s_ci, long s_t,
                                                               float scale) {
     __shared__ float4 red[8][33];
-    const long total4 = (long)RS * Ci * Co / 4;
-    const int Co4 = Co >> 2;
-    const int ox = threadIdx.x & 31, sl = threadIdx.x >> 5;
-    for (long base = (long)blockIdx.x * 32; base < total4; base += (long)gridDim.x * 32) {
-        const long i = base + ox;
-        float4 a = make_float4(0.f, 0.f, 0.f, 0.f), b = a;
-        if (i < total4) {
-            const float4* p = reinterpret_cast<const float4*>(part) + i;
-            int z = sl;
-            for (; z + 8 < splits; z += 16) {
-                float4 u = p[(long)z * total4], v = p[(long)(z + 8) * total4];
-                a.x += u.x; a.y += u.y; a.z += u.z; a.w += u.w;
-                b.x += v.x; b.y += v.y; b.z += v.z; b.w += v.w;
-            }
-            if (z < splits) { float4 u = p[(long)z * total4]; a.x += u.x; a.y += u.y; a.z += u.z; a.w += u.w; }
-        }
-        red[sl][ox] = make_float4(a.x + b.x, a.y + b.y, a.z + b.z, a.w + b.w);
-        __syncthreads();
-        if (sl == 0 && i < total4) {
-            float4 t4 = red[0][ox];
-#pragma unroll
-            for (int k = 1; k < 8; ++k) { float4 u = red[k][ox]; t4.x += u.x; t4.y += u.y; t4.z += u.z; t4.w += u.w; }
-            const int co = (int)(i % Co4) * 4;
-            const long rr = i / Co4;
-            const int ci = (int)(rr % Ci), t = (int)(rr / Ci);
-            float* o = dW + ci * s_ci + t * s_t;
-            o[(co + 0) * s_co] = t4.x * scale;
-            o[(co + 1) * s_co] = t4.y * scale;
-            o[(co + 2) * s_co] = t4.z * scale;
-            o[(co + 3) * s_co] = t4.w * scale;
-        }
-        __syncthreads();
-    }
+    const umi_wgrad_pending d{part, dW, s_co, s_ci, s_t, scale, splits, RS, Ci, Co};
+    wg_reduce_elems<true>(d, red, (int)blockIdx.x, (int)gridDim.x);
 }
 
 constexpr int WGT_CO = 32, WGT_CI = 8;
@@ -923,51 +969,114 @@
     if (d.s_co == d.RS && d.s_ci == (long)d.Co * d.RS) return 2;
     return 0;
 }
+constexpr int WGT_EPT = (WGT_CI * 9 * (WGT_CO / 4) + 255) / 256;
+
+template <int NS>
+__device__ __forceinline__ float4 wg_tree_few(const float4* v) {
+    float4 t = make_float4(0.f, 0.f, 0.f, 0.f);
+#pragma unroll
+    for (int l = 0; l < 8; ++l) {
+        float4 a = make_float4(0.f, 0.f, 0.f, 0.f);
+        const float4 b = a;
+        if (l < NS) wg_add4(a, v[l]);
+        const float4 s = make_float4(a.x + b.x, a.y + b.y, a.z + b.z, a.w + b.w);
+        if (l == 0) t = s; else wg_add4(t, s);
+    }
+    return t;
+}
+template <int NS, int EB>
+__device__ __forceinline__ void wg_tile_few(const float4* __restrict__ p0, const int* off, int nel, long total4, float4* out) {
+#pragma unroll
+    for (int i0 = 0; i0 < WGT_EPT; i0 += EB) {
+        float4 v[EB][NS];
+#pragma unroll
+        for (int i = 0; i < EB; ++i)
+            if (i0 + i < WGT_EPT && (int)threadIdx.x + 256 * (i0 + i) < nel) {
+#pragma unroll
+                for (int l = 0; l < NS; ++l) v[i][l] = p0[off[i0 + i] + (long)l * total4];
+            }
+#pragma unroll
+        for (int i = 0; i < EB; ++i)
+            if (i0 + i < WGT_EPT && (int)threadIdx.x + 256 * (i0 + i) < nel) out[i0 + i] = wg_tree_few<NS>(v[i]);
+    }
+}
+__device__ __forceinline__ float4 wg_tile_many(const float4* __restrict__ p, long total4, int splits) {
+    float4 t = make_float4(0.f, 0.f, 0.f, 0.f);
+    const int nj = (splits + 7) >> 3;
+#pragma unroll
+    for (int l0 = 0; l0 < 8; l0 += 4) {
+        float4 a[4], b[4];
+#pragma unroll
+        for (int l = 0; l < 4; ++l) a[l] = b[l] = make_float4(0.f, 0.f, 0.f, 0.f);
+        for (int j = 0; j < nj; j += 2) {
+            float4 v[8];
+#pragma unroll
+            for (int u = 0; u < 8; ++u) { const int z = l0 + (u & 3) + 8 * (j + (u >> 2)); v[u] = p[(long)(z < splits ? z : splits - 1) * total4]; }
+#pragma unroll
+            for (int u = 0; u < 8; ++u) wg_pin4(v[u]);
+#pragma unroll
+            for (int u = 0; u < 8; ++u)
+                if (l0 + (u & 3) + 8 * (j + (u >> 2)) < splits) wg_add4(u < 4 ? a[u & 3] : b[u & 3], v[u]);
+        }
+#pragma unroll
+        for (int l = 0; l < 4; ++l) {
+            const float4 s = make_float4(a[l].x + b[l].x, a[l].y + b[l].y, a[l].z + b[l].z, a[l].w + b[l].w);
+            if (l0 + l == 0) t = s; else wg_add4(t, s);
+        }
+    }
+    return t;
+}
+
 __device__ void wg_reduce_tiles(const umi_wgrad_pending& d, int mode, int my_blk, int n_blk) {
-    __shared__ float4 redt[8][33];
     __shared__ float tile[WGT_CO * WGT_CI * 9 + 64];
-    const int ox = threadIdx.x & 31, sl = threadIdx.x >> 5;
-    const int RS = d.RS, ncob = d.Co / WGT_CO, ncib = d.Ci / WGT_CI, rows = WGT_CI * RS;
+    const int RS = d.RS, ncob = d.Co / WGT_CO, ncib = d.Ci / WGT_CI;
+    const int nel = WGT_CI * RS * (WGT_CO / 4);
     const long total4 = (long)RS * d.Ci * d.Co / 4;
+    const float4* __restrict__ part4 = reinterpret_cast<const float4*>(d.part);
     for (int tl = my_blk; tl < ncob * ncib; tl += n_blk) {
         const int cob = tl % ncob, cib = tl / ncob;
-        for (int r0 = 0; r0 < rows; r0 += 4) {
-            const int row = r0 + (ox >> 3), c4 = ox & 7;
-            const int tap = row / WGT_CI, cil = row - tap * WGT_CI;
-            float4 a = make_float4(0.f, 0.f, 0.f, 0.f), b = a;
-            if (row < rows) {
-                const float4* p = reinterpret_cast<const float4*>(d.part) + (((long)tap * d.Ci + cib * WGT_CI + cil) * d.Co + cob * WGT_CO) / 4 + c4;
-                int z = sl;
-                for (; z + 8 < d.splits; z += 16) {
-                    float4 u = p[(long)z * total4], v = p[(long)(z + 8) * total4];
-                    a.x += u.x; a.y += u.y; a.z += u.z; a.w += u.w;
-                    b.x += v.x; b.y += v.y; b.z += v.z; b.w += v.w;
-                }
-                if (z < d.splits) { float4 u = p[(long)z * total4]; a.x += u.x; a.y += u.y; a.z += u.z; a.w += u.w; }
-                a = make_float4(a.x + b.x, a.y + b.y, a.z + b.z, a.w + b.w);
-            }
-            redt[sl][ox] = a;
-            __syncthreads();
-            if (sl == 0 && row < rows) {
-                float4 t4 = redt[0][ox];
-#pragma unroll
-                for (int k = 1; k < 8; ++k) { float4 u = redt[k][ox]; t4.x += u.x; t4.y += u.y; t4.z += u.z; t4.w += u.w; }
-                const float v[4] = {t4.x * d.scale, t4.y * d.scale, t4.z * d.scale, t4.w * d.scale};
-#pragma unroll
-                for (int k = 0; k < 4; ++k) {
-                    const int co = c4 * 4 + k;
-                    const int idx = mode == 1 ? co * (WGT_CI * RS + 1) + cil * RS + tap : cil * (WGT_CO * RS + 1) + co * RS + tap;
-                    tile[idx] = v[k];
-                }
-            }
-            __syncthreads();
-        }
+        const float4* p0 = part4 + ((long)cib * WGT_CI * d.Co + cob * WGT_CO) / 4;
+        int off[WGT_EPT];
+#pragma unroll
+        for (int i = 0; i < WGT_EPT; ++i) {
+            const int e = (int)threadIdx.x + 256 * i, row = e >> 3;
+            off[i] = e < nel ? (int)((((long)(row / WGT_CI) * d.Ci + row % WGT_CI) * d.Co) / 4) + (e & 7) : 0;
+        }
+        float4 r[WGT_EPT];
+        switch (d.splits) {
+        case 1: wg_tile_few<1, WGT_EPT>(p0, off, nel, total4, r); break;
+        case 2: wg_tile_few<2, WGT_EPT>(p0, off, nel, total4, r); break;
+        case 3: wg_tile_few<3, WGT_EPT>(p0, off, nel, total4, r); break;
+        case 4: wg_tile_few<4, WGT_EPT>(p0, off, nel, total4, r); break;
+        case 5: wg_tile_few<5, 1>(p0, off, nel, total4, r); break;
+        case 6: wg_tile_few<6, 1>(p0, off, nel, total4, r); break;
+        case 7: wg_tile_few<7, 1>(p0, off, nel, total4, r); break;
+        case 8: wg_tile_few<8, 1>(p0, off, nel, total4, r); break;
+        default:
+#pragma unroll
+            for (int i = 0; i < WGT_EPT; ++i)
+                if ((int)threadIdx.x + 256 * i < nel) r[i] = wg_tile_many(p0 + off[i], total4, d.splits);
+        }
+#pragma unroll
+        for (int i = 0; i < WGT_EPT; ++i) {
+            const int e = (int)threadIdx.x + 256 * i, row = e >> 3, c4 = e & 7;
+            if (e >= nel) continue;
+            const int tap = row / WGT_CI, cil = row % WGT_CI;
+            const float v[4] = {r[i].x * d.scale, r[i].y * d.scale, r[i].z * d.scale, r[i].w * d.scale};
+#pragma unroll
+            for (int k = 0; k < 4; ++k) {
+                const int co = c4 * 4 + k;
+                const int idx = mode == 1 ? co * (WGT_CI * RS + 1) + cil * RS + tap : cil * (WGT_CO * RS + 1) + co * RS + tap;
+                tile[idx] = v[k];
+            }
+        }
+        __syncthreads();
         const int inner = mode == 1 ? WGT_CI * RS : WGT_CO * RS, outer = mode == 1 ? WGT_CO : WGT_CI;
         for (int e = threadIdx.x; e < inner * outer; e += 256) {
-            const int o = e / inner, r = e - o * inner;
-            float* dst = mode == 1 ? d.dW + (long)(cob * WGT_CO + o) * d.s_co + (long)(cib * WGT_CI) * d.s_ci + r
-                                   : d.dW + (long)(cib * WGT_CI + o) * d.s_ci + (long)(cob * WGT_CO) * d.s_co + r;
-            *dst = tile[o * (inner + 1) + r];
+            const int o = e / inner, r_ = e - o * inner;
+            float* dst = mode == 1 ? d.dW + (long)(cob * WGT_CO + o) * d.s_co + (long)(cib * WGT_CI) * d.s_ci + r_
+                                   : d.dW + (long)(cib * WGT_CI + o) * d.s_ci + (long)(cob * WGT_CO) * d.s_co + r_;
+            *dst = tile[o * (inner + 1) + r_];
         }
         __syncthreads();
     }
@@ -982,55 +1091,8 @@
     const umi_wgrad_pending d = t.e[ent];
     const int my_blk = (int)blockIdx.x - t.blk0[ent], n_blk = t.blk0[ent + 1] - t.blk0[ent];
     if (const int tm = wg_tmode(d)) { wg_reduce_tiles(d, tm, my_blk, n_blk); return; }
-    const int ox = threadIdx.x & 31, sl = threadIdx.x >> 5;
-    const bool vec = d.Co % 4 == 0 && (((uintptr_t)d.part) & 15) == 0;
-    const int W4 = vec ? 4 : 1;
-    const long total = (long)d.RS * d.Ci * d.Co / W4;
-    const int CoW = d.Co / W4;
-    for (long base = (long)my_blk * 32; base < total; base += (long)n_blk * 32) {
-        const long i = base + ox;
-        float4 a = make_float4(0.f, 0.f, 0.f, 0.f), b = a;
-        if (i < total) {
-            if (vec) {
-                const float4* p = reinterpret_cast<const float4*>(d.part) + i;
-                int z = sl;
-                for (; z + 8 < d.splits; z += 16) {
-                    float4 u = p[(long)z * total], v = p[(long)(z + 8) * total];
-                    a.x += u.x; a.y += u.y; a.z += u.z; a.w += u.w;
-                    b.x += v.x; b.y += v.y; b.z += v.z; b.w += v.w;
-                }
-                if (z < d.splits) { float4 u = p[(long)z * total]; a.x += u.x; a.y += u.y; a.z += u.z; a.w += u.w; }
-                a = make_float4(a.x + b.x, a.y + b.y, a.z + b.z, a.w + b.w);
-            } else {
-                for (int z = sl; z < d.splits; z += 8) a.x += d.part[(long)z * total + i];
-            }
-        }
-        red[sl][ox] = a;
-        __syncthreads();
-        if (sl == 0 && i < total) {
-            float4 t4 = red[0][ox];
-            if (vec) {
-#pragma unroll
-                for (int k = 1; k < 8; ++k) { float4 u = red[k][ox]; t4.x += u.x; t4.y += u.y; t4.z += u.z; t4.w += u.w; }
-            } else {
-                float s0 = 0.f;
-#pragma unroll
-                for (int k = 0; k < 8; ++k) s0 += red[k][ox].x;
-                t4.x = s0;
-            }
-            const int co = (int)(i % CoW) * W4;
-            const long rr = i / CoW;
-            const int ci = (int)(rr % d.Ci), tp = (int)(rr / d.Ci);
-            float* o = d.dW + ci * d.s_ci + tp * d.s_t;
-            o[(co + 0) * d.s_co] = t4.x * d.scale;
-            if (vec) {
-                o[(co + 1) * d.s_co] = t4.y * d.scale;
-                o[(co + 2) * d.s_co] = t4.z * d.scale;
-                o[(co + 3) * d.s_co] = t4.w * d.scale;
-            }
-        }
-        __syncthreads();
-    }
+    if (d.Co % 4 == 0 && (((uintptr_t)d.part) & 15) == 0) wg_reduce_elems<true>(d, red, my_blk, n_blk);
+    else wg_reduce_elems<false>(d, red, my_blk, n_blk);
 }
 
 extern "C" int umi_wgrad_reduce_group(int n, const void* items, umi_stream_t stream) {
diff --git a/unet-torch_amd/csrc/optim_kernels.hip b/unet-torch_amd/csrc/optim_kernels.hip
--- a/unet-torch_amd/csrc/optim_kernels.hip
+++ b/unet-torch_amd/csrc/optim_kernels.hip
@@ -161,6 +161,106 @@
     }
 }
 
+template <typename T, int U>
+__device__ __forceinline__ void pack_stage_v4(const umi_pack_desc& d, T* tl, int k0, int n0, bool k_inner) {
+    const int TT = d.T, nq = PT / 4 * TT;
+    const int i0 = k_inner ? k0 : n0, o0 = k_inner ? n0 : k0;
+    const int I = k_inner ? d.K : d.N, O = k_inner ? d.N : d.K;
+    const long so = k_inner ? d.sn : d.sk;
+    const int vq = i0 < I ? (I - i0 < PT ? I - i0 : PT) * TT / 4 : 0;
+    const float* base = d.src + (long)(i0 < I ? i0 : 0) * TT;
+    for (int e0 = threadIdx.x; e0 < PT * nq; e0 += 256 * U) {
+        float4 v[U];
+        int ol[U], q[U];
+        bool ok[U];
+#pragma unroll
+        for (int u = 0; u < U; ++u) {
+            const int e = e0 + 256 * u;
+            ol[u] = e / nq;
+            q[u] = e - ol[u] * nq;
+            ok[u] = e < PT * nq && q[u] < vq && o0 + ol[u] < O;
+            const int oc = o0 + ol[u] < O ? o0 + ol[u] : O - 1, qc = q[u] < vq ? q[u] : (vq ? vq - 1 : 0);
+            v[u] = *reinterpret_cast<const float4*>(base + (long)oc * so + 4 * qc);
+        }
+#pragma unroll
+        for (int u = 0; u < U; ++u) asm volatile("" : "+v"(v[u].x), "+v"(v[u].y), "+v"(v[u].z), "+v"(v[u].w));
+#pragma unroll
+        for (int u = 0; u < U; ++u) {
+            if (e0 + 256 * u >= PT * nq) continue;
+            const float f[4] = {v[u].x, v[u].y, v[u].z, v[u].w};
+#pragma unroll
+            for (int j = 0; j < 4; ++j) {
+                const int r = 4 * q[u] + j, il = r / TT, ts = r - il * TT;
+                const int t = d.flip_t ? TT - 1 - ts : ts;
+                const int kl = k_inner ? il : ol[u], nl = k_inner ? ol[u] : il;
+                tl[(t * PT + kl) * (PT + 2) + nl] = (T)(ok[u] ? f[j] : 0.f);
+            }
+        }
+    }
+}
+
+__device__ inline bool pack_v4_ok(const umi_pack_desc& d, bool k_inner) {
+    const long si = k_inner ? d.sk : d.sn, so = k_inner ? d.sn : d.sk;
+    const int I = k_inner ? d.K : d.N;
+    return d.st == 1 && si == d.T && I % 4 == 0 && so % 4 == 0 && (((uintptr_t)d.src) & 15) == 0;
+}
+
+template <typename T>
+__device__ void pack_tiles_k8_pair(const umi_pack_desc& f, const umi_pack_desc& g, int my_blk, int n_blk) {
+    __shared__ T tl[9 * PT * (PT + 2)];
+    const int nkt = (f.Kpad + PT - 1) / PT, nnt = (f.Npad + PT - 1) / PT;
+    const int kb8 = f.Kpad >> 3, ldn = f.ldn ? f.ldn : f.Npad, TT = f.T;
+    const int gkb8 = f.Npad >> 3, gldn = g.ldn ? g.ldn : f.Kpad;
+    const bool k_inner = f.sk <= f.sn, v4 = pack_v4_ok(f, k_inner);
+    const bool gflip = (g.flip_t != 0) != (f.flip_t != 0);
+    T* dst = (T*)f.dst;
+    T* gdst = (T*)g.dst;
+    typedef T vec8 __attribute__((ext_vector_type(8)));
+    for (int tile = my_blk; tile < nkt * nnt; tile += n_blk) {
+        const int k0 = (tile % nkt) * PT, n0 = (tile / nkt) * PT;
+        if (v4) {
+            if (TT == 9) pack_stage_v4<T, 9>(f, tl, k0, n0, k_inner);
+            else if (TT == 4) pack_stage_v4<T, 4>(f, tl, k0, n0, k_inner);
+            else pack_stage_v4<T, 1>(f, tl, k0, n0, k_inner);
+        } else if (TT == 9) pack_stage<T, 12>(f, tl, k0, n0, k_inner);
+        else pack_stage<T, 4>(f, tl, k0, n0, k_inner);
+        __syncthreads();
+        for (int e = threadIdx.x; e < TT * (PT / 8) * PT; e += 256) {
+            const int nl = e % PT, r = e / PT, kg = r % (PT / 8), t = r / (PT / 8);
+            const int k = k0 + kg * 8, n = n0 + nl;
+            if (k >= f.Kpad || n >= f.Npad) continue;
+            vec8 pv;
+#pragma unroll
+            for (int j = 0; j < 8; ++j) pv[j] = tl[(t * PT + kg * 8 + j) * (PT + 2) + nl];
+            *reinterpret_cast<vec8*>(dst + (((long)t * kb8 + (k >> 3)) * ldn + n) * 8) = pv;
+        }
+        for (int e = threadIdx.x; e < TT * (PT / 8) * PT; e += 256) {
+            const int kl = e % PT, r = e / PT, ng = r % (PT / 8), t = r / (PT / 8);
+            const int k = k0 + kl, n = n0 + ng * 8;
+            if (k >= f.Kpad || n >= f.Npad) continue;
+            vec8 pv;
+#pragma unroll
+            for (int j = 0; j < 8; ++j) pv[j] = tl[(t * PT + kl) * (PT + 2) + ng * 8 + j];
+            const int tg = gflip ? TT - 1 - t : t;
+            *reinterpret_cast<vec8*>(gdst + (((long)tg * gkb8 + (n >> 3)) * gldn + k) * 8) = pv;
+        }
+        __syncthreads();
+    }
+}
+
+template <typename T>
+__global__ __launch_bounds__(256) void pack_pairs_kernel(const umi_pack_desc* __restrict__ descs, int n_pairs) {
+    const int blk = blockIdx.x;
+    int lo = 0, hi = n_pairs - 1;
+    while (lo < hi) {
+        const int mid = (lo + hi + 1) >> 1;
+        if (descs[2 * mid].blk0 <= blk) lo = mid; else hi = mid - 1;
+    }
+    const umi_pack_desc f = descs[2 * lo], g = descs[2 * lo + 1];
+    const int n_blk = ((f.Kpad + PT - 1) / PT) * ((f.Npad + PT - 1) / PT);
+    pack_tiles_k8_pair<T>(f, g, blk - f.blk0, n_blk);
+}
+
 template <typename T>
 __global__ __launch_bounds__(256) void pack_multi_kernel(const umi_pack_desc* __restrict__ descs, int n_desc) {
     const int blk = blockIdx.x;
@@ -309,3 +409,12 @@
     UMI_LAUNCH_CHECK();
     return UMI_OK;
 }
+
+extern "C" int umi_pack_kn8_pairs(const void* descs, int n_pairs, int total_blocks, int dtype, umi_stream_t stream) {
+    if (!descs || n_pairs <= 0 || total_blocks <= 0 || (((uintptr_t)descs) & 7)) return UMI_ERR_BADARG;
+    if (dtype != UMI_F16) return UMI_ERR_UNSUPPORTED;
+    hipLaunchKernelGGL((pack_pairs_kernel<half_t>), dim3(total_blocks), dim3(256), 0, (hipStream_t)stream,
+                       (const umi_pack_desc*)descs, n_pairs);
+    UMI_LAUNCH_CHECK();
+    return UMI_OK;
+}
diff --git a/unet-torch_amd/umi/graph.py b/unet-torch_amd/umi/graph.py
--- a/unet-torch_amd/umi/graph.py
+++ b/unet-torch_amd/umi/graph.py
@@ -236,14 +236,14 @@
                 if fuse:
                     dz = self.alloc(N, Ho, Wo, Co, device=out.device)
                     if ops.conv_wgrad_bnapply(a.raw, a.tx, o.grad, out, tx, rstd, dbeta, dgamma, dz, gw, Ci * R * S, R * S, 1,
-                                              inv, R, S, stride, pad):
+                                              inv, R, S, stride, pad, defer=self.deferred.open("wgrad_reduce", fills=(gw,))):
                         o.grad = dz
                     else:
                         fuse = False
                         ops.bn_bwd_apply(o.grad, out, tx, rstd, dbeta, dgamma)
                 if stem_fuse:
                     if not ops.conv_wgrad_bnapply(a.raw, a.tx, o.grad, out, tx, rstd, dbeta, dgamma, None, gw, Ci * R * S, R * S, 1,
-                                                  inv, R, S, stride, pad):
+                                                  inv, R, S, stride, pad, defer=self.deferred.open("wgrad_reduce", fills=(gw,))):
                         stem_fuse = False
                         ops.bn_bwd_apply(o.grad, out, tx, rstd, dbeta, dgamma)
                 if not fuse and not stem_fuse:
diff --git a/unet-torch_amd/umi/ops.py b/unet-torch_amd/umi/ops.py
--- a/unet-torch_amd/umi/ops.py
+++ b/unet-torch_amd/umi/ops.py
@@ -1,3 +1,5 @@
+
+import os
 
 import numpy as np
 import torch
@@ -286,26 +288,58 @@
         L.call("umi_wstd_bwd_multi", dev_ptr, n, rows, g_flat.data_ptr(), dw_flat.data_ptr() if dw_flat is not None else None,
                _stream())
 
+    @staticmethod
+    def _pairs(its):
+        first, mate = {}, {}
+        for i, (_, e, w) in enumerate(its):
+            T, K, N, st, sk, sn, flip = e.args
+            if not e.k8 or e.ldn or T > 9 or K % 8 or N % 8:
+                continue
+            j = first.get((w.data_ptr(), T, N, K, st, sn, sk))
+            if j is not None and j not in mate and not its[j][1].args[6]:
+                mate[j] = i
+            else:
+                first.setdefault((w.data_ptr(), T, K, N, st, sk, sn), i)
+        used = set(mate) | set(mate.values())
+        return [(its[j], its[i]) for j, i in mate.items()], [it for i, it in enumerate(its) if i not in used]
+
     def _repack(self, items):
         by_dtype = {}
         for it in items:
             by_dtype.setdefault(it[1].dst.dtype, []).append(it)
         blk = None
         for dtype, its in by_dtype.items():
-            tkey = tuple((id(e), w.data_ptr()) for _, e, w in its)
-            tab = self._tables.get(tkey)
-            if tab is None:
-                blk = blk or L.fn("umi_pack_block_elems")()
-                arr = np.zeros(len(its), dtype=_PACK_DESC)
-                b0 = 0
-                for i, (_, e, w) in enumerate(its):
-                    T, K, N, st, sk, sn, flip = e.args
-                    arr[i] = (w.data_ptr(), e.ptr, st, sk, sn, T, K, N, flip, K, N, int(e.k8), b0, e.ldn, 0)
-                    b0 += (T * K * N + blk - 1) // blk
-                tab = self._tables[tkey] = (self._upload(arr), b0, len(its))
-            dev_ptr, total, n = tab
-            L.call("umi_pack_kn_multi", dev_ptr, n, total, L.UMI_F32 if dtype == torch.float32 else L.UMI_F16,
-                   _stream())
+            pairs, rest = self._pairs(its) if dtype == torch.float16 and os.environ.get("UMI_NO_PACK_PAIRS") != "1" else ([], its)
+            if pairs:
+                tkey = ("pairs",) + tuple((id(f[1]), id(g[1]), f[2].data_ptr()) for f, g in pairs)
+                tab = self._tables.get(tkey)
+                if tab is None:
+                    arr = np.zeros(2 * len(pairs), dtype=_PACK_DESC)
+                    b0 = 0
+                    for i, (f, g) in enumerate(pairs):
+                        for j, (_, e, w) in enumerate((f, g)):
+                            T, K, N, st, sk, sn, flip = e.args
+                            arr[2 * i + j] = (w.data_ptr(), e.ptr, st, sk, sn, T, K, N, flip, K, N, 1, b0, 0, 0)
+                        T, K, N = f[1].args[:3]
+                        b0 += ((K + 31) // 32) * ((N + 31) // 32)
+                    tab = self._tables[tkey] = (self._upload(arr), b0, len(pairs))
+                dev_ptr, total, n = tab
+                L.call("umi_pack_kn8_pairs", dev_ptr, n, total, L.UMI_F16, _stream())
+            if rest:
+                tkey = tuple((id(e), w.data_ptr()) for _, e, w in rest)
+                tab = self._tables.get(tkey)
+                if tab is None:
+                    blk = blk or L.fn("umi_pack_block_elems")()
+                    arr = np.zeros(len(rest), dtype=_PACK_DESC)
+                    b0 = 0
+                    for i, (_, e, w) in enumerate(rest):
+                        T, K, N, st, sk, sn, flip = e.args
+                        arr[i] = (w.data_ptr(), e.ptr, st, sk, sn, T, K, N, flip, K, N, int(e.k8), b0, e.ldn, 0)
+                        b0 += (T * K * N + blk - 1) // blk
+                    tab = self._tables[tkey] = (self._upload(arr), b0, len(rest))
+                dev_ptr, total, n = tab
+                L.call("umi_pack_kn_multi", dev_ptr, n, total, L.UMI_F32 if dtype == torch.float32 else L.UMI_F16,
+                       _stream())
             for _, e, w in its:
                 e.ver = self._ver(w)
 
@@ -542,18 +576,28 @@
            sum_dz.data_ptr(), sum_dzx.data_ptr(), N * H * W, C, _dt(y), _stream())
 
 
-def conv_wgrad_bnapply(x, txa, da, y, tx_bn, rstd, sum_dz, sum_dzx, dz, dW, s_co, s_ci, s_t, out_scale, R, S, stride, pad):
+def conv_wgrad_bnapply(x, txa, da, y, tx_bn, rstd, sum_dz, sum_dzx, dz, dW, s_co, s_ci, s_t, out_scale, R, S, stride, pad, defer=None):
+    import ctypes
     N, H, W, Ci, ldx = _nhwc(x)
     _, Ho, Wo, Co, ldda = _nhwc(da)
     if (Ho, Wo) != (H, W) or da.dtype != torch.float16:
         return False
     assert dW.dtype == torch.float32 and dW.is_contiguous() and (dz is None or dz.shape == da.shape)
     nb = L.fn("umi_conv_wgrad_ws_bytes")(N, Ho, Wo, Ci, Co, R, S, _dt(x), 0)
-    ws = workspace(nb, x.device)
-    return L.supported("umi_conv_wgrad_bnapply", x.data_ptr(), ldx, _ptr(txa), da.data_ptr(), ldda, y.data_ptr(), _nhwc(y)[4],
-                       tx_bn.data_ptr(), rstd.data_ptr(), sum_dz.data_ptr(), sum_dzx.data_ptr(),
-                       _ptr(dz), _nhwc(dz)[4] if dz is not None else 0, dW.data_ptr(), s_co, s_ci, s_t, out_scale,
-                       N, H, W, Ci, Co, R, S, stride, pad, _dt(x), 0, ws.data_ptr(), ws.numel(), _stream())
+    args = (x.data_ptr(), ldx, _ptr(txa), da.data_ptr(), ldda, y.data_ptr(), _nhwc(y)[4],
+            tx_bn.data_ptr(), rstd.data_ptr(), sum_dz.data_ptr(), sum_dzx.data_ptr(),
+            _ptr(dz), _nhwc(dz)[4] if dz is not None else 0, dW.data_ptr(), s_co, s_ci, s_t, out_scale,
+            N, H, W, Ci, Co, R, S, stride, pad, _dt(x), 0)
+    if defer is None:
+        ws = workspace(nb, x.device)
+        return L.supported("umi_conv_wgrad_bnapply", *args, ws.data_ptr(), ws.numel(), _stream())
+    ws = torch.empty(max(nb, 16), dtype=torch.uint8, device=x.device)
+    pend = _WgPending()
+    if not L.supported("umi_conv_wgrad_bnapply_deferred", *args, ws.data_ptr(), ws.numel(), ctypes.addressof(pend), _stream()):
+        return False
+    if pend.part:
+        defer.append((pend, ws, dW))
+    return True
 
 
 _WgPending = L.STRUCTS["umi_wgrad_pending"]
```
